# NVlabs/nvbio

Measured on AMD Instinct MI355X. Metric: aligned reads/s (100 bp, band=15), higher is better.
Workload: dtype int32 results (int16 lanes where proven exact; all-int32 kernel in roofline.a32); 1 GPU; nvbio::aln batched banded SW (configs[1]): 10000000 x 100 bp reads vs 150 bp windows per GPU, band=15, LOCAL Gotoh (2,-1,-2,-1); reads_per_gpu=10000000, read_len=100, band=15, type=LOCAL, parallelism=read-shard x1, gather to rank 0

## Files before the change

### include/nvbio_hip.h

```cpp
#ifndef NVBIO_HIP_H
#define NVBIO_HIP_H

#include <stdint.h>

#ifdef __cplusplus
extern "C" {
#endif

#define NVBIO_HIP_ABI_VERSION 2

enum { NVBIO_HIP_GLOBAL = 0, NVBIO_HIP_LOCAL = 1, NVBIO_HIP_SEMI_GLOBAL = 2 };

typedef struct nvbio_hip_string_set {
    const uint32_t* words;
    uint64_t        n_words;
    uint32_t        bits;
    uint32_t        big_endian;
    const uint64_t* begin;
    const uint32_t* length;
    uint32_t        fixed_length;
    uint32_t        _pad;
} nvbio_hip_string_set;

typedef struct nvbio_hip_gotoh_scheme {
    int32_t match, mismatch, gap_open, gap_ext;
} nvbio_hip_gotoh_scheme;


int nvbio_hip_banded_gotoh_score(
    const nvbio_hip_gotoh_scheme* scheme , int32_t type, uint32_t band_len,
    const nvbio_hip_string_set* patterns ,
    const nvbio_hip_string_set* texts    ,
    uint32_t max_pattern_len, uint32_t max_text_len ,
    uint32_t n, int32_t* out_score, uint32_t* out_sink, void* stream);

int nvbio_hip_gotoh_score(
    const nvbio_hip_gotoh_scheme* scheme , int32_t type,
    const nvbio_hip_string_set* patterns, const nvbio_hip_string_set* texts,
    uint32_t max_pattern_len, uint32_t max_text_len, const int32_t* min_score ,
    uint32_t n, int32_t* out_score, uint32_t* out_sink, uint8_t* out_ok, void* stream);

typedef struct nvbio_hip_sw_scheme { int32_t match, mismatch, deletion, insertion; } nvbio_hip_sw_scheme;

int nvbio_hip_banded_sw_score(
    const nvbio_hip_sw_scheme* scheme , int32_t type, uint32_t band_len,
    const nvbio_hip_string_set* patterns, const nvbio_hip_string_set* texts,
    uint32_t max_pattern_len, uint32_t max_text_len,
    uint32_t n, int32_t* out_score, uint32_t* out_sink, void* stream);
int nvbio_hip_sw_score(
    const nvbio_hip_sw_scheme* scheme , int32_t type,
    const nvbio_hip_string_set* patterns, const nvbio_hip_string_set* texts,
    uint32_t max_pattern_len, uint32_t max_text_len,
    uint32_t n, int32_t* out_score, uint32_t* out_sink, void* stream);

enum { NVBIO_HIP_GOTOH_ALIGNER = 0, NVBIO_HIP_SW_ALIGNER = 1 };
enum { NVBIO_HIP_PATTERN_BLOCKING = 0, NVBIO_HIP_TEXT_BLOCKING = 1 };
int nvbio_hip_alignment_score(
    int32_t aligner, int32_t algorithm, const int32_t* scheme4 , int32_t type,
    const nvbio_hip_string_set* patterns, const nvbio_hip_string_set* texts,
    uint32_t max_pattern_len, uint32_t max_text_len, const int32_t* min_score ,
    uint32_t n, int32_t* out_score, uint32_t* out_sink, uint8_t* out_ok , void* stream);

typedef struct nvbio_hip_gotoh_qual_scheme {
    int32_t match;
    int32_t pattern_gap_open, pattern_gap_ext, text_gap_open, text_gap_ext;
    int32_t mismatch[256];
} nvbio_hip_gotoh_qual_scheme;

int nvbio_hip_banded_gotoh_score_qual(
    const nvbio_hip_gotoh_qual_scheme* scheme , int32_t type, uint32_t band_len,
    const nvbio_hip_string_set* patterns, const uint8_t* quals, uint64_t n_quals,
    const nvbio_hip_string_set* texts,
    uint32_t max_pattern_len, uint32_t max_text_len,
    uint32_t n, int32_t* out_score, uint32_t* out_sink, void* stream);

int nvbio_hip_banded_gotoh_score_qual_views(
    const nvbio_hip_gotoh_qual_scheme* scheme , int32_t type, uint32_t band_len,
    const nvbio_hip_string_set* patterns, const uint8_t* quals, uint64_t n_quals, const uint8_t* pattern_flags ,
    const nvbio_hip_string_set* texts,
    uint32_t max_pattern_len, uint32_t max_text_len,
    uint32_t n, int32_t* out_score, uint32_t* out_sink, void* stream);

int nvbio_hip_banded_gotoh_score_qual_wave(
    const nvbio_hip_gotoh_qual_scheme* scheme, int32_t type, uint32_t band_len,
    const nvbio_hip_string_set* patterns, const uint8_t* quals , uint64_t n_quals,
    const nvbio_hip_string_set* texts, uint32_t max_pattern_len,
    uint32_t n, const uint32_t* n_on_device , const uint32_t* job_index , const uint32_t* out_index ,
    const uint32_t* gate , uint32_t gate_limit,
    int32_t* out_score, uint32_t* out_sink, void* stream);

int nvbio_hip_banded_gotoh_score_qual_bounded(
    const nvbio_hip_gotoh_qual_scheme* scheme, int32_t type, uint32_t band_len,
    const nvbio_hip_string_set* patterns, const uint8_t* quals, uint64_t n_quals, const uint8_t* pattern_flags,
    const nvbio_hip_string_set* texts,
    uint32_t max_pattern_len, uint32_t max_text_len,
    uint32_t n, const uint32_t* n_on_device, const int32_t* min_score, uint32_t* work_counter, const uint32_t* out_index,
    const uint32_t* gate , uint32_t gate_limit,
    int32_t* out_score, uint32_t* out_sink, void* stream);

uint64_t nvbio_hip_banded_gotoh_traceback_temp_bytes(uint32_t band_len, uint32_t max_pattern_len, uint32_t n);
int nvbio_hip_banded_gotoh_traceback(
    const nvbio_hip_gotoh_scheme* scheme , int32_t type, uint32_t band_len,
    const nvbio_hip_string_set* patterns, const nvbio_hip_string_set* texts,
    uint32_t max_pattern_len, uint32_t max_text_len, uint32_t n,
    int32_t* out_score, uint32_t* out_sink, uint32_t* out_source,
    uint16_t* out_cigar, uint32_t cigar_stride, uint32_t* out_cigar_len,
    void* temp, uint64_t temp_bytes, void* stream);
int nvbio_hip_banded_gotoh_traceback_qual(
    const nvbio_hip_gotoh_qual_scheme* scheme , int32_t type, uint32_t band_len,
    const nvbio_hip_string_set* patterns, const uint8_t* quals, uint64_t n_quals,
    const nvbio_hip_string_set* texts,
    uint32_t max_pattern_len, uint32_t max_text_len, uint32_t n,
    int32_t* out_score, uint32_t* out_sink, uint32_t* out_source,
    uint16_t* out_cigar, uint32_t cigar_stride, uint32_t* out_cigar_len,
    void* temp, uint64_t temp_bytes, void* stream);
int nvbio_hip_banded_gotoh_traceback_qual_known(
    const nvbio_hip_gotoh_qual_scheme* scheme , int32_t type, uint32_t band_len,
    const nvbio_hip_string_set* patterns, const uint8_t* quals, uint64_t n_quals,
    const nvbio_hip_string_set* texts,
    uint32_t max_pattern_len, uint32_t max_text_len, uint32_t n,
    int32_t* score , uint32_t* sink , uint32_t* out_source,
    uint16_t* out_cigar, uint32_t cigar_stride, uint32_t* out_cigar_len,
    void* temp, uint64_t temp_bytes, void* stream);

uint64_t nvbio_hip_gotoh_traceback_temp_bytes(uint32_t max_pattern_len, uint32_t max_text_len, uint32_t n);
int nvbio_hip_gotoh_traceback(
    const nvbio_hip_gotoh_scheme* scheme , int32_t type,
    const nvbio_hip_string_set* patterns, const nvbio_hip_string_set* texts,
    uint32_t max_pattern_len, uint32_t max_text_len, uint32_t n,
    int32_t* out_score, uint32_t* out_sink, uint32_t* out_source,
    uint16_t* out_cigar, uint32_t cigar_stride, uint32_t* out_cigar_len,
    void* temp, uint64_t temp_bytes, void* stream);

int nvbio_hip_gotoh_traceback_qual(
    const nvbio_hip_gotoh_qual_scheme* scheme , int32_t type,
    const nvbio_hip_string_set* patterns, const uint8_t* quals, uint64_t n_quals, const nvbio_hip_string_set* texts,
    uint32_t max_pattern_len, uint32_t max_text_len, uint32_t n,
    int32_t* out_score, uint32_t* out_sink, uint32_t* out_source,
    uint16_t* out_cigar, uint32_t cigar_stride, uint32_t* out_cigar_len,
    void* temp, uint64_t temp_bytes, void* stream);

int nvbio_hip_gotoh_traceback_known_score(
    const nvbio_hip_gotoh_scheme* scheme , int32_t type,
    const nvbio_hip_string_set* patterns, const nvbio_hip_string_set* texts, const int32_t* known_score,
    uint32_t max_pattern_len, uint32_t max_text_len, uint32_t n,
    int32_t* out_score, uint32_t* out_sink, uint32_t* out_source,
    uint16_t* out_cigar, uint32_t cigar_stride, uint32_t* out_cigar_len,
    void* temp, uint64_t temp_bytes, void* stream);
int nvbio_hip_gotoh_traceback_qual_known_score(
    const nvbio_hip_gotoh_qual_scheme* scheme , int32_t type,
    const nvbio_hip_string_set* patterns, const uint8_t* quals, uint64_t n_quals, const nvbio_hip_string_set* texts, const int32_t* known_score,
    uint32_t max_pattern_len, uint32_t max_text_len, uint32_t n,
    int32_t* out_score, uint32_t* out_sink, uint32_t* out_source,
    uint16_t* out_cigar, uint32_t cigar_stride, uint32_t* out_cigar_len,
    void* temp, uint64_t temp_bytes, void* stream);

uint64_t nvbio_hip_known_score_redone(void);

int nvbio_hip_banded_sw_traceback(
    const nvbio_hip_sw_scheme* scheme , int32_t type, uint32_t band_len,
    const nvbio_hip_string_set* patterns, const nvbio_hip_string_set* texts,
    uint32_t max_pattern_len, uint32_t max_text_len, uint32_t n,
    int32_t* out_score, uint32_t* out_sink, uint32_t* out_source,
    uint16_t* out_cigar, uint32_t cigar_stride, uint32_t* out_cigar_len,
    void* temp, uint64_t temp_bytes, void* stream);
int nvbio_hip_sw_traceback(
    const nvbio_hip_sw_scheme* scheme , int32_t type,
    const nvbio_hip_string_set* patterns, const nvbio_hip_string_set* texts,
    uint32_t max_pattern_len, uint32_t max_text_len, uint32_t n,
    int32_t* out_score, uint32_t* out_sink, uint32_t* out_source,
    uint16_t* out_cigar, uint32_t cigar_stride, uint32_t* out_cigar_len,
    void* temp, uint64_t temp_bytes, void* stream);

int nvbio_hip_alignment_score_qual(
    const nvbio_hip_gotoh_qual_scheme* scheme , int32_t algorithm, int32_t type,
    const nvbio_hip_string_set* patterns, const uint8_t* quals, uint64_t n_quals, const nvbio_hip_string_set* texts,
    uint32_t max_pattern_len, uint32_t max_text_len, const int32_t* min_score ,
    uint32_t n, int32_t* out_score, uint32_t* out_sink, uint8_t* out_ok , void* stream);

int nvbio_hip_alignment_score_qual_jobs(
    const nvbio_hip_gotoh_qual_scheme* scheme , int32_t algorithm, int32_t type,
    const nvbio_hip_string_set* patterns, const uint8_t* quals, uint64_t n_quals, const nvbio_hip_string_set* texts,
    uint32_t max_pattern_len, uint32_t max_text_len, const int32_t* min_score ,
    uint32_t n, const uint32_t* n_on_device, const uint32_t* job_index, const uint32_t* gate, uint32_t gate_limit, int32_t wave_form,
    int32_t* out_score, uint32_t* out_sink, uint8_t* out_ok , void* stream);

int nvbio_hip_hamming_score(
    const nvbio_hip_sw_scheme* scheme , int32_t algorithm, int32_t type,
    const nvbio_hip_string_set* patterns, const nvbio_hip_string_set* texts,
    uint32_t max_pattern_len, uint32_t max_text_len, const int32_t* min_score ,
    uint32_t n, int32_t* out_score, uint32_t* out_sink, uint8_t* out_ok , void* stream);
int nvbio_hip_hamming_score_qual(
    const nvbio_hip_gotoh_qual_scheme* scheme , int32_t algorithm, int32_t type,
    const nvbio_hip_string_set* patterns, const uint8_t* quals, uint64_t n_quals, const nvbio_hip_string_set* texts,
    uint32_t max_pattern_len, uint32_t max_text_len, const int32_t* min_score ,
    uint32_t n, int32_t* out_score, uint32_t* out_sink, uint8_t* out_ok , void* stream);
int nvbio_hip_hamming_score_qual_jobs(
    const nvbio_hip_gotoh_qual_scheme* scheme , int32_t algorithm, int32_t type,
    const nvbio_hip_string_set* patterns, const uint8_t* quals, uint64_t n_quals, const nvbio_hip_string_set* texts,
    uint32_t max_pattern_len, uint32_t max_text_len, const int32_t* min_score ,
    uint32_t n, const uint32_t* n_on_device, const uint32_t* job_index, const uint32_t* gate, uint32_t gate_limit, int32_t wave_form,
    int32_t* out_score, uint32_t* out_sink, uint8_t* out_ok , void* stream);

typedef struct nvbio_hip_fmindex {
    uint32_t        length;
    uint32_t        primary;
    uint32_t        L2[5];
    uint32_t        sa_int;
    const uint32_t* bwt_occ;
    const uint32_t* ssa;
    const uint32_t* ktab;
    uint32_t        ktab_k;
    uint32_t        _pad;
    const uint32_t* dimer;
    uint32_t        dimer_p1, dimer_fill1;
    uint32_t        dimer_S[4], dimer_T[4];
    const uint32_t* trimer;
} nvbio_hip_fmindex;

int nvbio_hip_fm_rank(const nvbio_hip_fmindex* fmi, const uint32_t* k, const uint8_t* c,
                      uint32_t n, uint32_t* out, void* stream);

int nvbio_hip_fm_rank4(const nvbio_hip_fmindex* fmi, const uint32_t* k,
                       uint32_t n, uint32_t* out, void* stream);

int nvbio_hip_fm_rank_range(const nvbio_hip_fmindex* fmi, const uint32_t* range, const uint8_t* c,
                            uint32_t n, uint32_t* out, void* stream);

int nvbio_hip_fm_match(const nvbio_hip_fmindex* fmi, const nvbio_hip_string_set* seeds,
                       uint32_t n, uint32_t* out_range, void* stream);

uint64_t nvbio_hip_fm_dimer_index_bytes(uint32_t length);
uint64_t nvbio_hip_fm_build_dimer_index_temp_bytes(uint32_t length);
int nvbio_hip_fm_build_dimer_index(const nvbio_hip_fmindex* fmi, uint32_t* out_dimer, void* temp, uint64_t temp_bytes, void* stream);
int nvbio_hip_fm_attach_dimer_index(nvbio_hip_fmindex* fmi, const uint32_t* dimer, void* stream);

uint64_t nvbio_hip_fm_trimer_index_bytes(uint32_t length);
uint64_t nvbio_hip_fm_build_trimer_index_temp_bytes(uint32_t length);
int nvbio_hip_fm_build_trimer_index(const nvbio_hip_fmindex* fmi, uint32_t* out_trimer, void* temp, uint64_t temp_bytes, void* stream);
int nvbio_hip_fm_attach_trimer_index(nvbio_hip_fmindex* fmi, const uint32_t* trimer, void* stream);

int nvbio_hip_banded_gotoh_score_host(const nvbio_hip_gotoh_scheme* scheme, int32_t type, uint32_t band_len,
                                      const nvbio_hip_string_set* patterns, const nvbio_hip_string_set* texts,
                                      uint32_t n, int32_t* out_score, uint32_t* out_sink, int32_t n_threads);
int nvbio_hip_banded_sw_score_host(const nvbio_hip_sw_scheme* scheme, int32_t type, uint32_t band_len,
                                   const nvbio_hip_string_set* patterns, const nvbio_hip_string_set* texts,
                                   uint32_t n, int32_t* out_score, uint32_t* out_sink, int32_t n_threads);
int nvbio_hip_alignment_score_host(int32_t aligner, int32_t algorithm, const int32_t* scheme4, int32_t type,
                                   const nvbio_hip_string_set* patterns, const nvbio_hip_string_set* texts, const int32_t* min_score ,
                                   uint32_t n, int32_t* out_score, uint32_t* out_sink, uint8_t* out_ok , int32_t n_threads);
int nvbio_hip_hamming_score_host(const nvbio_hip_sw_scheme* scheme, int32_t algorithm, int32_t type,
                                 const nvbio_hip_string_set* patterns, const nvbio_hip_string_set* texts, const int32_t* min_score ,
                                 uint32_t n, int32_t* out_score, uint32_t* out_sink, uint8_t* out_ok , int32_t n_threads);
int nvbio_hip_hamming_score_qual_host(const nvbio_hip_gotoh_qual_scheme* scheme, int32_t algorithm, int32_t type,
                                      const nvbio_hip_string_set* patterns, const uint8_t* quals, uint64_t n_quals, const nvbio_hip_string_set* texts,
                                      const int32_t* min_score ,
                                      uint32_t n, int32_t* out_score, uint32_t* out_sink, uint8_t* out_ok , int32_t n_threads);
int nvbio_hip_fm_rank_host(const nvbio_hip_fmindex* fmi, const uint32_t* k, const uint8_t* c, uint32_t n, uint32_t* out, int32_t n_threads);
int nvbio_hip_fm_match_host(const nvbio_hip_fmindex* fmi, const nvbio_hip_string_set* seeds, uint32_t n, uint32_t* out_range, int32_t n_threads);
int nvbio_hip_fm_locate_host(const nvbio_hip_fmindex* fmi, const uint32_t* sa_rows, uint32_t n, uint32_t* out_pos, int32_t n_threads);

int nvbio_hip_fm_build_ktab(const nvbio_hip_fmindex* fmi, uint32_t k, uint32_t* out_ktab, void* stream);
uint64_t nvbio_hip_fm_dense_ssa_entries(uint32_t length, uint32_t sa_int);
int nvbio_hip_fm_build_dense_ssa(const nvbio_hip_fmindex* fmi, uint32_t sa_int_out, uint32_t* out_ssa, void* stream);

typedef struct nvbio_hip_map_params {
    uint32_t seed_len;
    uint32_t min_read_len;
    uint32_t max_hits;
    uint32_t max_reseed;
    uint32_t retry;
    uint32_t rep_seeds;
    uint32_t fw, rc;
} nvbio_hip_map_params;

int nvbio_hip_map_exact(const nvbio_hip_fmindex* fmi, const nvbio_hip_string_set* reads,
                        const uint32_t* in_queue, uint32_t n, const nvbio_hip_map_params* params ,
                        const uint32_t* seed_freq_by_len ,
                        uint64_t* out_hits, uint32_t hits_stride, uint32_t* out_counts, uint8_t* out_reseed, void* stream);

enum { NVBIO_HIP_EXACT_MAPPING = 0, NVBIO_HIP_APPROX_MAPPING = 1, NVBIO_HIP_CASE_PRUNING_MAPPING = 2 };

int nvbio_hip_map(int32_t algorithm, uint32_t subseed_len,
                  const nvbio_hip_fmindex* fmi, const nvbio_hip_fmindex* rfmi ,
                  const nvbio_hip_string_set* reads, const uint32_t* in_queue, uint32_t n,
                  const nvbio_hip_map_params* params , const uint32_t* seed_freq_by_len ,
                  uint64_t* out_hits, uint32_t hits_stride, uint32_t* out_counts, uint8_t* out_reseed, void* stream);

uint64_t nvbio_hip_alignment_invalid(void);
int nvbio_hip_init_alignments(uint32_t n_reads, const uint32_t* read_len , uint32_t fixed_read_len,
                              const int32_t* worst_score_by_len , uint32_t mate,
                              uint64_t* best_alignments, uint32_t best_stride, void* stream);
int nvbio_hip_score_reduce(uint32_t n_active, const uint32_t* read_ids , const uint64_t* hit_begin,
                           const int32_t* hit_score, const uint32_t* hit_loc, const uint8_t* hit_rc,
                           const uint32_t* read_len , uint32_t fixed_read_len,
                           uint64_t* best_alignments, uint32_t best_stride, void* stream);

uint32_t nvbio_hip_sum_tree_node_count(uint32_t size);
int nvbio_hip_select_init(uint32_t n_reads, const char* read_names, const uint32_t* read_names_idx,
                          const uint64_t* hits, uint32_t hits_stride, const uint32_t* hit_counts,
                          float* probs, uint32_t probs_stride, uint32_t* trys , uint32_t* rseeds,
                          uint32_t max_effort_init, int32_t randomized, int32_t top_seed, void* stream);
int nvbio_hip_select_init_queued(uint32_t n_queue, const uint32_t* queue, const char* read_names, const uint32_t* read_names_idx,
                                 const uint64_t* hits, uint32_t hits_stride, const uint32_t* hit_counts,
                                 float* probs, uint32_t probs_stride, uint32_t* trys , uint32_t* rseeds,
                                 uint32_t max_effort_init, int32_t randomized, int32_t top_seed, void* stream);
uint64_t nvbio_hip_select_temp_bytes(uint32_t n_active, uint32_t n_multi);
int nvbio_hip_select(int32_t randomized, uint32_t n_multi, const uint32_t* active_in, uint32_t n_active,
                     uint64_t* hits, uint32_t hits_stride, uint32_t* hit_counts,
                     float* probs, uint32_t probs_stride, uint32_t* rseeds, const uint32_t* trys,
                     uint32_t* active_out, uint64_t* hit_begin, uint32_t* hit_read_id, uint32_t* hit_loc, uint32_t* hit_seed,
                     uint32_t* out_sizes, void* temp, uint64_t temp_bytes, void* stream);
int nvbio_hip_hit_deque_replay(uint32_t n_cases, const uint32_t* case_start, const uint8_t* ops, const uint64_t* vals, const uint32_t* caps,
                               const uint64_t* state_start, uint64_t* scratch, uint32_t scratch_stride, uint64_t* out_states, void* stream);
int nvbio_hip_locate_hits(const nvbio_hip_fmindex* fmi, const nvbio_hip_fmindex* rfmi, uint32_t n,
                          uint32_t* hit_loc, const uint32_t* hit_seed, void* stream);
int nvbio_hip_score_best_setup(uint32_t n_hits, const uint32_t* hit_read_id, const uint32_t* hit_loc, const uint32_t* hit_seed,
                               const uint64_t* read_begin , const uint32_t* read_len , uint32_t fixed_read_len,
                               uint64_t rc_offset, uint32_t band_len, uint32_t genome_length,
                               const uint64_t* best_alignments, uint32_t best_stride, int32_t score_limit,
                               uint64_t* pattern_begin, uint32_t* pattern_len ,
                               uint64_t* text_begin, uint32_t* text_len, int32_t* min_score,
                               int32_t* known_score ,
                               uint32_t* job_count , uint32_t* job_hit , void* stream);
int nvbio_hip_score_reduce_best_approx(uint32_t n_active, const uint32_t* active_reads, const uint64_t* hit_begin,
                                       const int32_t* hit_score, const uint32_t* hit_loc, const uint32_t* hit_seed,
                                       const uint32_t* read_len , uint32_t fixed_read_len,
                                       uint64_t* best_alignments, uint32_t best_stride, int32_t worst_score,
                                       uint32_t* trys, uint32_t* hit_counts,
                                       uint32_t n_ext, uint32_t min_ext, uint32_t max_ext, uint32_t max_effort,
                                       const int32_t* known_score ,
                                       const uint32_t* hit_sink , uint32_t* best_sink ,
                                       void* stream);
int nvbio_hip_traceback_best_known(uint32_t n, const uint32_t* idx , const uint64_t* best_alignments, const uint32_t* best_sink ,
                                   int32_t* out_score, uint32_t* out_sink , void* stream);

int nvbio_hip_score_reduce_paired(uint32_t n_active, const uint32_t* read_ids , const uint64_t* hit_begin,
    const uint32_t* hit_loc, const uint32_t* hit_sink, const int32_t* hit_score, const uint8_t* hit_rc,
    const uint32_t* opposite_loc, const uint32_t* opposite_sink, const uint32_t* opposite_sink2,
    const int32_t* opposite_score, const int32_t* opposite_score2,
    const uint32_t* read_len , uint32_t fixed_read_len, uint32_t anchor, int32_t pe_policy, int32_t pe_unpaired, int32_t score_limit,
    uint64_t* best_alignments, uint64_t* best_alignments_o, uint32_t best_stride, void* stream);

typedef struct nvbio_hip_pe_params {
    int32_t  pe_policy, min_frag_len, max_frag_len, pe_overlap, score_limit;
    uint32_t anchor, genome_length;
} nvbio_hip_pe_params;

int nvbio_hip_opposite_mate_windows(uint32_t n_hits, const uint32_t* hit_read_id, const uint8_t* hit_rc, const uint32_t* hit_loc, const int32_t* hit_score,
    const uint32_t* a_read_len , const uint32_t* o_read_len , uint32_t a_fixed_len, uint32_t o_fixed_len,
    const uint64_t* best_alignments, const uint64_t* best_alignments_o, uint32_t best_stride,
    int32_t match, const int32_t* min_score_by_len , int32_t text_gap_open, int32_t text_gap_ext, const nvbio_hip_pe_params* params ,
    uint8_t* out_valid, int32_t* out_min_score, uint8_t* out_read_rc, uint32_t* out_genome_begin, uint32_t* out_genome_end, void* stream);

int nvbio_hip_anchor_score_setup(uint32_t n_hits, const uint32_t* hit_read_id, const uint32_t* hit_loc, const uint32_t* hit_seed,
    const uint64_t* a_read_begin , const uint32_t* a_read_len , const uint32_t* o_read_len ,
    uint32_t a_fixed_len, uint32_t o_fixed_len, uint64_t rc_offset,
    uint32_t band_len, uint32_t genome_length, const uint64_t* best_alignments, const uint64_t* best_alignments_o, uint32_t best_stride,
    int32_t match, const int32_t* min_score_by_len , int32_t score_limit, uint32_t anchor,
    uint64_t* pattern_begin, uint32_t* pattern_len , uint64_t* text_begin, uint32_t* text_len, int32_t* min_score, void* stream);
int nvbio_hip_anchor_score_finish(uint32_t n_hits, const int32_t* raw_score, const uint32_t* raw_sink , const uint64_t* text_begin,
    const int32_t* min_score, int32_t worst_score, int32_t* hit_score, uint32_t* hit_sink, void* stream);
int nvbio_hip_opposite_score_setup(uint32_t n_hits, const uint32_t* hit_read_id, const uint32_t* hit_seed, const uint32_t* hit_loc, const int32_t* hit_score,
    int32_t worst_score, const uint32_t* a_read_len, const uint32_t* o_read_len, uint32_t a_fixed_len, uint32_t o_fixed_len,
    const uint64_t* best_alignments, const uint64_t* best_alignments_o, uint32_t best_stride,
    int32_t match, const int32_t* min_score_by_len , int32_t text_gap_open, int32_t text_gap_ext, const nvbio_hip_pe_params* params ,
    uint8_t* out_valid, int32_t* out_min_score, uint8_t* out_read_rc, uint32_t* out_genome_begin, uint32_t* out_genome_end,
    const uint64_t* o_read_begin, uint64_t o_rc_offset, uint64_t* out_pattern_begin, uint64_t* out_text_begin, uint32_t* out_text_len, void* stream);
int nvbio_hip_opposite_score_finish(uint32_t n_valid, const uint32_t* valid_idx, const uint8_t* valid_flags, const int32_t* raw_score , const uint32_t* raw_sink ,
    const int32_t* min_score , const uint32_t* genome_begin , int32_t worst_score,
    int32_t* opposite_score, int32_t* opposite_score2, uint32_t* opposite_loc, uint32_t* opposite_sink, uint32_t* opposite_sink2, void* stream);
int nvbio_hip_score_reduce_paired_best_approx(uint32_t n_active, const uint32_t* active_reads, const uint64_t* hit_begin,
    const uint32_t* hit_loc, const uint32_t* hit_sink, const int32_t* hit_score, const uint32_t* hit_seed,
    const uint32_t* opposite_loc, const uint32_t* opposite_sink, const uint32_t* opposite_sink2, const int32_t* opposite_score, const int32_t* opposite_score2,
    const uint32_t* read_len , uint32_t fixed_read_len, uint32_t anchor, int32_t pe_policy, int32_t pe_unpaired, int32_t score_limit,
    uint64_t* best_alignments, uint64_t* best_alignments_o, uint32_t best_stride,
    uint32_t* trys, uint32_t* hit_counts, uint32_t n_ext, uint32_t min_ext, uint32_t max_ext, uint32_t max_effort, void* stream);
int nvbio_hip_anchor_memo_mark(uint32_t n_hits, const uint32_t* hit_read_id, const uint32_t* hit_seed, const uint64_t* text_begin, const uint32_t* text_len,
    uint32_t anchor, const uint32_t* memo, uint8_t* from_memo, uint32_t* text_len_out,
    uint32_t* live_count , uint32_t* live_idx , void* stream);
int nvbio_hip_anchor_score_finish_memo(uint32_t n_hits, const int32_t* raw_score, const uint32_t* raw_sink, const uint64_t* text_begin, const int32_t* min_score,
    int32_t worst_score, const uint8_t* from_memo, const uint32_t* hit_read_id, const uint32_t* memo, int32_t* hit_score, uint32_t* hit_sink, void* stream);
int nvbio_hip_anchor_memo_update(uint32_t n_active, const uint32_t* active_reads, const uint64_t* hit_begin, const uint32_t* hit_read_id, const uint32_t* hit_seed,
    const uint64_t* text_begin, const uint32_t* text_len_setup, const uint8_t* from_memo, const int32_t* raw_score, const uint32_t* raw_sink, uint32_t anchor, uint32_t* memo, void* stream);
int nvbio_hip_list_flagged(uint32_t n, const uint8_t* flags, uint32_t value, uint32_t* count, uint32_t* idx, void* stream);
int nvbio_hip_opposite_memo_lookup(uint32_t n_hits, const uint32_t* hit_read_id, uint8_t* valid, const uint8_t* read_rc, const uint32_t* genome_begin,
    const uint32_t* genome_end, const int32_t* min_score, uint32_t anchor, const uint32_t* memo, int32_t worst_score,
    int32_t* opposite_score, int32_t* opposite_score2, uint32_t* opposite_loc, uint32_t* opposite_sink, uint32_t* opposite_sink2,
    uint32_t* text_len , void* stream);
int nvbio_hip_opposite_memo_update(uint32_t n_active, const uint32_t* active_reads, const uint64_t* hit_begin, const uint8_t* valid, const uint8_t* read_rc,
    const uint32_t* genome_begin, const uint32_t* genome_end, const int32_t* min_score, const int32_t* opposite_score, const uint32_t* opposite_sink,
    uint32_t anchor, uint32_t* memo, void* stream);
int nvbio_hip_mark_discordant(uint32_t n_reads, uint64_t* best_alignments, uint64_t* best_alignments_o, uint32_t best_stride, void* stream);

int nvbio_hip_pack_read_queue(uint32_t n, const uint32_t* queue, uint32_t top_flag, uint32_t* out, void* stream);

int nvbio_hip_mark_unaligned(uint32_t n_active, const uint32_t* active_reads, const uint64_t* best_alignments, uint8_t* reseed, void* stream);
uint64_t nvbio_hip_copy_flagged_temp_bytes(uint32_t n);
int nvbio_hip_copy_flagged(uint32_t n, const uint32_t* in, const uint8_t* flags, uint32_t* out, uint32_t* out_count ,
                           void* temp, uint64_t temp_bytes, void* stream);
int nvbio_hip_scatter_rows(uint32_t n, const uint32_t* idx, const void* src, void* dst, uint32_t row_bytes , void* stream);
int nvbio_hip_gather_rows(uint32_t n, const uint32_t* idx, const void* src, void* dst, uint32_t row_bytes , void* stream);
int nvbio_hip_traceback_best_setup(uint32_t n, const uint32_t* idx , const uint64_t* best_alignments, uint32_t band_len, uint32_t genome_length,
                                   const uint64_t* read_begin , const uint32_t* read_len , uint32_t fixed_read_len,
                                   uint64_t rc_offset, uint64_t mate_offset, int32_t want,
                                   uint8_t* out_valid, uint64_t* pattern_begin, uint32_t* pattern_len ,
                                   uint64_t* text_begin, uint32_t* text_len, void* stream);
int nvbio_hip_traceback_best_setup_mates(uint32_t n, const uint32_t* idx , const uint64_t* best_alignments, uint32_t band_len, uint32_t genome_length,
                                         const uint64_t* const read_begin[2] , const uint32_t* const read_len[2],
                                         const uint32_t fixed_read_len[2], const uint64_t rc_offset[2], uint64_t mate_offset, int32_t want,
                                         uint8_t* out_valid, uint64_t* pattern_begin, uint32_t* pattern_len, uint64_t* text_begin, uint32_t* text_len, void* stream);

int nvbio_hip_finish_alignment(uint32_t n, const uint8_t* valid, const nvbio_hip_string_set* patterns, const uint8_t* quals , uint64_t n_quals,
                               const nvbio_hip_string_set* texts, const uint16_t* cigar, uint32_t cigar_stride, const uint32_t* cigar_len,
                               const uint32_t* cigar_source , int32_t match, const int32_t* mismatch_by_quality , int32_t n_penalty,
                               const int32_t* gap_costs , const uint32_t* idx , uint64_t* best_alignments, uint8_t* out_mds, uint32_t mds_stride, uint32_t* out_mds_len, void* stream);

int nvbio_hip_gather_ranges(uint32_t n_ranges, uint32_t n_reads, const uint64_t* hits, uint32_t hits_stride, const uint32_t* hit_count_scan,
                            uint64_t* out_ranges, void* stream);
int nvbio_hip_select_all(uint64_t begin, uint32_t count, uint32_t n_reads, uint32_t n_ranges, const uint64_t* hits, uint32_t hits_stride,
                         const uint32_t* hit_count_scan, const uint64_t* hit_range_scan, uint32_t* out_loc, uint32_t* out_seed, uint32_t* out_read_id,
                         void* stream);
int nvbio_hip_mark_straddling(uint32_t n, const uint32_t* idx_queue, uint32_t n_sequences, const uint32_t* sequence_index, const uint32_t* hit_loc,
                              uint32_t seed_len, uint8_t* flags, void* stream);
int nvbio_hip_score_all_setup(uint32_t n, const uint32_t* idx , const uint32_t* hit_read_id, const uint32_t* hit_loc, const uint32_t* hit_seed,
                              const uint64_t* read_begin , const uint32_t* read_len , uint32_t fixed_read_len, uint64_t rc_offset,
                              uint32_t band_len, uint32_t genome_length,
                              uint64_t* pattern_begin, uint32_t* pattern_len , uint64_t* text_begin, uint32_t* text_len, void* stream);
int nvbio_hip_score_all_output(uint32_t n, const uint32_t* idx , const uint32_t* hit_read_id, const uint32_t* hit_loc, const uint32_t* hit_seed,
                               const int32_t* score, const int32_t* min_score_by_len , const uint32_t* read_len , uint32_t fixed_read_len,
                               uint8_t* out_flags, uint64_t* out_alignments, uint32_t* out_read_id, void* stream);
int nvbio_hip_traceback_all_setup(uint32_t n, const uint64_t* alignments, const uint32_t* read_id,
                                  const uint64_t* read_begin , const uint32_t* read_len , uint32_t fixed_read_len, uint64_t rc_offset,
                                  uint32_t band_len, uint32_t genome_length,
                                  uint64_t* pattern_begin, uint32_t* pattern_len , uint64_t* text_begin, uint32_t* text_len, void* stream);

uint64_t nvbio_hip_all_mapping_temp_bytes(uint32_t n);
int nvbio_hip_inclusive_scan_u32(uint32_t n, const uint32_t* in, uint32_t* out, void* temp, uint64_t temp_bytes, void* stream);
int nvbio_hip_inclusive_scan_u64(uint32_t n, const uint64_t* in, uint64_t* out, void* temp, uint64_t temp_bytes, void* stream);
int nvbio_hip_sort_hi_bits(uint32_t n, const uint32_t* keys, uint32_t* out_idx, void* temp, uint64_t temp_bytes, void* stream);
int nvbio_hip_sort_hits(uint32_t n, const uint32_t* hit_read_id, const uint32_t* hit_loc, const uint32_t* hit_seed, uint32_t* out_idx, uint8_t* out_first,
                        void* temp, uint64_t temp_bytes, void* stream);
int nvbio_hip_sort_hits_pingpong(uint32_t n, const uint32_t* hit_read_id, const uint32_t* hit_loc, const uint32_t* hit_seed, uint32_t* out_idx, uint8_t* out_first,
                                 uint32_t* out_stale, void* temp, uint64_t temp_bytes, void* stream);

int nvbio_hip_mapq(int32_t version, int32_t match, int32_t monotone, const int32_t* min_score_by_len ,
                   uint32_t n_reads, const uint64_t* best_alignments, uint32_t best_stride,
                   const uint32_t* read_len , uint32_t fixed_read_len, uint8_t* out_mapq, void* stream);

int nvbio_hip_mapq_paired(int32_t version, int32_t match, int32_t monotone, const int32_t* min_score_by_len ,
                          uint32_t n_reads, const uint64_t* best_alignments, const uint64_t* best_alignments_o, uint32_t best_stride,
                          const uint32_t* read_len , const uint32_t* o_read_len ,
                          uint32_t fixed_read_len, uint32_t o_fixed_read_len, uint8_t* out_mapq, void* stream);

int nvbio_hip_fm_locate(const nvbio_hip_fmindex* fmi, const uint32_t* sa_rows,
                        uint32_t n, uint32_t* out_pos, void* stream);

int nvbio_hip_fm_locate_ssa_iterator(const nvbio_hip_fmindex* fmi, const uint32_t* sa_rows,
                                     uint32_t n, uint32_t* out_it, void* stream);
int nvbio_hip_fm_lookup_ssa_iterator(const nvbio_hip_fmindex* fmi, const uint32_t* it,
                                     uint32_t n, uint32_t* out_pos, void* stream);

uint64_t nvbio_hip_fm_filter_temp_bytes(uint32_t n);
int nvbio_hip_fm_filter_rank(const nvbio_hip_fmindex* fmi, const nvbio_hip_string_set* seeds,
                             uint32_t n, uint32_t* out_range, uint64_t* out_slots,
                             void* temp, uint64_t temp_bytes, void* stream);

int nvbio_hip_fm_filter_locate(const nvbio_hip_fmindex* fmi, const uint32_t* range, const uint64_t* slots,
                               uint32_t n_queries, uint64_t begin, uint64_t end,
                               uint32_t* out_hits, void* stream);

#define NVBIO_HIP_EXTEND_FORWARD   0
#define NVBIO_HIP_EXTEND_BACKWARDS 1
int nvbio_hip_fm_extend(int32_t direction, const nvbio_hip_fmindex* f_fmi, const nvbio_hip_fmindex* r_fmi,
                        const uint32_t* f_ranges, const uint32_t* r_ranges, const uint8_t* c, uint32_t n,
                        uint32_t* out_f_ranges, uint32_t* out_r_ranges, void* stream);

#define NVBIO_HIP_ERROR_CAPACITY 0x10001
uint64_t nvbio_hip_fm_mem_temp_bytes(uint32_t n, uint32_t max_pattern_len);
int nvbio_hip_fm_mem_rank(const nvbio_hip_fmindex* f_fmi, const nvbio_hip_fmindex* r_fmi, const nvbio_hip_string_set* strings,
                          uint32_t n, uint32_t max_pattern_len, uint32_t min_intv, uint32_t max_intv, uint32_t min_span,
                          uint32_t* out_ranges, uint64_t capacity, uint64_t* out_index, uint64_t* out_slots, uint64_t* out_n_ranges,
                          void* temp, uint64_t temp_bytes, void* stream);

int nvbio_hip_fm_mem_locate(const nvbio_hip_fmindex* f_fmi, const uint32_t* ranges, const uint64_t* slots, uint64_t n_ranges,
                            uint64_t begin, uint64_t end, uint32_t* out_hits, void* stream);

int nvbio_hip_fm_extend_host(int32_t direction, const nvbio_hip_fmindex* f_fmi, const nvbio_hip_fmindex* r_fmi,
                             const uint32_t* f_ranges, const uint32_t* r_ranges, const uint8_t* c, uint32_t n,
                             uint32_t* out_f_ranges, uint32_t* out_r_ranges, int32_t n_threads);
int nvbio_hip_fm_mem_rank_host(const nvbio_hip_fmindex* f_fmi, const nvbio_hip_fmindex* r_fmi, const nvbio_hip_string_set* strings,
                               uint32_t n, uint32_t max_pattern_len, uint32_t min_intv, uint32_t max_intv, uint32_t min_span,
                               uint32_t* out_ranges, uint64_t capacity, uint64_t* out_index, uint64_t* out_slots, uint64_t* out_n_ranges,
                               uint64_t* out_records, int32_t n_threads);
int nvbio_hip_fm_mem_locate_host(const nvbio_hip_fmindex* f_fmi, const uint32_t* ranges, const uint64_t* slots, uint64_t n_ranges,
                                 uint64_t begin, uint64_t end, uint32_t* out_hits, int32_t n_threads);

uint64_t nvbio_hip_fm_mem_split_temp_bytes(uint32_t n, uint32_t max_pattern_len, uint64_t capacity);
int nvbio_hip_fm_mem_rank_split(const nvbio_hip_fmindex* f_fmi, const nvbio_hip_fmindex* r_fmi, const nvbio_hip_string_set* strings,
                                uint32_t n, uint32_t max_pattern_len, uint32_t min_intv, uint32_t max_intv, uint32_t min_span,
                                uint32_t split_len, uint32_t split_width,
                                uint32_t* out_ranges, uint64_t capacity, uint64_t* out_index, uint64_t* out_slots, uint64_t* out_n_ranges,
                                void* temp, uint64_t temp_bytes, void* stream);
int nvbio_hip_fm_mem_rank_split_host(const nvbio_hip_fmindex* f_fmi, const nvbio_hip_fmindex* r_fmi, const nvbio_hip_string_set* strings,
                                     uint32_t n, uint32_t max_pattern_len, uint32_t min_intv, uint32_t max_intv, uint32_t min_span,
                                     uint32_t split_len, uint32_t split_width,
                                     uint32_t* out_ranges, uint64_t capacity, uint64_t* out_index, uint64_t* out_slots, uint64_t* out_n_ranges,
                                     uint64_t* out_records, int32_t n_threads);

uint64_t nvbio_hip_build_bwt_occ_temp_bytes(uint32_t n);
int nvbio_hip_build_bwt_occ(uint32_t n, const uint32_t* bwt_words, uint32_t* out_bwt_occ, uint32_t* out_L2,
                            void* temp, uint64_t temp_bytes, void* stream);

uint64_t nvbio_hip_suffix_sort_temp_bytes(uint64_t n);
int nvbio_hip_suffix_sort(const uint32_t* words, uint32_t bits, uint32_t big_endian, uint64_t n, uint32_t* sa_out,
                          void* temp, uint64_t temp_bytes, void* stream);
uint32_t nvbio_hip_suffix_sort_last_rounds(uint64_t* out_unresolved, uint32_t capacity);
uint64_t nvbio_hip_bwt_temp_bytes(uint64_t n);
int nvbio_hip_bwt(const uint32_t* words, uint32_t bits, uint32_t big_endian, uint64_t n, uint32_t sa_int, uint32_t* bwt_words_out,
                  uint32_t* primary_out, uint32_t* ssa_out, uint32_t* sa_out, void* temp, uint64_t temp_bytes, void* stream);
int nvbio_hip_suffix_sort_host(const uint32_t* words, uint32_t bits, uint32_t big_endian, uint64_t n, uint32_t* sa_out, int32_t n_threads);
int nvbio_hip_bwt_host(const uint32_t* words, uint32_t bits, uint32_t big_endian, uint64_t n, uint32_t sa_int, uint32_t* bwt_words_out,
                       uint32_t* primary_out, uint32_t* ssa_out, uint32_t* sa_out, int32_t n_threads);

int nvbio_hip_device_malloc(void** ptr, uint64_t bytes);
int nvbio_hip_device_free(void* ptr);
int nvbio_hip_device_free_ordered(void* ptr);
int nvbio_hip_device_free_after(void* ptr, void* stream);
int nvbio_hip_device_trim(void);
int nvbio_hip_device_mem_info(uint64_t* free_bytes, uint64_t* total_bytes, uint64_t* idle_cached_bytes);
int nvbio_hip_memcpy(void* dst, const void* src, uint64_t bytes, int kind, void* stream);
int nvbio_hip_memset(void* dst, int value, uint64_t bytes, void* stream);
int nvbio_hip_stream_synchronize(void* stream);
int nvbio_hip_stream_query(void* stream);
int nvbio_hip_host_malloc(void** ptr, uint64_t bytes);
int nvbio_hip_host_free(void* ptr);

int nvbio_hip_stream_create(void** stream, uint32_t non_blocking);
int nvbio_hip_stream_destroy(void* stream);

int nvbio_hip_comm_available(void);
int nvbio_hip_device_count(void);
int nvbio_hip_set_device(int device);
int nvbio_hip_get_device(void);
int nvbio_hip_comm_unique_id(uint8_t* id128);
int nvbio_hip_comm_init_rank(void** comm, int world, int rank, const uint8_t* id128);
int nvbio_hip_comm_init_all(void** comms, int n_devices, const int* devices );
int nvbio_hip_comm_destroy(void* comm);
int nvbio_hip_comm_rank(void* comm, int* rank, int* world);
int nvbio_hip_gather_records(void* comm, const void* send, const uint64_t* counts, uint32_t record_bytes, void* recv , int root, void* stream);
int nvbio_hip_comm_abort(void* comm);
typedef struct nvbio_hip_comm_transport {
    int (*rank)(void* comm, int* rank, int* world);
    int (*group_start)(void* comm);
    int (*group_end)(void* comm);
    int (*send)(void* comm, const void* buf, uint64_t bytes, int peer, void* stream);
    int (*recv)(void* comm, void* buf, uint64_t bytes, int peer, void* stream);
    int (*copy)(void* comm, void* dst, const void* src, uint64_t bytes, void* stream);
    int (*abort)(void* comm);
} nvbio_hip_comm_transport;
void nvbio_hip_comm_set_transport(const nvbio_hip_comm_transport* transport);

int nvbio_hip_set_test_switch(const char* name, int value);
int nvbio_hip_get_test_switch(const char* name);
const char* nvbio_hip_test_switch_name(int index);

int         nvbio_hip_abi_version(void);
const char* nvbio_hip_arch(void);
const char* nvbio_hip_last_kernel(void);
const char* nvbio_hip_last_kernel_detail(void);
const char* nvbio_hip_last_kernel_cell(void);
const char* nvbio_hip_last_kernel_frame(void);
const char* nvbio_hip_last_kernel_row(void);
const char* nvbio_hip_last_kernel_const(void);
const char* nvbio_hip_last_kernel_fetch(void);

#ifdef __cplusplus
}
#endif
#endif
```

### nvbio_amd/_lib.py

```python
import ctypes as C
import os

HERE = os.path.dirname(os.path.abspath(__file__))
LIB_PATH = os.path.join(HERE, "lib", "libnvbio_hip.so")

SYMBOLS = [
    "nvbio_hip_banded_gotoh_score", "nvbio_hip_banded_gotoh_score_qual", "nvbio_hip_banded_gotoh_score_qual_views", "nvbio_hip_banded_gotoh_score_qual_bounded", "nvbio_hip_banded_gotoh_score_qual_wave", "nvbio_hip_gotoh_score", "nvbio_hip_banded_sw_score", "nvbio_hip_sw_score", "nvbio_hip_alignment_score", "nvbio_hip_alignment_score_qual", "nvbio_hip_alignment_score_qual_jobs",
    "nvbio_hip_hamming_score", "nvbio_hip_hamming_score_qual", "nvbio_hip_hamming_score_qual_jobs", "nvbio_hip_hamming_score_host", "nvbio_hip_hamming_score_qual_host",
    "nvbio_hip_banded_gotoh_traceback_temp_bytes", "nvbio_hip_banded_gotoh_traceback", "nvbio_hip_banded_gotoh_traceback_qual",
    "nvbio_hip_gotoh_traceback_temp_bytes", "nvbio_hip_gotoh_traceback", "nvbio_hip_gotoh_traceback_qual", "nvbio_hip_gotoh_traceback_known_score", "nvbio_hip_gotoh_traceback_qual_known_score", "nvbio_hip_known_score_redone", "nvbio_hip_banded_sw_traceback", "nvbio_hip_sw_traceback",
    "nvbio_hip_fm_rank", "nvbio_hip_fm_rank4", "nvbio_hip_fm_rank_range",
    "nvbio_hip_fm_match", "nvbio_hip_fm_build_ktab", "nvbio_hip_fm_dense_ssa_entries", "nvbio_hip_fm_build_dense_ssa",
    "nvbio_hip_banded_gotoh_score_host", "nvbio_hip_banded_sw_score_host", "nvbio_hip_alignment_score_host",
    "nvbio_hip_fm_rank_host", "nvbio_hip_fm_match_host", "nvbio_hip_fm_locate_host",
    "nvbio_hip_fm_dimer_index_bytes", "nvbio_hip_fm_build_dimer_index_temp_bytes", "nvbio_hip_fm_build_dimer_index", "nvbio_hip_fm_attach_dimer_index",
    "nvbio_hip_fm_trimer_index_bytes", "nvbio_hip_fm_build_trimer_index_temp_bytes", "nvbio_hip_fm_build_trimer_index", "nvbio_hip_fm_attach_trimer_index", "nvbio_hip_map_exact", "nvbio_hip_map",
    "nvbio_hip_alignment_invalid", "nvbio_hip_init_alignments", "nvbio_hip_score_reduce", "nvbio_hip_score_reduce_paired", "nvbio_hip_opposite_mate_windows", "nvbio_hip_mapq", "nvbio_hip_mapq_paired", "nvbio_hip_fm_locate",
    "nvbio_hip_sum_tree_node_count", "nvbio_hip_select_init", "nvbio_hip_select_init_queued", "nvbio_hip_select_temp_bytes", "nvbio_hip_select", "nvbio_hip_locate_hits", "nvbio_hip_hit_deque_replay",
    "nvbio_hip_score_best_setup", "nvbio_hip_score_reduce_best_approx",
    "nvbio_hip_anchor_score_setup", "nvbio_hip_anchor_score_finish", "nvbio_hip_anchor_memo_mark", "nvbio_hip_anchor_score_finish_memo", "nvbio_hip_anchor_memo_update", "nvbio_hip_opposite_score_setup", "nvbio_hip_opposite_score_finish",
    "nvbio_hip_score_reduce_paired_best_approx", "nvbio_hip_mark_discordant",
    "nvbio_hip_pack_read_queue", "nvbio_hip_mark_unaligned", "nvbio_hip_copy_flagged_temp_bytes", "nvbio_hip_copy_flagged", "nvbio_hip_traceback_best_setup", "nvbio_hip_traceback_best_setup_mates", "nvbio_hip_finish_alignment", "nvbio_hip_scatter_rows",
    "nvbio_hip_gather_ranges", "nvbio_hip_select_all", "nvbio_hip_mark_straddling", "nvbio_hip_score_all_setup", "nvbio_hip_score_all_output",
    "nvbio_hip_traceback_all_setup", "nvbio_hip_all_mapping_temp_bytes", "nvbio_hip_inclusive_scan_u32", "nvbio_hip_inclusive_scan_u64", "nvbio_hip_sort_hi_bits",
    "nvbio_hip_sort_hits", "nvbio_hip_sort_hits_pingpong", "nvbio_hip_gather_rows", "nvbio_hip_list_flagged", "nvbio_hip_opposite_memo_lookup", "nvbio_hip_opposite_memo_update", "nvbio_hip_traceback_best_known", "nvbio_hip_banded_gotoh_traceback_qual_known",
    "nvbio_hip_fm_locate_ssa_iterator", "nvbio_hip_fm_lookup_ssa_iterator",
    "nvbio_hip_fm_filter_temp_bytes", "nvbio_hip_fm_filter_rank", "nvbio_hip_fm_filter_locate",
    "nvbio_hip_fm_extend", "nvbio_hip_fm_mem_temp_bytes", "nvbio_hip_fm_mem_rank", "nvbio_hip_fm_mem_locate",
    "nvbio_hip_fm_extend_host", "nvbio_hip_fm_mem_rank_host", "nvbio_hip_fm_mem_locate_host",
    "nvbio_hip_fm_mem_split_temp_bytes", "nvbio_hip_fm_mem_rank_split", "nvbio_hip_fm_mem_rank_split_host",
    "nvbio_hip_build_bwt_occ_temp_bytes", "nvbio_hip_build_bwt_occ",
    "nvbio_hip_suffix_sort_temp_bytes", "nvbio_hip_suffix_sort", "nvbio_hip_suffix_sort_last_rounds", "nvbio_hip_bwt_temp_bytes", "nvbio_hip_bwt",
    "nvbio_hip_suffix_sort_host", "nvbio_hip_bwt_host",
    "nvbio_hip_device_malloc", "nvbio_hip_device_free", "nvbio_hip_device_free_ordered", "nvbio_hip_device_free_after", "nvbio_hip_device_trim", "nvbio_hip_device_mem_info", "nvbio_hip_memcpy", "nvbio_hip_memset",
    "nvbio_hip_stream_synchronize", "nvbio_hip_stream_query", "nvbio_hip_host_malloc", "nvbio_hip_host_free", "nvbio_hip_stream_create", "nvbio_hip_stream_destroy",
    "nvbio_hip_comm_available", "nvbio_hip_device_count", "nvbio_hip_set_device", "nvbio_hip_get_device", "nvbio_hip_comm_unique_id", "nvbio_hip_comm_init_rank",
    "nvbio_hip_comm_init_all", "nvbio_hip_comm_destroy", "nvbio_hip_comm_rank", "nvbio_hip_gather_records", "nvbio_hip_comm_abort", "nvbio_hip_comm_set_transport",
    "nvbio_hip_abi_version", "nvbio_hip_arch", "nvbio_hip_last_kernel", "nvbio_hip_last_kernel_detail", "nvbio_hip_last_kernel_cell", "nvbio_hip_last_kernel_frame", "nvbio_hip_last_kernel_row", "nvbio_hip_last_kernel_const", "nvbio_hip_last_kernel_fetch", "nvbio_hip_set_test_switch", "nvbio_hip_get_test_switch", "nvbio_hip_test_switch_name",
]


class PeParamsStruct(C.Structure):
    _fields_ = [("pe_policy", C.c_int32), ("min_frag_len", C.c_int32), ("max_frag_len", C.c_int32), ("pe_overlap", C.c_int32),
                ("score_limit", C.c_int32), ("anchor", C.c_uint32), ("genome_length", C.c_uint32)]


class StringSetStruct(C.Structure):
    _fields_ = [("words", C.c_void_p), ("n_words", C.c_uint64), ("bits", C.c_uint32), ("big_endian", C.c_uint32),
                ("begin", C.c_void_p), ("length", C.c_void_p), ("fixed_length", C.c_uint32), ("_pad", C.c_uint32)]


class GotohSchemeStruct(C.Structure):
    _fields_ = [("match", C.c_int32), ("mismatch", C.c_int32), ("gap_open", C.c_int32), ("gap_ext", C.c_int32)]


class GotohQualSchemeStruct(C.Structure):
    _fields_ = [("match", C.c_int32), ("pattern_gap_open", C.c_int32), ("pattern_gap_ext", C.c_int32),
                ("text_gap_open", C.c_int32), ("text_gap_ext", C.c_int32), ("mismatch", C.c_int32 * 256)]


class MapParamsStruct(C.Structure):
    _fields_ = [(k, C.c_uint32) for k in ("seed_len", "min_read_len", "max_hits", "max_reseed", "retry", "rep_seeds", "fw", "rc")]


class FMIndexStruct(C.Structure):
    _fields_ = [("length", C.c_uint32), ("primary", C.c_uint32), ("L2", C.c_uint32 * 5), ("sa_int", C.c_uint32),
                ("bwt_occ", C.c_void_p), ("ssa", C.c_void_p), ("ktab", C.c_void_p), ("ktab_k", C.c_uint32), ("_pad", C.c_uint32),
                ("dimer", C.c_void_p), ("dimer_p1", C.c_uint32), ("dimer_fill1", C.c_uint32),
                ("dimer_S", C.c_uint32 * 4), ("dimer_T", C.c_uint32 * 4), ("trimer", C.c_void_p)]


_lib = None
ABI_VERSION = 2
ERROR_CAPACITY = 0x10001


def lib():
    global _lib
    if _lib is None:
        if not os.path.exists(LIB_PATH):
            raise RuntimeError(
                "nvbio_amd: %s is missing -- build it with `python -m nvbio_amd.build` "
                "(hipcc --offload-arch=gfx950); there is no CPU fallback" % LIB_PATH)
        L = C.CDLL(LIB_PATH)
        try:
            L.nvbio_hip_abi_version.restype = C.c_int
            found = L.nvbio_hip_abi_version()
        except AttributeError:
            found = None
        if found != ABI_VERSION:
            raise RuntimeError("nvbio_amd: lib/libnvbio_hip.so has ABI version %s, this package needs %d -- rebuild it (python -m nvbio_amd.build)" % (found, ABI_VERSION))
        for s in SYMBOLS:
            getattr(L, s)
        vp, u32, u64, i32 = C.c_void_p, C.c_uint32, C.c_uint64, C.c_int32
        P = C.POINTER
        L.nvbio_hip_banded_gotoh_score.argtypes = [P(GotohSchemeStruct), i32, u32, P(StringSetStruct), P(StringSetStruct), u32, u32, u32, vp, vp, vp]
        L.nvbio_hip_banded_gotoh_score_qual.argtypes = [P(GotohQualSchemeStruct), i32, u32, P(StringSetStruct), vp, u64, P(StringSetStruct), u32, u32, u32, vp, vp, vp]
        L.nvbio_hip_banded_gotoh_score_qual_views.argtypes = [P(GotohQualSchemeStruct), i32, u32, P(StringSetStruct), vp, u64, vp, P(StringSetStruct), u32, u32, u32, vp, vp, vp]
        L.nvbio_hip_banded_gotoh_score_qual_bounded.argtypes = [P(GotohQualSchemeStruct), i32, u32, P(StringSetStruct), vp, u64, vp, P(StringSetStruct), u32, u32, u32, vp, vp, vp, vp, vp, u32, vp, vp, vp]
        L.nvbio_hip_banded_gotoh_score_qual_wave.argtypes = [P(GotohQualSchemeStruct), i32, u32, P(StringSetStruct), vp, u64, P(StringSetStruct), u32, u32, vp, vp, vp, vp, u32, vp, vp, vp]
        L.nvbio_hip_banded_gotoh_traceback_temp_bytes.argtypes = [u32, u32, u32]
        L.nvbio_hip_banded_gotoh_traceback_temp_bytes.restype = u64
        L.nvbio_hip_banded_gotoh_traceback.argtypes = [P(GotohSchemeStruct), i32, u32, P(StringSetStruct), P(StringSetStruct), u32, u32, u32,
                                                       vp, vp, vp, vp, u32, vp, vp, u64, vp]
        L.nvbio_hip_banded_gotoh_traceback_qual.argtypes = [P(GotohQualSchemeStruct), i32, u32, P(StringSetStruct), vp, u64, P(StringSetStruct), u32, u32, u32,
                                                            vp, vp, vp, vp, u32, vp, vp, u64, vp]
        L.nvbio_hip_banded_gotoh_traceback_qual_known.argtypes = [P(GotohQualSchemeStruct), i32, u32, P(StringSetStruct), vp, u64, P(StringSetStruct), u32, u32, u32,
                                                            vp, vp, vp, vp, u32, vp, vp, u64, vp]
        L.nvbio_hip_banded_sw_score.argtypes = [P(GotohSchemeStruct), i32, u32, P(StringSetStruct), P(StringSetStruct), u32, u32, u32, vp, vp, vp]
        L.nvbio_hip_sw_score.argtypes = [P(GotohSchemeStruct), i32, P(StringSetStruct), P(StringSetStruct), u32, u32, u32, vp, vp, vp]
        L.nvbio_hip_alignment_score.argtypes = [i32, i32, vp, i32, P(StringSetStruct), P(StringSetStruct), u32, u32, vp, u32, vp, vp, vp, vp]
        L.nvbio_hip_gotoh_traceback_temp_bytes.argtypes = [u32, u32, u32]
        L.nvbio_hip_gotoh_traceback_temp_bytes.restype = u64
        L.nvbio_hip_gotoh_traceback.argtypes = [P(GotohSchemeStruct), i32, P(StringSetStruct), P(StringSetStruct), u32, u32, u32,
                                                vp, vp, vp, vp, u32, vp, vp, u64, vp]
        L.nvbio_hip_gotoh_traceback_qual.argtypes = [P(GotohQualSchemeStruct), i32, P(StringSetStruct), vp, u64, P(StringSetStruct), u32, u32, u32,
                                                     vp, vp, vp, vp, u32, vp, vp, u64, vp]
        L.nvbio_hip_gotoh_traceback_known_score.argtypes = [P(GotohSchemeStruct), i32, P(StringSetStruct), P(StringSetStruct), vp, u32, u32, u32,
                                                            vp, vp, vp, vp, u32, vp, vp, u64, vp]
        L.nvbio_hip_gotoh_traceback_qual_known_score.argtypes = [P(GotohQualSchemeStruct), i32, P(StringSetStruct), vp, u64, P(StringSetStruct), vp, u32, u32, u32,
                                                                 vp, vp, vp, vp, u32, vp, vp, u64, vp]
        L.nvbio_hip_known_score_redone.argtypes = []; L.nvbio_hip_known_score_redone.restype = u64
        L.nvbio_hip_banded_sw_traceback.argtypes = [P(GotohSchemeStruct), i32, u32, P(StringSetStruct), P(StringSetStruct), u32, u32, u32,
                                                    vp, vp, vp, vp, u32, vp, vp, u64, vp]
        L.nvbio_hip_sw_traceback.argtypes = [P(GotohSchemeStruct), i32, P(StringSetStruct), P(StringSetStruct), u32, u32, u32,
                                             vp, vp, vp, vp, u32, vp, vp, u64, vp]
        L.nvbio_hip_alignment_score_qual.argtypes = [P(GotohQualSchemeStruct), i32, i32, P(StringSetStruct), vp, u64, P(StringSetStruct), u32, u32, vp, u32, vp, vp, vp, vp]
        L.nvbio_hip_gotoh_score.argtypes = [P(GotohSchemeStruct), i32, P(StringSetStruct), P(StringSetStruct), u32, u32, vp, u32, vp, vp, vp, vp]
        L.nvbio_hip_hamming_score.argtypes = [P(GotohSchemeStruct), i32, i32, P(StringSetStruct), P(StringSetStruct), u32, u32, vp, u32, vp, vp, vp, vp]
        L.nvbio_hip_hamming_score_qual.argtypes = [P(GotohQualSchemeStruct), i32, i32, P(StringSetStruct), vp, u64, P(StringSetStruct), u32, u32, vp, u32, vp, vp, vp, vp]
        L.nvbio_hip_hamming_score_qual_jobs.argtypes = [P(GotohQualSchemeStruct), i32, i32, P(StringSetStruct), vp, u64, P(StringSetStruct), u32, u32, vp,
                                                        u32, vp, vp, vp, u32, i32, vp, vp, vp, vp]
        L.nvbio_hip_hamming_score_host.argtypes = [P(GotohSchemeStruct), i32, i32, P(StringSetStruct), P(StringSetStruct), vp, u32, vp, vp, vp, i32]
        L.nvbio_hip_hamming_score_qual_host.argtypes = [P(GotohQualSchemeStruct), i32, i32, P(StringSetStruct), vp, u64, P(StringSetStruct), vp, u32, vp, vp, vp, i32]
        L.nvbio_hip_fm_rank.argtypes = [P(FMIndexStruct), vp, vp, u32, vp, vp]
        L.nvbio_hip_fm_rank4.argtypes = [P(FMIndexStruct), vp, u32, vp, vp]
        L.nvbio_hip_fm_rank_range.argtypes = [P(FMIndexStruct), vp, vp, u32, vp, vp]
        L.nvbio_hip_fm_match.argtypes = [P(FMIndexStruct), P(StringSetStruct), u32, vp, vp]
        L.nvbio_hip_fm_build_ktab.argtypes = [P(FMIndexStruct), u32, vp, vp]
        L.nvbio_hip_banded_gotoh_score_host.argtypes = [P(GotohSchemeStruct), i32, u32, P(StringSetStruct), P(StringSetStruct), u32, vp, vp, i32]
        L.nvbio_hip_banded_sw_score_host.argtypes = [P(GotohSchemeStruct), i32, u32, P(StringSetStruct), P(StringSetStruct), u32, vp, vp, i32]
        L.nvbio_hip_alignment_score_host.argtypes = [i32, i32, vp, i32, P(StringSetStruct), P(StringSetStruct), vp, u32, vp, vp, vp, i32]
        L.nvbio_hip_fm_rank_host.argtypes = [P(FMIndexStruct), vp, vp, u32, vp, i32]
        L.nvbio_hip_fm_match_host.argtypes = [P(FMIndexStruct), P(StringSetStruct), u32, vp, i32]
        L.nvbio_hip_fm_locate_host.argtypes = [P(FMIndexStruct), vp, u32, vp, i32]
        L.nvbio_hip_fm_dimer_index_bytes.argtypes = [u32]; L.nvbio_hip_fm_dimer_index_bytes.restype = u64
        L.nvbio_hip_fm_build_dimer_index_temp_bytes.argtypes = [u32]; L.nvbio_hip_fm_build_dimer_index_temp_bytes.restype = u64
        L.nvbio_hip_fm_build_dimer_index.argtypes = [P(FMIndexStruct), vp, vp, u64, vp]
        L.nvbio_hip_fm_attach_dimer_index.argtypes = [P(FMIndexStruct), vp, vp]
        L.nvbio_hip_fm_trimer_index_bytes.argtypes = [u32]; L.nvbio_hip_fm_trimer_index_bytes.restype = u64
        L.nvbio_hip_fm_build_trimer_index_temp_bytes.argtypes = [u32]; L.nvbio_hip_fm_build_trimer_index_temp_bytes.restype = u64
        L.nvbio_hip_fm_build_trimer_index.argtypes = [P(FMIndexStruct), vp, vp, u64, vp]
        L.nvbio_hip_fm_attach_trimer_index.argtypes = [P(FMIndexStruct), vp, vp]
        L.nvbio_hip_map_exact.argtypes = [P(FMIndexStruct), P(StringSetStruct), vp, u32, P(MapParamsStruct), vp, vp, u32, vp, vp, vp]
        L.nvbio_hip_map.argtypes = [i32, u32, P(FMIndexStruct), P(FMIndexStruct), P(StringSetStruct), vp, u32, P(MapParamsStruct), vp, vp, u32, vp, vp, vp]
        L.nvbio_hip_alignment_invalid.argtypes = []
        L.nvbio_hip_alignment_invalid.restype = u64
        L.nvbio_hip_init_alignments.argtypes = [u32, vp, u32, vp, u32, vp, u32, vp]
        L.nvbio_hip_score_reduce.argtypes = [u32, vp, vp, vp, vp, vp, vp, u32, vp, u32, vp]
        L.nvbio_hip_sum_tree_node_count.argtypes = [u32]; L.nvbio_hip_sum_tree_node_count.restype = u32
        L.nvbio_hip_select_init.argtypes = [u32, vp, vp, vp, u32, vp, vp, u32, vp, vp, u32, i32, i32, vp]
        L.nvbio_hip_select_init_queued.argtypes = [u32, vp, vp, vp, vp, u32, vp, vp, u32, vp, vp, u32, i32, i32, vp]
        L.nvbio_hip_select_temp_bytes.argtypes = [u32, u32]; L.nvbio_hip_select_temp_bytes.restype = u64
        L.nvbio_hip_select.argtypes = [i32, u32, vp, u32, vp, u32, vp, vp, u32, vp, vp, vp, vp, vp, vp, vp, vp, vp, u64, vp]
        L.nvbio_hip_hit_deque_replay.argtypes = [u32, vp, vp, vp, vp, vp, vp, u32, vp, vp]
        L.nvbio_hip_locate_hits.argtypes = [P(FMIndexStruct), P(FMIndexStruct), u32, vp, vp, vp]
        L.nvbio_hip_score_best_setup.argtypes = [u32, vp, vp, vp, vp, vp, u32, u64, u32, u32, vp, u32, i32, vp, vp, vp, vp, vp, vp, vp, vp, vp]
        L.nvbio_hip_score_reduce_best_approx.argtypes = [u32, vp, vp, vp, vp, vp, vp, u32, vp, u32, i32, vp, vp, u32, u32, u32, u32, vp, vp, vp, vp]
        L.nvbio_hip_traceback_best_known.argtypes = [u32, vp, vp, vp, vp, vp, vp]
        L.nvbio_hip_anchor_score_setup.argtypes = [u32, vp, vp, vp, vp, vp, vp, u32, u32, u64, u32, u32, vp, vp, u32, i32, vp, i32, u32, vp, vp, vp, vp, vp, vp]
        L.nvbio_hip_anchor_score_finish.argtypes = [u32, vp, vp, vp, vp, i32, vp, vp, vp]
        L.nvbio_hip_opposite_score_setup.argtypes = [u32, vp, vp, vp, vp, i32, vp, vp, u32, u32, vp, vp, u32, i32, vp, i32, i32, P(PeParamsStruct), vp, vp, vp, vp, vp, vp, u64, vp, vp, vp, vp]
        L.nvbio_hip_scatter_rows.argtypes = [u32, vp, vp, vp, u32, vp]
        L.nvbio_hip_gather_rows.argtypes = [u32, vp, vp, vp, u32, vp]
        L.nvbio_hip_opposite_memo_lookup.argtypes = [u32, vp, vp, vp, vp, vp, vp, u32, vp, i32, vp, vp, vp, vp, vp, vp, vp]
        L.nvbio_hip_opposite_memo_update.argtypes = [u32, vp, vp, vp, vp, vp, vp, vp, vp, vp, u32, vp, vp]
        L.nvbio_hip_gather_ranges.argtypes = [u32, u32, vp, u32, vp, vp, vp]
        L.nvbio_hip_select_all.argtypes = [u64, u32, u32, u32, vp, u32, vp, vp, vp, vp, vp, vp]
        L.nvbio_hip_mark_straddling.argtypes = [u32, vp, u32, vp, vp, u32, vp, vp]
        L.nvbio_hip_score_all_setup.argtypes = [u32, vp, vp, vp, vp, vp, vp, u32, u64, u32, u32, vp, vp, vp, vp, vp]
        L.nvbio_hip_score_all_output.argtypes = [u32, vp, vp, vp, vp, vp, vp, vp, u32, vp, vp, vp, vp]
        L.nvbio_hip_traceback_all_setup.argtypes = [u32, vp, vp, vp, vp, u32, u64, u32, u32, vp, vp, vp, vp, vp]
        L.nvbio_hip_all_mapping_temp_bytes.argtypes = [u32]; L.nvbio_hip_all_mapping_temp_bytes.restype = u64
        L.nvbio_hip_inclusive_scan_u32.argtypes = [u32, vp, vp, vp, u64, vp]
        L.nvbio_hip_inclusive_scan_u64.argtypes = [u32, vp, vp, vp, u64, vp]
        L.nvbio_hip_sort_hi_bits.argtypes = [u32, vp, vp, vp, u64, vp]
        L.nvbio_hip_sort_hits.argtypes = [u32, vp, vp, vp, vp, vp, vp, u64, vp]
        L.nvbio_hip_sort_hits_pingpong.argtypes = [u32, vp, vp, vp, vp, vp, vp, vp, u64, vp]
        L.nvbio_hip_opposite_score_finish.argtypes = [u32, vp, vp, vp, vp, vp, vp, i32, vp, vp, vp, vp, vp, vp]
        L.nvbio_hip_score_reduce_paired_best_approx.argtypes = [u32, vp, vp, vp, vp, vp, vp, vp, vp, vp, vp, vp, vp, u32, u32, i32, i32, i32, vp, vp, u32, vp, vp, u32, u32, u32, u32, vp]
        L.nvbio_hip_mark_discordant.argtypes = [u32, vp, vp, u32, vp]
        L.nvbio_hip_pack_read_queue.argtypes = [u32, vp, u32, vp, vp]
        L.nvbio_hip_mark_unaligned.argtypes = [u32, vp, vp, vp, vp]
        L.nvbio_hip_copy_flagged_temp_bytes.argtypes = [u32]; L.nvbio_hip_copy_flagged_temp_bytes.restype = u64
        L.nvbio_hip_copy_flagged.argtypes = [u32, vp, vp, vp, vp, vp, u64, vp]
        L.nvbio_hip_finish_alignment.argtypes = [u32, vp, P(StringSetStruct), vp, u64, P(StringSetStruct), vp, u32, vp, vp, i32, vp, i32, vp, vp, vp, vp, u32, vp, vp]
        L.nvbio_hip_traceback_best_setup.argtypes = [u32, vp, vp, u32, u32, vp, vp, u32, u64, u64, i32, vp, vp, vp, vp, vp, vp]
        L.nvbio_hip_traceback_best_setup_mates.argtypes = [u32, vp, vp, u32, u32, C.POINTER(C.c_void_p), C.POINTER(C.c_void_p), C.POINTER(C.c_uint32), C.POINTER(C.c_uint64),
                                                           u64, i32, vp, vp, vp, vp, vp, vp]
        L.nvbio_hip_score_reduce_paired.argtypes = [u32, vp, vp, vp, vp, vp, vp, vp, vp, vp, vp, vp, vp, u32, u32, i32, i32, i32, vp, vp, u32, vp]
        L.nvbio_hip_opposite_mate_windows.argtypes = [u32, vp, vp, vp, vp, vp, vp, u32, u32, vp, vp, u32, i32, vp, i32, i32, P(PeParamsStruct),
                                                      vp, vp, vp, vp, vp, vp]
        L.nvbio_hip_mapq.argtypes = [i32, i32, i32, vp, u32, vp, u32, vp, u32, vp, vp]
        L.nvbio_hip_mapq_paired.argtypes = [i32, i32, i32, vp, u32, vp, vp, u32, vp, vp, u32, u32, vp, vp]
        L.nvbio_hip_fm_locate.argtypes = [P(FMIndexStruct), vp, u32, vp, vp]
        L.nvbio_hip_fm_locate_ssa_iterator.argtypes = [P(FMIndexStruct), vp, u32, vp, vp]
        L.nvbio_hip_fm_lookup_ssa_iterator.argtypes = [P(FMIndexStruct), vp, u32, vp, vp]
        L.nvbio_hip_fm_filter_temp_bytes.argtypes = [u32]
        L.nvbio_hip_fm_filter_temp_bytes.restype = u64
        L.nvbio_hip_fm_filter_rank.argtypes = [P(FMIndexStruct), P(StringSetStruct), u32, vp, vp, vp, u64, vp]
        L.nvbio_hip_fm_filter_locate.argtypes = [P(FMIndexStruct), vp, vp, u32, u64, u64, vp, vp]
        L.nvbio_hip_fm_extend.argtypes = [i32, P(FMIndexStruct), P(FMIndexStruct), vp, vp, vp, u32, vp, vp, vp]
        L.nvbio_hip_fm_mem_temp_bytes.argtypes = [u32, u32]
        L.nvbio_hip_fm_mem_temp_bytes.restype = u64
        L.nvbio_hip_fm_mem_rank.argtypes = [P(FMIndexStruct), P(FMIndexStruct), P(StringSetStruct), u32, u32, u32, u32, u32, vp, u64, vp, vp, P(u64), vp, u64, vp]
        L.nvbio_hip_fm_mem_locate.argtypes = [P(FMIndexStruct), vp, vp, u64, u64, u64, vp, vp]
        L.nvbio_hip_fm_extend_host.argtypes = [i32, P(FMIndexStruct), P(FMIndexStruct), vp, vp, vp, u32, vp, vp, i32]
        L.nvbio_hip_fm_mem_rank_host.argtypes = [P(FMIndexStruct), P(FMIndexStruct), P(StringSetStruct), u32, u32, u32, u32, u32, vp, u64, vp, vp, P(u64), P(u64), i32]
        L.nvbio_hip_fm_mem_locate_host.argtypes = [P(FMIndexStruct), vp, vp, u64, u64, u64, vp, i32]
        L.nvbio_hip_fm_mem_split_temp_bytes.argtypes = [u32, u32, u64]
        L.nvbio_hip_fm_mem_split_temp_bytes.restype = u64
        L.nvbio_hip_fm_mem_rank_split.argtypes = [P(FMIndexStruct), P(FMIndexStruct), P(StringSetStruct), u32, u32, u32, u32, u32, u32, u32, vp, u64, vp, vp, P(u64), vp, u64, vp]
        L.nvbio_hip_fm_mem_rank_split_host.argtypes = [P(FMIndexStruct), P(FMIndexStruct), P(StringSetStruct), u32, u32, u32, u32, u32, u32, u32, vp, u64, vp, vp, P(u64), P(u64), i32]
        L.nvbio_hip_build_bwt_occ_temp_bytes.argtypes = [u32]
        L.nvbio_hip_build_bwt_occ_temp_bytes.restype = u64
        L.nvbio_hip_build_bwt_occ.argtypes = [u32, vp, vp, vp, vp, u64, vp]
        L.nvbio_hip_suffix_sort_temp_bytes.argtypes = [u64]
        L.nvbio_hip_suffix_sort_temp_bytes.restype = u64
        L.nvbio_hip_suffix_sort.argtypes = [vp, u32, u32, u64, vp, vp, u64, vp]
        L.nvbio_hip_suffix_sort_last_rounds.argtypes = [P(u64), u32]
        L.nvbio_hip_suffix_sort_last_rounds.restype = u32
        L.nvbio_hip_bwt_temp_bytes.argtypes = [u64]
        L.nvbio_hip_bwt_temp_bytes.restype = u64
        L.nvbio_hip_bwt.argtypes = [vp, u32, u32, u64, u32, vp, P(u32), vp, vp, vp, u64, vp]
        L.nvbio_hip_suffix_sort_host.argtypes = [vp, u32, u32, u64, vp, i32]
        L.nvbio_hip_bwt_host.argtypes = [vp, u32, u32, u64, u32, vp, P(u32), vp, vp, i32]
        L.nvbio_hip_comm_unique_id.argtypes = [vp]
        L.nvbio_hip_comm_init_rank.argtypes = [P(vp), C.c_int, C.c_int, vp]
        L.nvbio_hip_comm_init_all.argtypes = [vp, C.c_int, vp]
        L.nvbio_hip_comm_destroy.argtypes = [vp]
        L.nvbio_hip_comm_rank.argtypes = [vp, P(C.c_int), P(C.c_int)]
        L.nvbio_hip_gather_records.argtypes = [vp, vp, vp, u32, vp, C.c_int, vp]
        L.nvbio_hip_set_device.argtypes = [C.c_int]
        L.nvbio_hip_abi_version.restype = C.c_int
        L.nvbio_hip_set_test_switch.argtypes = [C.c_char_p, C.c_int]
        L.nvbio_hip_get_test_switch.argtypes = [C.c_char_p]
        L.nvbio_hip_fm_dense_ssa_entries.argtypes = [u32, u32]
        L.nvbio_hip_fm_dense_ssa_entries.restype = u64
        L.nvbio_hip_fm_build_dense_ssa.argtypes = [P(FMIndexStruct), u32, vp, vp]
        L.nvbio_hip_test_switch_name.argtypes = [C.c_int]
        L.nvbio_hip_test_switch_name.restype = C.c_char_p
        L.nvbio_hip_device_free_after.argtypes = [vp, vp]
        L.nvbio_hip_device_mem_info.argtypes = [P(u64), P(u64), P(u64)]
        L.nvbio_hip_arch.restype = C.c_char_p
        L.nvbio_hip_last_kernel.restype = C.c_char_p
        L.nvbio_hip_last_kernel_detail.restype = C.c_char_p
        L.nvbio_hip_last_kernel_cell.restype = C.c_char_p
        L.nvbio_hip_last_kernel_frame.restype = C.c_char_p
        L.nvbio_hip_last_kernel_fetch.restype = C.c_char_p
        L.nvbio_hip_last_kernel_row.restype = C.c_char_p
        L.nvbio_hip_last_kernel_const.restype = C.c_char_p
        _lib = L
    return _lib


def check(err, what):
    if err != 0:
        raise RuntimeError("nvbio_amd: %s failed with hipError %d" % (what, err))


def test_switch_names():
    out, k = [], 0
    while True:
        n = lib().nvbio_hip_test_switch_name(k)
        if not n:
            return out
        out.append(n.decode()); k += 1


def device_mem_info():
    f, t, i = C.c_uint64(), C.c_uint64(), C.c_uint64()
    check(lib().nvbio_hip_device_mem_info(C.byref(f), C.byref(t), C.byref(i)), "nvbio_hip_device_mem_info")
    return f.value, t.value, i.value


def set_test_switch(name, value):
    check(lib().nvbio_hip_set_test_switch(name.encode(), int(value)), "nvbio_hip_set_test_switch(%s)" % name)


class test_switch:

    def __init__(self, name, value):
        self.name, self.value = name, int(value)

    def __enter__(self):
        self.saved = lib().nvbio_hip_get_test_switch(self.name.encode())
        set_test_switch(self.name, self.value)
        return self

    def __exit__(self, *exc):
        set_test_switch(self.name, self.saved)
        return False


def current_stream_ptr():
    import torch
    if not torch.cuda.is_available():
        return C.c_void_p(0)
    return C.c_void_p(torch.cuda.current_stream().cuda_stream)
```

### nvbio_amd/csrc/banded_gotoh.hip

```cpp
#include "banded_gotoh_bounded.h"
#define NVB_PAIR_EXTERN
#include "banded_gotoh_pair.h"
#include <mutex>
#include <unordered_map>
#include <atomic>
#include <vector>
#include <algorithm>
#include <cstring>
#include <cstdlib>

namespace nvb {

thread_local const char* g_last_kernel = "";
thread_local PairLaunch g_last_pair;

#define NVB_DECL(B) \
    extern template hipError_t launch_band_width<B, NoQual>(const GotohParams&, const NoQual&, int, bool, hipStream_t); \
    extern template hipError_t launch_band_width<B, QualArgs>(const GotohParams&, const QualArgs&, int, bool, hipStream_t);
NVB_DECL(3) NVB_DECL(5) NVB_DECL(7) NVB_DECL(15) NVB_DECL(31)
#undef NVB_DECL
#define NVB_DECL(B) extern template hipError_t launch_band_width_asym<B>(const GotohParams&, int, bool, hipStream_t);
NVB_DECL(3) NVB_DECL(5) NVB_DECL(7) NVB_DECL(15) NVB_DECL(31)
#undef NVB_DECL
#define NVB_DECL(B) \
    extern template hipError_t launch_band_width_bounded<B, NoQual>(const GotohParams&, const NoQual&, const BoundArgs&, int, bool, hipStream_t); \
    extern template hipError_t launch_band_width_bounded<B, QualArgs>(const GotohParams&, const QualArgs&, const BoundArgs&, int, bool, hipStream_t);
NVB_DECL(3) NVB_DECL(5) NVB_DECL(7) NVB_DECL(15) NVB_DECL(31)
#undef NVB_DECL

template <typename QA>
static hipError_t launch_bounded(const GotohParams& p, const QA& qa, const BoundArgs& ba, int type, uint32_t band, bool width16, hipStream_t s)
{
    switch (band) {
    case 3:  return launch_band_width_bounded<3, QA>(p, qa, ba, type, width16, s);
    case 5:  return launch_band_width_bounded<5, QA>(p, qa, ba, type, width16, s);
    case 7:  return launch_band_width_bounded<7, QA>(p, qa, ba, type, width16, s);
    case 15: return launch_band_width_bounded<15, QA>(p, qa, ba, type, width16, s);
    case 31: return launch_band_width_bounded<31, QA>(p, qa, ba, type, width16, s);
    default: return hipErrorNotSupported;
    }
}

static hipError_t launch_asym(const GotohParams& p, int type, uint32_t band, bool width16, hipStream_t s)
{
    switch (band) {
    case 3:  return launch_band_width_asym<3>(p, type, width16, s);
    case 5:  return launch_band_width_asym<5>(p, type, width16, s);
    case 7:  return launch_band_width_asym<7>(p, type, width16, s);
    case 15: return launch_band_width_asym<15>(p, type, width16, s);
    case 31: return launch_band_width_asym<31>(p, type, width16, s);
    default: return hipErrorNotSupported;
    }
}

template <typename QA>
static hipError_t launch(const GotohParams& p, const QA& qa, int type, uint32_t band, bool width16, hipStream_t s)
{
    switch (band) {
    case 3:  return launch_band_width<3, QA>(p, qa, type, width16, s);
    case 5:  return launch_band_width<5, QA>(p, qa, type, width16, s);
    case 7:  return launch_band_width<7, QA>(p, qa, type, width16, s);
    case 15: return launch_band_width<15, QA>(p, qa, type, width16, s);
    case 31: return launch_band_width<31, QA>(p, qa, type, width16, s);
    default: return hipErrorNotSupported;
    }
}

static uint32_t max_len_16bit(int32_t match, int32_t best_pair , int64_t A , int32_t gap_open, int32_t gap_ext, int type, uint32_t band,
                              int32_t row_step )
{
    if (gap_open > 0 || gap_ext > 0) return 0;
    if (A == 0) return 0xFFFFFFFFu;
    if (type == NVBIO_HIP_LOCAL) {
        if (match < 0 || A > 100) return 0;
        const int64_t per_row = int64_t(std::max(best_pair, 0)) + row_step;
        if (per_row <= 0) return 0xFFFFFFFFu;
        return uint32_t(1022 / per_row);
    }
    const int64_t lim = (15000 / A - int64_t(band) - 2) / (row_step ? 2 : 1);
    return lim <= 0 ? 0u : uint32_t(lim);
}

static bool pair_admitted(const GotohParams& p, int type, uint32_t band, uint32_t lim16)
{
    if (test_switch(SW_BANDED_PAIR) == 1 || type != NVBIO_HIP_LOCAL || band != 15u) return false;
    if (p.pat.length || p.txt.length || p.n_dev || p.out_index || p.gate) return false;
    const uint32_t M = p.pat.fixed_length, N = p.txt.fixed_length;
    if (M == 0u || M > lim16 || uint64_t(N) < uint64_t(M) + band - 1u) return false;
    if (p.gap_ext > 0 || p.gap_open > p.gap_ext) return false;
    return p.mismatch >= p.gap_open && int64_t(std::max(p.match, p.mismatch)) - p.gap_open <= 7 && p.match >= p.gap_open;
}

static bool pair_stream_admitted(const GotohParams& p)
{
    return p.pat.s.bits != 8u && p.pat.s.n_words <= (1ull << 29) && p.txt.s.n_words <= (1ull << 29);
}
template <typename CELL, int ROW>
static hipError_t launch_pair_row(const GotohParams& p, hipStream_t s)
{
    g_last_pair.row = (ROW & PF_ROW2) ? "fold2" : "plain";
    g_last_pair.consts = (ROW & PF_CONST2) ? "literal" : "scalar";
    g_last_pair.fetch = "generic";
    if (!pair_stream_admitted(p)) return launch_band_pair<15, CELL, PF_SINK_VCC | ROW>(p, s);
    g_last_pair.fetch = "stream";
    switch (PF_STREAM | (p.pat.s.bits == 2u ? PF_PAT2 : 0) | (p.pat.s.big_endian ? PF_PBE : 0) | (p.txt.s.big_endian ? PF_TBE : 0)) {
#define NVB_CASE(F) case (F): return launch_band_pair<15, CELL, (F) | ROW>(p, s);
    NVB_PAIR_STREAM_FORMS(NVB_CASE)
#undef NVB_CASE
    }
    return hipErrorNotSupported;
}
template <typename CELL>
static hipError_t launch_pair(const GotohParams& p, hipStream_t s)
{
    if constexpr (CELL::COLUMN)
    {
        if (test_switch(SW_PAIR_ROW) != 1)
        {
            if (test_switch(SW_PAIR_CONST) != 1)
                switch (p.gap_ext) {
                case  0: return launch_pair_row<CELL, PF_ROW2 | PF_CONST2>(p, s);
                case -1: return launch_pair_row<CELL, PF_ROW2 | PF_CONST2 | PF_GE1>(p, s);
                case -2: return launch_pair_row<CELL, PF_ROW2 | PF_CONST2 | PF_GE2>(p, s);
                case -3: return launch_pair_row<CELL, PF_ROW2 | PF_CONST2 | PF_GE3>(p, s);
                }
            return launch_pair_row<CELL, PF_ROW2>(p, s);
        }
    }
    return launch_pair_row<CELL, 0>(p, s);
}

static bool pair_max3_admitted(const GotohParams& p)
{
    if (test_switch(SW_BANDED_PAIR) == 2) return false;
    const int64_t per_row = int64_t(std::max(std::max(p.match, p.mismatch), 0)) - p.gap_ext;
    return int64_t(p.pat.fixed_length) * per_row <= PM3_ROW_LIMIT;
}

static bool pair_column_admitted(const GotohParams& p)
{
    if (test_switch(SW_BANDED_PAIR) == 3 || !pair_max3_admitted(p)) return false;
    const int64_t s_max = std::max(p.match, p.mismatch), G = -int64_t(p.gap_ext) * 32, D = (int64_t(p.gap_ext) - p.gap_open) * 32;
    if (s_max - p.gap_open - p.gap_ext > PD3_BYTE_LIMIT) return false;
    return pd3_top(D, G, p.pat.fixed_length, std::max<int64_t>(s_max, 0)) <= PD3_TOP;
}

}

template <typename QA>
static int banded_gotoh_dispatch(nvb::GotohParams& p, const QA& qa, int64_t max_abs_cost, int32_t best_pair, int32_t type, uint32_t band_len,
                                 const nvbio_hip_string_set* patterns, hipStream_t s, const char* tag16, const char* tag32, const bool views = false,
                                 const nvb::BoundArgs* bound = nullptr, const bool asym = false, const bool plain_entry = false)
{
    using namespace nvb;
    g_last_pair = PairLaunch();
    const bool rt = !asym && !bound;
    const uint32_t lim_plain = test_switch(SW_FORCE_32BIT) == 1 ? 0u
                             : max_len_16bit(p.match, best_pair, max_abs_cost, std::max(p.gap_open, p.txt_gap_open), std::max(p.gap_ext, p.txt_gap_ext), type, band_len, 0);
    const uint32_t lim16 = !rt ? lim_plain : test_switch(SW_FORCE_32BIT) == 1 ? 0u
                         : max_len_16bit(p.match, best_pair, max_abs_cost, std::max(p.gap_open, p.txt_gap_open), std::max(p.gap_ext, p.txt_gap_ext), type, band_len,
                                         p.gap_ext < 0 ? -p.gap_ext : 0);
    const uint32_t lim16p = (rt && type == NVBIO_HIP_LOCAL && lim_plain > lim16) ? lim_plain : lim16;
    const bool fixed = (patterns->length == nullptr);
    hipError_t e = hipSuccess;
    {
        const uint32_t maxM = fixed ? patterns->fixed_length : p.stage_pw ;
        p.stage_pw = p.stage_tw = 0;
        if (maxM != 0 && test_switch(SW_NO_STAGING) != 1) {
            uint32_t pw = stage_words_pattern(32u / patterns->bits - 1u, maxM, patterns->bits);
            if (views) {
                const uint32_t per = 32u / patterns->bits, c16 = (maxM + 15u) & ~15u;
                pw = std::max(pw, (per - 1u + c16 + 16u + per - 1u) / per + (patterns->bits == 4 ? 3u : 2u));
            }
            pw = (pw + 3u) & ~3u;
            const uint32_t tw = (stage_words_text(15u, maxM, band_len) + 3u) & ~3u;
            if ((pw + tw) * 1024u <= 32768u) { p.stage_pw = pw; p.stage_tw = tw; }
        }
    }
    auto go = [&](const bool width16) -> hipError_t {
        if (asym)   return launch_asym(p, type, band_len, width16, s);
        if (!bound) return launch<QA>(p, qa, type, band_len, width16, s);
        if (hipError_t z = hipMemsetAsync(bound->counter, 0, 4u, s)) return z;
        return launch_bounded<QA>(p, qa, *bound, type, band_len, width16, s);
    };
    p.plain16 = 0u;
    if (plain_entry && pair_admitted(p, type, band_len, lim16)) {
        g_last_kernel = g_last_pair.kernel = tag16;
        const bool max3 = pair_max3_admitted(p);
        const bool column = max3 && pair_column_admitted(p);
        g_last_pair.cell = max3 ? "max3" : "u16";
        g_last_pair.frame = column ? "column" : "row";
        return column ? launch_pair<PD3>(p, s) : max3 ? launch_pair<PM3>(p, s) : launch_pair<P16>(p, s);
    }
    if (lim16 > 0 && (!fixed || patterns->fixed_length <= lim16)) {
        p.len_lo = 0; p.len_hi = lim16;
        g_last_kernel = tag16;
        e = go(true);
        if (e != hipSuccess) return e;
    }
    if (lim16p > lim16 && (!fixed || (patterns->fixed_length > lim16 && patterns->fixed_length <= lim16p))) {
        p.len_lo = lim16 + 1u; p.len_hi = lim16p; p.plain16 = 1u;
        if (fixed) g_last_kernel = tag16;
        e = go(true);
        p.plain16 = 0u;
        if (e != hipSuccess) return e;
    }
    if (lim16p != 0xFFFFFFFFu && (!fixed || patterns->fixed_length > lim16p)) {
        p.len_lo = lim16p > 0 ? lim16p + 1 : 0; p.len_hi = 0xFFFFFFFFu;
        if (fixed || lim16p == 0) g_last_kernel = tag32;
        e = go(false);
    }
    return e;
}

static int check_banded_args(int32_t type, uint32_t band_len, const nvbio_hip_string_set* patterns, const nvbio_hip_string_set* texts)
{
    if (!patterns || !texts) return hipErrorInvalidValue;
    if (type < 0 || type > 2) return hipErrorInvalidValue;
    if (!(patterns->bits == 2 || patterns->bits == 4 || patterns->bits == 8) || texts->bits != 2) return hipErrorNotSupported;
    if (!(band_len == 3 || band_len == 5 || band_len == 7 || band_len == 15 || band_len == 31)) return hipErrorNotSupported;
    return hipSuccess;
}
static int check_banded_ptrs(const nvbio_hip_string_set* patterns, const nvbio_hip_string_set* texts, const int32_t* out_score, const uint32_t* out_sink)
{
    if (!out_score || !out_sink) return hipErrorInvalidValue;
    if (!patterns->words || !texts->words || !patterns->begin || !texts->begin ||
        patterns->n_words == 0 || texts->n_words == 0) return hipErrorInvalidValue;
    return hipSuccess;
}
static inline int64_t iabs64(int32_t v) { return v < 0 ? -int64_t(v) : int64_t(v); }

NVB_API int nvbio_hip_banded_gotoh_score(
    const nvbio_hip_gotoh_scheme* scheme, int32_t type, uint32_t band_len,
    const nvbio_hip_string_set* patterns, const nvbio_hip_string_set* texts,
    uint32_t max_pattern_len, uint32_t max_text_len,
    uint32_t n, int32_t* out_score, uint32_t* out_sink, void* stream)
{
    (void)max_text_len;
    using namespace nvb;
    if (!scheme) return hipErrorInvalidValue;
    if (int e = check_banded_args(type, band_len, patterns, texts)) return e;
    if (n == 0) return hipSuccess;
    if (int e = check_banded_ptrs(patterns, texts, out_score, out_sink)) return e;

    GotohParams p;
    p.pat = make_string_set(patterns);
    p.txt = make_string_set(texts);
    p.match = scheme->match; p.mismatch = scheme->mismatch;
    p.gap_open = scheme->gap_open; p.gap_ext = scheme->gap_ext;
    p.txt_gap_open = scheme->gap_open; p.txt_gap_ext = scheme->gap_ext;
    p.n = n; p.out_score = out_score; p.out_sink = out_sink; p.n_dev = nullptr; p.out_index = nullptr; p.gate = nullptr; p.gate_limit = 0;
    p.stage_pw = max_pattern_len; p.stage_tw = 0;
    const int64_t A = std::max(std::max(iabs64(scheme->match), iabs64(scheme->mismatch)), std::max(iabs64(scheme->gap_open), iabs64(scheme->gap_ext)));
    return banded_gotoh_dispatch(p, NoQual(), A, std::max(scheme->match, scheme->mismatch), type, band_len, patterns, to_stream(stream),
                                 "banded_gotoh_score_kernel<A16>", "banded_gotoh_score_kernel<A32>", false, nullptr, false, true);
}

NVB_API int nvbio_hip_banded_gotoh_score_qual(
    const nvbio_hip_gotoh_qual_scheme* scheme, int32_t type, uint32_t band_len,
    const nvbio_hip_string_set* patterns, const uint8_t* quals, uint64_t n_quals,
    const nvbio_hip_string_set* texts,
    uint32_t max_pattern_len, uint32_t max_text_len,
    uint32_t n, int32_t* out_score, uint32_t* out_sink, void* stream)
{
    return nvbio_hip_banded_gotoh_score_qual_views(scheme, type, band_len, patterns, quals, n_quals, nullptr, texts, max_pattern_len, max_text_len, n, out_score, out_sink, stream);
}

NVB_API int nvbio_hip_banded_gotoh_score_qual_views(
    const nvbio_hip_gotoh_qual_scheme* scheme, int32_t type, uint32_t band_len,
    const nvbio_hip_string_set* patterns, const uint8_t* quals, uint64_t n_quals, const uint8_t* pattern_flags,
    const nvbio_hip_string_set* texts,
    uint32_t max_pattern_len, uint32_t max_text_len,
    uint32_t n, int32_t* out_score, uint32_t* out_sink, void* stream)
{
    (void)max_text_len;
    using namespace nvb;
    if (!scheme) return hipErrorInvalidValue;
    if (int e = check_banded_args(type, band_len, patterns, texts)) return e;
    if (n == 0) return hipSuccess;
    if (int e = check_banded_ptrs(patterns, texts, out_score, out_sink)) return e;
    if (!quals || n_quals < 4) return hipErrorInvalidValue;
    if (pattern_flags && patterns->bits == 8u) return hipErrorNotSupported;

    GotohParams p;
    p.pat = make_string_set(patterns);
    p.txt = make_string_set(texts);
    p.match = scheme->match; p.mismatch = 0;
    p.gap_open = scheme->pattern_gap_open; p.gap_ext = scheme->pattern_gap_ext;
    p.txt_gap_open = scheme->text_gap_open; p.txt_gap_ext = scheme->text_gap_ext;
    p.n = n; p.out_score = out_score; p.out_sink = out_sink; p.n_dev = nullptr; p.out_index = nullptr; p.gate = nullptr; p.gate_limit = 0;
    p.stage_pw = max_pattern_len; p.stage_tw = 0;
    QualArgs qa;
    qa.quals = quals; qa.n_quals = n_quals; qa.flags = pattern_flags;
    int64_t A = std::max(std::max(iabs64(scheme->match), iabs64(scheme->pattern_gap_open)), std::max(iabs64(scheme->pattern_gap_ext),
                std::max(iabs64(scheme->text_gap_open), iabs64(scheme->text_gap_ext))));
    int32_t best_pair = scheme->match;
    for (int i = 0; i < 256; ++i) { qa.lut[i] = scheme->mismatch[i]; A = std::max(A, iabs64(scheme->mismatch[i])); best_pair = std::max(best_pair, scheme->mismatch[i]); }
    return banded_gotoh_dispatch(p, qa, A, best_pair, type, band_len, patterns, to_stream(stream),
                                 pattern_flags ? "banded_gotoh_score_kernel<A16,qual,views>" : "banded_gotoh_score_kernel<A16,qual>",
                                 pattern_flags ? "banded_gotoh_score_kernel<A32,qual,views>" : "banded_gotoh_score_kernel<A32,qual>", pattern_flags != nullptr);
}

NVB_API int nvbio_hip_banded_gotoh_score_qual_bounded(
    const nvbio_hip_gotoh_qual_scheme* scheme, int32_t type, uint32_t band_len,
    const nvbio_hip_string_set* patterns, const uint8_t* quals, uint64_t n_quals, const uint8_t* pattern_flags,
    const nvbio_hip_string_set* texts,
    uint32_t max_pattern_len, uint32_t max_text_len,
    uint32_t n, const uint32_t* n_on_device, const int32_t* min_score, uint32_t* work_counter, const uint32_t* out_index,
    const uint32_t* gate, uint32_t gate_limit,
    int32_t* out_score, uint32_t* out_sink, void* stream)
{
    (void)max_text_len;
    using namespace nvb;
    if (!scheme || (min_score && !work_counter) || (min_score && gate)) return hipErrorInvalidValue;
    if (int e = check_banded_args(type, band_len, patterns, texts)) return e;
    if (n == 0) return hipSuccess;
    if (int e = check_banded_ptrs(patterns, texts, out_score, out_sink)) return e;
    if (!quals || n_quals < 4) return hipErrorInvalidValue;
    if (pattern_flags && patterns->bits == 8u) return hipErrorNotSupported;

    GotohParams p;
    p.pat = make_string_set(patterns);
    p.txt = make_string_set(texts);
    p.match = scheme->match; p.mismatch = 0;
    p.gap_open = scheme->pattern_gap_open; p.gap_ext = scheme->pattern_gap_ext;
    p.txt_gap_open = scheme->text_gap_open; p.txt_gap_ext = scheme->text_gap_ext;
    p.n = n; p.out_score = out_score; p.out_sink = out_sink; p.n_dev = nullptr; p.out_index = nullptr; p.gate = nullptr; p.gate_limit = 0;
    p.stage_pw = max_pattern_len; p.stage_tw = 0;
    QualArgs qa;
    qa.quals = quals; qa.n_quals = n_quals; qa.flags = pattern_flags;
    int64_t A = std::max(std::max(iabs64(scheme->match), iabs64(scheme->pattern_gap_open)), std::max(iabs64(scheme->pattern_gap_ext),
                std::max(iabs64(scheme->text_gap_open), iabs64(scheme->text_gap_ext))));
    int32_t best_pair = scheme->match;
    for (int i = 0; i < 256; ++i) { qa.lut[i] = scheme->mismatch[i]; A = std::max(A, iabs64(scheme->mismatch[i])); best_pair = std::max(best_pair, scheme->mismatch[i]); }
    if (!min_score)
    {
        p.n_dev = n_on_device; p.out_index = out_index; p.gate = gate; p.gate_limit = gate_limit;
        return banded_gotoh_dispatch(p, qa, A, best_pair, type, band_len, patterns, to_stream(stream),
                                     pattern_flags ? "banded_gotoh_score_kernel<A16,qual,views>" : "banded_gotoh_score_kernel<A16,qual>",
                                     pattern_flags ? "banded_gotoh_score_kernel<A32,qual,views>" : "banded_gotoh_score_kernel<A32,qual>", pattern_flags != nullptr);
    }
    BoundArgs ba;
    const bool gaps_ok = scheme->pattern_gap_open <= 0 && scheme->pattern_gap_ext <= 0;
    ba.min_score = gaps_ok ? min_score : nullptr;
    ba.n_dev = n_on_device; ba.counter = work_counter; ba.out_index = out_index;
    ba.cap = std::max(best_pair, 0);
    static const int refill = [] { const char* e = getenv("NVBIO_HIP_BOUNDED_REFILL"); return std::min(64, std::max(1, e ? atoi(e) : 16)); }();
    ba.refill = uint32_t(refill);
    return banded_gotoh_dispatch(p, qa, A, best_pair, type, band_len, patterns, to_stream(stream),
                                 "banded_gotoh_score_bounded_kernel<A16,qual>", "banded_gotoh_score_bounded_kernel<A32,qual>", pattern_flags != nullptr, &ba);
}

NVB_API int nvbio_hip_banded_sw_score(
    const nvbio_hip_sw_scheme* scheme, int32_t type, uint32_t band_len,
    const nvbio_hip_string_set* patterns, const nvbio_hip_string_set* texts,
    uint32_t max_pattern_len, uint32_t max_text_len,
    uint32_t n, int32_t* out_score, uint32_t* out_sink, void* stream)
{
    if (!scheme) return hipErrorInvalidValue;
    if (scheme->deletion == scheme->insertion)
    {
        const nvbio_hip_gotoh_scheme g = { scheme->match, scheme->mismatch, scheme->deletion, scheme->deletion };
        return nvbio_hip_banded_gotoh_score(&g, type, band_len, patterns, texts, max_pattern_len, max_text_len, n, out_score, out_sink, stream);
    }
    (void)max_text_len;
    using namespace nvb;
    if (int e = check_banded_args(type, band_len, patterns, texts)) return e;
    if (n == 0) return hipSuccess;
    if (int e = check_banded_ptrs(patterns, texts, out_score, out_sink)) return e;
    GotohParams p;
    p.pat = make_string_set(patterns);
    p.txt = make_string_set(texts);
    p.match = scheme->match; p.mismatch = scheme->mismatch;
    p.gap_open = p.gap_ext = scheme->insertion;
    p.f_gap_open = p.f_gap_ext = scheme->deletion;
    p.txt_gap_open = p.txt_gap_ext = scheme->deletion;
    p.n = n; p.out_score = out_score; p.out_sink = out_sink; p.n_dev = nullptr; p.out_index = nullptr; p.gate = nullptr; p.gate_limit = 0;
    p.stage_pw = max_pattern_len; p.stage_tw = 0;
    const int64_t A = std::max(std::max(iabs64(scheme->match), iabs64(scheme->mismatch)), std::max(iabs64(scheme->deletion), iabs64(scheme->insertion)));
    return banded_gotoh_dispatch(p, NoQual(), A, std::max(scheme->match, scheme->mismatch), type, band_len, patterns, to_stream(stream),
                                 "banded_gotoh_score_kernel<A16X>", "banded_gotoh_score_kernel<A32X>", false, nullptr, true);
}

namespace nvb {
static std::mutex g_streams_mtx;
static std::vector<hipStream_t> g_streams[64];
static void register_stream(int dev, hipStream_t s) { if (dev >= 0 && dev < 64) { std::lock_guard<std::mutex> lock(g_streams_mtx); g_streams[dev].push_back(s); } }
static void forget_stream(hipStream_t s)
{
    std::lock_guard<std::mutex> lock(g_streams_mtx);
    for (auto& v : g_streams) v.erase(std::remove(v.begin(), v.end(), s), v.end());
}

struct CachedBlock { void* ptr; uint64_t bytes; uint64_t stamp; };
struct BlockCache
{
    std::mutex mtx;
    std::vector<CachedBlock> idle;
    std::unordered_map<void*, uint64_t> live;
    uint64_t idle_bytes = 0, clock = 0;
};
static BlockCache g_cache[64];
static int env_int(const char* name, int dflt) { const char* e = getenv(name); return e ? atoi(e) : dflt; }
static uint64_t cache_keep_bytes() { static const uint64_t keep = uint64_t(std::max(0, env_int("NVBIO_HIP_POOL_KEEP_MB", 2048))) << 20; return keep; }
static hipMemPool_t rocm_pool(int dev)
{
    static std::mutex mtx;
    static hipMemPool_t pools[64] = {};
    static bool tried[64] = {};
    static const bool use = env_int("NVBIO_HIP_ROCM_POOL", 0) == 1;
    if (!use || dev < 0 || dev >= 64) return nullptr;
    std::lock_guard<std::mutex> lock(mtx);
    if (!tried[dev]) {
        tried[dev] = true;
        hipMemPoolProps props = {};
        props.allocType = hipMemAllocationTypePinned;
        props.handleTypes = hipMemHandleTypeNone;
        props.location.type = hipMemLocationTypeDevice;
        props.location.id = dev;
        hipMemPool_t pool = nullptr;
        if (hipMemPoolCreate(&pool, &props) == hipSuccess) {
            uint64_t keep = uint64_t(256) << 20;
            (void)hipMemPoolSetAttribute(pool, hipMemPoolAttrReleaseThreshold, &keep);
            pools[dev] = pool;
        } else (void)hipGetLastError();
    }
    return pools[dev];
}
static void drop_idle(BlockCache& c, std::vector<void*>& victims, uint64_t keep)
{
    while (c.idle_bytes > keep && !c.idle.empty())
    {
        size_t k = 0;
        for (size_t j = 1; j < c.idle.size(); ++j) if (c.idle[j].stamp < c.idle[k].stamp) k = j;
        victims.push_back(c.idle[k].ptr);
        c.idle_bytes -= c.idle[k].bytes;
        c.idle[k] = c.idle.back(); c.idle.pop_back();
    }
}
}
NVB_API int nvbio_hip_device_malloc(void** ptr, uint64_t bytes)
{
    if (!ptr) return hipErrorInvalidValue;
    int dev = 0;
    if (hipError_t e = hipGetDevice(&dev)) return e;
    if (dev < 0 || dev >= 64) return hipMalloc(ptr, bytes ? bytes : 1);
    if (hipMemPool_t pool = nvb::rocm_pool(dev))
    {
        if (hipError_t e = hipMallocFromPoolAsync(ptr, bytes ? bytes : 1, pool, nullptr)) return e;
        return hipStreamSynchronize(nullptr);
    }
    const uint64_t n = ((bytes ? bytes : 1) + 511ull) & ~511ull;
    nvb::BlockCache& c = nvb::g_cache[dev];
    void* p = nullptr;
    {
        std::lock_guard<std::mutex> lock(c.mtx);
        size_t best = c.idle.size();
        for (size_t k = 0; k < c.idle.size(); ++k)
            if (c.idle[k].bytes >= n && c.idle[k].bytes <= 2u * n && (best == c.idle.size() || c.idle[k].bytes < c.idle[best].bytes)) best = k;
        if (best != c.idle.size())
        {
            p = c.idle[best].ptr;
            c.live[p] = c.idle[best].bytes;
            c.idle_bytes -= c.idle[best].bytes;
            c.idle[best] = c.idle.back(); c.idle.pop_back();
        }
    }
    if (!p)
    {
        hipError_t e = hipMalloc(&p, n);
        if (e != hipSuccess)
        {
            (void)hipGetLastError();
            std::vector<void*> victims;
            { std::lock_guard<std::mutex> lock(c.mtx); nvb::drop_idle(c, victims, 0); }
            for (void* v : victims) (void)hipFree(v);
            e = hipMalloc(&p, n);
            if (e != hipSuccess) return e;
        }
        std::lock_guard<std::mutex> lock(c.mtx);
        c.live[p] = n;
    }
    *ptr = p;
    static const int poison = nvb::env_int("NVBIO_HIP_POISON_ALLOC", -1);
    if (poison >= 0) (void)hipMemsetAsync(p, poison & 255, bytes ? bytes : 1, nullptr);
    return hipStreamSynchronize(nullptr);
}
static int free_impl(void* ptr, bool ordered, hipStream_t extra = nullptr)
{
    if (!ptr) return hipSuccess;
    int dev = 0;
    static const bool sync_free = nvb::env_int("NVBIO_HIP_SYNC_FREE", 0) == 1;
    const bool have_dev = hipGetDevice(&dev) == hipSuccess && dev >= 0 && dev < 64;
    if (!have_dev) { if (hipError_t e = hipDeviceSynchronize()) return e; return hipFree(ptr); }
    if (sync_free || !ordered) { if (hipError_t e = hipDeviceSynchronize()) return e; }
    else
    {
        std::lock_guard<std::mutex> lock(nvb::g_streams_mtx);
        std::vector<hipStream_t> behind(nvb::g_streams[dev]);
        if (extra && std::find(behind.begin(), behind.end(), extra) == behind.end()) behind.push_back(extra);
        for (hipStream_t s : behind)
        {
            hipEvent_t ev = nullptr;
            hipError_t e = hipEventCreateWithFlags(&ev, hipEventDisableTiming);
            if (e == hipSuccess) e = hipEventRecord(ev, s);
            if (e == hipSuccess) e = hipStreamWaitEvent(nullptr, ev, 0);
            if (ev) (void)hipEventDestroy(ev);
            if (e != hipSuccess)
            {
                (void)hipGetLastError();
                if (hipError_t es = hipDeviceSynchronize()) return es;
                break;
            }
        }
    }
    if (nvb::rocm_pool(dev)) return hipFreeAsync(ptr, nullptr);
    nvb::BlockCache& c = nvb::g_cache[dev];
    std::vector<void*> victims;
    {
        std::lock_guard<std::mutex> lock(c.mtx);
        auto it = c.live.find(ptr);
        if (it == c.live.end()) victims.push_back(ptr);
        else
        {
            c.idle.push_back(nvb::CachedBlock{ ptr, it->second, ++c.clock });
            c.idle_bytes += it->second;
            c.live.erase(it);
            nvb::drop_idle(c, victims, nvb::cache_keep_bytes());
        }
    }
    hipError_t r = hipSuccess;
    for (void* v : victims) { const hipError_t e = hipFree(v); if (e != hipSuccess) r = e; }
    return r;
}
NVB_API int nvbio_hip_device_free(void* ptr)         { return free_impl(ptr, false); }
NVB_API int nvbio_hip_device_free_ordered(void* ptr) { return free_impl(ptr, true); }
NVB_API int nvbio_hip_device_free_after(void* ptr, void* stream) { return free_impl(ptr, true, nvb::to_stream(stream)); }
NVB_API int nvbio_hip_device_trim(void)
{
    int dev = 0;
    if (hipError_t e = hipGetDevice(&dev)) return e;
    if (dev < 0 || dev >= 64) return hipSuccess;
    std::vector<void*> victims;
    { std::lock_guard<std::mutex> lock(nvb::g_cache[dev].mtx); nvb::drop_idle(nvb::g_cache[dev], victims, 0); }
    hipError_t r = hipSuccess;
    for (void* v : victims) { const hipError_t e = hipFree(v); if (e != hipSuccess) r = e; }
    return r;
}
NVB_API int nvbio_hip_device_mem_info(uint64_t* free_bytes, uint64_t* total_bytes, uint64_t* idle_cached_bytes)
{
    size_t f = 0, t = 0;
    if (hipError_t e = hipMemGetInfo(&f, &t)) return e;
    int dev = 0;
    uint64_t idle = 0;
    if (hipGetDevice(&dev) == hipSuccess && dev >= 0 && dev < 64) { std::lock_guard<std::mutex> lock(nvb::g_cache[dev].mtx); idle = nvb::g_cache[dev].idle_bytes; }
    if (free_bytes) *free_bytes = f;
    if (total_bytes) *total_bytes = t;
    if (idle_cached_bytes) *idle_cached_bytes = idle;
    return hipSuccess;
}
namespace nvb {
uint32_t seeding_grid(uint64_t n_items) { return uint32_t((n_items + 255u) / 256u); }
}
NVB_API int nvbio_hip_stream_create(void** stream, uint32_t non_blocking)
{
    if (!stream) return hipErrorInvalidValue;
    hipStream_t s = nullptr;
    const hipError_t e = hipStreamCreateWithFlags(&s, non_blocking ? hipStreamNonBlocking : hipStreamDefault);
    *stream = s;
    int dev = 0;
    if (e == hipSuccess && hipGetDevice(&dev) == hipSuccess) nvb::register_stream(dev, s);
    return e;
}
NVB_API int nvbio_hip_stream_destroy(void* stream)
{
    if (!stream) return hipSuccess;
    nvb::forget_stream(nvb::to_stream(stream));
    return hipStreamDestroy(nvb::to_stream(stream));
}

namespace nvb {
static std::atomic<int> g_switch[SW_COUNT];
static const char* const g_switch_name[SW_COUNT] = { "NVBIO_HIP_FORCE_32BIT", "NVBIO_HIP_NO_STAGING", "NVBIO_HIP_FULL_GENERIC", "NVBIO_HIP_ED_SWEEP",
                                                     "NVBIO_HIP_FULL_SINGLE_JOB", "NVBIO_HIP_FULL_ROWS", "NVBIO_HIP_TRACEBACK_LANES", "NVBIO_HIP_SELECT_LANES",
                                                     "NVBIO_HIP_BANDED_PAIR", "NVBIO_HIP_PAIR_ROW", "NVBIO_HIP_PAIR_CONST" };
static void seed_switches()
{
    static std::once_flag once;
    std::call_once(once, [] { for (int k = 0; k < SW_COUNT; ++k) { const char* e = getenv(g_switch_name[k]); g_switch[k].store(e ? atoi(e) : 0, std::memory_order_relaxed); } });
}
int test_switch(TestSwitch which) { seed_switches(); return g_switch[which].load(std::memory_order_relaxed); }
}
NVB_API int nvbio_hip_set_test_switch(const char* name, int value)
{
    if (!name) return hipErrorInvalidValue;
    nvb::seed_switches();
    for (int k = 0; k < nvb::SW_COUNT; ++k)
        if (strcmp(name, nvb::g_switch_name[k]) == 0) { nvb::g_switch[k].store(value, std::memory_order_relaxed); return hipSuccess; }
    return hipErrorInvalidValue;
}
NVB_API const char* nvbio_hip_test_switch_name(int index) { return (index >= 0 && index < nvb::SW_COUNT) ? nvb::g_switch_name[index] : nullptr; }
NVB_API int nvbio_hip_get_test_switch(const char* name)
{
    if (!name) return -1;
    for (int k = 0; k < nvb::SW_COUNT; ++k) if (strcmp(name, nvb::g_switch_name[k]) == 0) return nvb::test_switch(nvb::TestSwitch(k));
    return -1;
}

NVB_API int nvbio_hip_memcpy(void* dst, const void* src, uint64_t bytes, int kind, void* stream)
{
    const hipMemcpyKind k = kind == 1 ? hipMemcpyHostToDevice : kind == 2 ? hipMemcpyDeviceToHost : hipMemcpyDeviceToDevice;
    if (bytes == 0) return hipSuccess;
    hipError_t e = hipMemcpyAsync(dst, src, bytes, k, nvb::to_stream(stream));
    if (e != hipSuccess) return e;
    return kind == 2 ? hipStreamSynchronize(nvb::to_stream(stream)) : hipSuccess;
}
NVB_API int nvbio_hip_memset(void* dst, int value, uint64_t bytes, void* stream) { return bytes ? hipMemsetAsync(dst, value, bytes, nvb::to_stream(stream)) : hipSuccess; }
NVB_API int nvbio_hip_stream_synchronize(void* stream) { return hipStreamSynchronize(nvb::to_stream(stream)); }
NVB_API int nvbio_hip_stream_query(void* stream)
{
    const hipError_t e = hipStreamQuery(nvb::to_stream(stream));
    if (e == hipErrorNotReady) (void)hipGetLastError();
    return e;
}
NVB_API int nvbio_hip_host_malloc(void** ptr, uint64_t bytes)
{
    if (!ptr) return hipErrorInvalidValue;
    *ptr = nullptr;
    return hipHostMalloc(ptr, bytes ? bytes : 1u, hipHostMallocDefault);
}
NVB_API int nvbio_hip_host_free(void* ptr) { return ptr ? hipHostFree(ptr) : hipSuccess; }

NVB_API int         nvbio_hip_abi_version(void) { return NVBIO_HIP_ABI_VERSION; }
NVB_API const char* nvbio_hip_arch(void)        { return "gfx950"; }
NVB_API const char* nvbio_hip_last_kernel(void) { return nvb::g_last_kernel; }
static const char* pair_fact(const char* fact) { return (nvb::g_last_pair.kernel && nvb::g_last_pair.kernel == nvb::g_last_kernel) ? fact : ""; }
NVB_API const char* nvbio_hip_last_kernel_detail(void) { return pair_fact("pair"); }
NVB_API const char* nvbio_hip_last_kernel_fetch(void)  { return pair_fact(nvb::g_last_pair.fetch); }
NVB_API const char* nvbio_hip_last_kernel_frame(void)  { return pair_fact(nvb::g_last_pair.frame); }
NVB_API const char* nvbio_hip_last_kernel_row(void)    { return pair_fact(nvb::g_last_pair.row); }
NVB_API const char* nvbio_hip_last_kernel_const(void)  { return pair_fact(nvb::g_last_pair.consts); }
NVB_API const char* nvbio_hip_last_kernel_cell(void)   { return pair_fact(nvb::g_last_pair.cell); }
```

### nvbio_amd/csrc/banded_gotoh_pair.h

```cpp
#pragma once
#include "banded_gotoh_impl.h"

namespace nvb {

template <int BAND>
struct PairState {
    uint32_t S[BAND];
    uint32_t F[BAND - 1];
    uint32_t tc[16];
    uint32_t z;
    uint32_t best[2], besti[2];
};

enum PairForm : int {
    PF_SINK_VCC = 0, PF_SINK_KEY = 1,
    PF_STREAM   = 4,
    PF_PAT2     = 2,
    PF_PBE      = 8, PF_TBE = 256,
    PF_KO_SINK  = 16, PF_KO_TABLE = 32, PF_KO_FETCH = 64, PF_KO_BOUND = 128,
    PF_FOLD2    = 1024,
    PF_CONST2   = 16384 | 131072,
    PF_GE1      = 32768, PF_GE2 = 65536, PF_GE3 = PF_GE1 | PF_GE2
};
constexpr int pair_ge(int form)     { return (form / PF_GE1) & 3; }
constexpr int pair_ge_bits(int ge)  { return ge * PF_GE1; }
constexpr int PF_ROW2 = PF_FOLD2;
#define NVB_PAIR_STREAM_FORMS_(Y, A) \
    Y(A, PF_STREAM) Y(A, PF_STREAM | PF_PBE) Y(A, PF_STREAM | PF_TBE) Y(A, PF_STREAM | PF_PBE | PF_TBE) \
    Y(A, PF_STREAM | PF_PAT2) Y(A, PF_STREAM | PF_PAT2 | PF_PBE) Y(A, PF_STREAM | PF_PAT2 | PF_TBE) Y(A, PF_STREAM | PF_PAT2 | PF_PBE | PF_TBE)
#define NVB_PAIR_APPLY_(X, F) X(F)
#define NVB_PAIR_STREAM_FORMS(X) NVB_PAIR_STREAM_FORMS_(NVB_PAIR_APPLY_, X)
#define NVB_PAIR_CELLS_(X, F) X(P16, (F)) X(PM3, (F)) X(PD3, (F)) X(PD3, (F) | PF_ROW2)
#define NVB_PAIR_GES_(X, F)   X(PD3, (F) | PF_ROW2 | PF_CONST2) X(PD3, (F) | PF_ROW2 | PF_CONST2 | PF_GE1) X(PD3, (F) | PF_ROW2 | PF_CONST2 | PF_GE2) X(PD3, (F) | PF_ROW2 | PF_CONST2 | PF_GE3)
#define NVB_PAIR_INSTANCES_B15(X)     NVB_PAIR_CELLS_(X, PF_SINK_VCC) NVB_PAIR_STREAM_FORMS_(NVB_PAIR_CELLS_, X)
#define NVB_PAIR_INSTANCES_B15_LIT(X) NVB_PAIR_GES_(X, PF_SINK_VCC) NVB_PAIR_STREAM_FORMS_(NVB_PAIR_GES_, X)
#define NVB_PAIR_INSTANCES(X)         NVB_PAIR_INSTANCES_B15(X) NVB_PAIR_INSTANCES_B15_LIT(X)

struct PairOps {
    static constexpr bool COLUMN = false;
    static __device__ __forceinline__ uint32_t rep(int32_t c)               { return (uint32_t(c) & 0xFFFFu) * 0x10001u; }
    static __device__ __forceinline__ uint32_t mx(uint32_t a, uint32_t b)   { uint32_t r; asm("v_pk_max_u16 %0, %1, %2" : "=v"(r) : "v"(a), "v"(b)); return r; }
    static constexpr uint32_t SEL_BASE = 0x0C040C00u;
    static __device__ __forceinline__ uint32_t subst(uint32_t tlo, uint32_t thi, uint32_t sel) { return __builtin_amdgcn_perm(thi, tlo, sel); }

    template <int FORM, int BAND>
    static __device__ __forceinline__ void sink(PairState<BAND>& st, uint32_t rowkey, const uint32_t i) { fold<FORM>(st, rowkey - st.z, i); }
    template <int FORM, int BAND>
    static __device__ __forceinline__ void fold(PairState<BAND>& st, const uint32_t rowkey, const uint32_t i)
    {
        if (FORM & PF_KO_SINK) { st.best[0] = mx(st.best[0], rowkey); return; }
        if (FORM & PF_SINK_KEY)
        {
            const uint32_t frame = (31u << 15) | (i << 5);
            uint32_t a, b, wa, wb;
            asm("v_and_b32 %[a], 0xffff, %[rk]\n\t"
                "v_lshrrev_b32 %[b], 16, %[rk]\n\t"
                "v_lshl_or_b32 %[wa], %[a], 15, %[fr]\n\t"
                "v_lshl_or_b32 %[wb], %[b], 15, %[fr]\n\t"
                "v_and_or_b32 %[wa], %[a], 31, %[wa]\n\t"
                "v_and_or_b32 %[wb], %[b], 31, %[wb]\n\t"
                "v_max_u32 %[ba], %[ba], %[wa]\n\t"
                "v_max_u32 %[bb], %[bb], %[wb]"
                : [a] "=&v"(a), [b] "=&v"(b), [wa] "=&v"(wa), [wb] "=&v"(wb), [ba] "+&v"(st.best[0]), [bb] "+&v"(st.best[1])
                : [rk] "v"(rowkey), [fr] "s"(frame));
            return;
        }
        const uint32_t rk[2] = { rowkey & 0xFFFFu, rowkey >> 16 };
        #pragma unroll
        for (int h = 0; h < 2; ++h)
        {
            const bool upd = (rk[h] | 31u) >= st.best[h];
            st.best[h]  = upd ? rk[h] : st.best[h];
            st.besti[h] = upd ? i : st.besti[h];
        }
    }
};

struct P16 : PairOps {
    static constexpr int32_t FLOOR = 0;

    template <int J, bool EDGE>
    static __device__ __forceinline__ void cell(uint32_t& Fj, const uint32_t Fnext, const uint32_t Snext, uint32_t& Sj, uint32_t& E, uint32_t& rowkey,
                                                const uint32_t g, const uint32_t D, const uint32_t G, const uint32_t tlo, const uint32_t thi, const uint32_t Z)
    {
        uint32_t d, h;
        if (EDGE)
            asm("v_perm_b32 %[d], %[thi], %[tlo], %[g]\n\t"
                "v_mov_b32 %[f], %[sn]\n\t"
                "v_add_u32 %[d], %[s], %[d]\n\t"
                "v_pk_max_u16 %[h], %[sn], %[z]\n\t"
                "v_pk_max_u16 %[h], %[h], %[d]\n\t"
                "v_pk_max_u16 %[h], %[h], %[e]\n\t"
                "v_sub_u32 %[s], %[h], %[dd]\n\t"
                "v_add_u32 %[d], %[sj], %[h]\n\t"
                "v_pk_max_u16 %[e], %[e], %[s]\n\t"
                "v_sub_u32 %[e], %[e], %[gg]\n\t"
                "v_pk_max_u16 %[rk], %[rk], %[d]"
                : [f] "=&v"(Fj), [d] "=&v"(d), [h] "=&v"(h), [s] "+v"(Sj), [e] "+v"(E), [rk] "+v"(rowkey)
                : [g] "v"(g), [tlo] "v"(tlo), [thi] "v"(thi), [sn] "v"(Snext), [dd] "v"(D), [gg] "v"(G), [z] "v"(Z), [sj] "n"(J * 0x10001));
        else
            asm("v_perm_b32 %[d], %[thi], %[tlo], %[g]\n\t"
                "v_pk_max_u16 %[f], %[fn], %[sn]\n\t"
                "v_add_u32 %[d], %[s], %[d]\n\t"
                "v_pk_max_u16 %[h], %[f], %[z]\n\t"
                "v_pk_max_u16 %[h], %[h], %[d]\n\t"
                "v_pk_max_u16 %[h], %[h], %[e]\n\t"
                "v_sub_u32 %[s], %[h], %[dd]\n\t"
                "v_add_u32 %[d], %[sj], %[h]\n\t"
                "v_pk_max_u16 %[e], %[e], %[s]\n\t"
                "v_sub_u32 %[e], %[e], %[gg]\n\t"
                "v_pk_max_u16 %[rk], %[rk], %[d]"
                : [f] "=&v"(Fj), [d] "=&v"(d), [h] "=&v"(h), [s] "+v"(Sj), [e] "+v"(E), [rk] "+v"(rowkey)
                : [g] "v"(g), [tlo] "v"(tlo), [thi] "v"(thi), [fn] "v"(Fnext), [sn] "v"(Snext), [dd] "v"(D), [gg] "v"(G), [z] "v"(Z), [sj] "n"(J * 0x10001));
    }

    template <int BAND, int R, int J, int END>
    struct Cells {
        static __device__ __forceinline__ void run(PairState<BAND>& st, uint32_t& E, uint32_t& rowkey, const uint32_t D, const uint32_t G, const uint32_t tlo, const uint32_t thi)
        {
            cell<J, J + 1 == BAND - 1>(st.F[J], st.F[J + 1 < BAND - 1 ? J + 1 : 0], st.S[J + 1], st.S[J], E, rowkey, st.tc[(R + J) & 15], D, G, tlo, thi, st.z);
            Cells<BAND, R, J + 1, END>::run(st, E, rowkey, D, G, tlo, thi);
        }
    };
    template <int BAND, int R, int END>
    struct Cells<BAND, R, END, END> {
        static __device__ __forceinline__ void run(PairState<BAND>&, uint32_t&, uint32_t&, uint32_t, uint32_t, uint32_t, uint32_t) {}
    };

    template <int BAND, int R, int FORM>
    static __device__ __forceinline__ void row(PairState<BAND>& st, const uint32_t i, const uint32_t D, const uint32_t G, const uint32_t g_new, const uint32_t tlo, const uint32_t thi)
    {
        st.z += G;
        st.F[0] = (1 == BAND - 1) ? st.S[1] : mx(st.F[1 < BAND - 1 ? 1 : 0], st.S[1]);
        uint32_t hi = mx(mx(st.F[0], st.S[0] + subst(tlo, thi, st.tc[R & 15])), st.z);
        uint32_t rowkey = hi;
        st.S[0] = hi - D;
        uint32_t E = st.S[0] - G;
        Cells<BAND, R, 1, BAND - 1>::run(st, E, rowkey, D, G, tlo, thi);
        st.tc[(R + BAND - 1) & 15] = g_new;
        hi = mx(mx(E, st.S[BAND - 1] + subst(tlo, thi, g_new)), st.z);
        rowkey = mx(rowkey, hi + uint32_t(BAND - 1) * 0x10001u);
        st.S[BAND - 1] = hi - D;
        sink<FORM>(st, rowkey, i);
    }
};

constexpr int32_t PM3_ROW_LIMIT = (0x7BFF - 255 - 0x0400 - 448) / 32;
struct PM3 : PairOps {
    static constexpr int32_t FLOOR = 0x0400;
    static __device__ __forceinline__ uint32_t mx3(uint32_t a, uint32_t b, uint32_t c) { uint32_t r; asm("v_pk_maximum3_f16 %0, %1, %2, %3" : "=v"(r) : "v"(a), "v"(b), "v"(c)); return r; }

    template <int J>
    static __device__ __forceinline__ void cell2(uint32_t& F0, uint32_t& F1, const uint32_t F2, uint32_t& S0, uint32_t& S1, const uint32_t S2, uint32_t& E, uint32_t& rowkey,
                                                 const uint32_t g0, const uint32_t g1, const uint32_t D, const uint32_t G, const uint32_t tlo, const uint32_t thi, const uint32_t Z)
    {
        uint32_t d0, d1, h;
        asm("v_perm_b32 %[d0], %[thi], %[tlo], %[g0]\n\t"
            "v_perm_b32 %[d1], %[thi], %[tlo], %[g1]\n\t"
            "v_pk_maximum3_f16 %[f0], %[f1], %[s1], %[z]\n\t"
            "v_pk_maximum3_f16 %[f1], %[f2], %[s2], %[z]\n\t"
            "v_add_u32 %[d0], %[s0], %[d0]\n\t"
            "v_add_u32 %[d1], %[s1], %[d1]\n\t"
            "v_pk_maximum3_f16 %[h], %[f0], %[d0], %[e]\n\t"
            "v_sub_u32 %[s0], %[h], %[dd]\n\t"
            "v_add_u32 %[d0], %[j0], %[h]\n\t"
            "v_pk_max_u16 %[e], %[e], %[s0]\n\t"
            "v_sub_u32 %[e], %[e], %[gg]\n\t"
            "v_pk_maximum3_f16 %[h], %[f1], %[d1], %[e]\n\t"
            "v_sub_u32 %[s1], %[h], %[dd]\n\t"
            "v_add_u32 %[d1], %[j1], %[h]\n\t"
            "v_pk_max_u16 %[e], %[e], %[s1]\n\t"
            "v_sub_u32 %[e], %[e], %[gg]\n\t"
            "v_pk_maximum3_f16 %[rk], %[rk], %[d0], %[d1]"
            : [f0] "=&v"(F0), [f1] "+&v"(F1), [d0] "=&v"(d0), [d1] "=&v"(d1), [h] "=&v"(h), [s0] "+&v"(S0), [s1] "+&v"(S1), [e] "+&v"(E), [rk] "+&v"(rowkey)
            : [g0] "v"(g0), [g1] "v"(g1), [tlo] "v"(tlo), [thi] "v"(thi), [f2] "v"(F2), [s2] "v"(S2), [dd] "v"(D), [gg] "v"(G), [z] "v"(Z),
              [j0] "n"(J * 0x10001), [j1] "n"((J + 1) * 0x10001));
    }

    template <int J>
    static __device__ __forceinline__ void tail2(uint32_t& F0, uint32_t& S0, uint32_t& S1, uint32_t& E, uint32_t& rowkey,
                                                 const uint32_t g0, const uint32_t g1, const uint32_t D, const uint32_t G, const uint32_t tlo, const uint32_t thi, const uint32_t Z)
    {
        uint32_t d0, d1, h;
        asm("v_perm_b32 %[d0], %[thi], %[tlo], %[g0]\n\t"
            "v_perm_b32 %[d1], %[thi], %[tlo], %[g1]\n\t"
            "v_pk_max_u16 %[f0], %[s1], %[z]\n\t"
            "v_add_u32 %[d0], %[s0], %[d0]\n\t"
            "v_add_u32 %[d1], %[s1], %[d1]\n\t"
            "v_pk_maximum3_f16 %[h], %[f0], %[d0], %[e]\n\t"
            "v_sub_u32 %[s0], %[h], %[dd]\n\t"
            "v_add_u32 %[d0], %[j0], %[h]\n\t"
            "v_pk_max_u16 %[e], %[e], %[s0]\n\t"
            "v_sub_u32 %[e], %[e], %[gg]\n\t"
            "v_pk_maximum3_f16 %[h], %[e], %[d1], %[z]\n\t"
            "v_sub_u32 %[s1], %[h], %[dd]\n\t"
            "v_add_u32 %[d1], %[j1], %[h]\n\t"
            "v_pk_maximum3_f16 %[rk], %[rk], %[d0], %[d1]"
            : [f0] "=&v"(F0), [d0] "=&v"(d0), [d1] "=&v"(d1), [h] "=&v"(h), [s0] "+&v"(S0), [s1] "+&v"(S1), [e] "+&v"(E), [rk] "+&v"(rowkey)
            : [g0] "v"(g0), [g1] "v"(g1), [tlo] "v"(tlo), [thi] "v"(thi), [dd] "v"(D), [gg] "v"(G), [z] "v"(Z),
              [j0] "n"(J * 0x10001), [j1] "n"((J + 1) * 0x10001));
    }

    template <int BAND, int R, int J, int END>
    struct Cells {
        static __device__ __forceinline__ void run(PairState<BAND>& st, uint32_t& E, uint32_t& rowkey, const uint32_t D, const uint32_t G, const uint32_t tlo, const uint32_t thi)
        {
            cell2<J>(st.F[J], st.F[J + 1], st.F[J + 2], st.S[J], st.S[J + 1], st.S[J + 2], E, rowkey, st.tc[(R + J) & 15], st.tc[(R + J + 1) & 15], D, G, tlo, thi, st.z);
            Cells<BAND, R, J + 2, END>::run(st, E, rowkey, D, G, tlo, thi);
        }
    };
    template <int BAND, int R, int END>
    struct Cells<BAND, R, END, END> {
        static __device__ __forceinline__ void run(PairState<BAND>&, uint32_t&, uint32_t&, uint32_t, uint32_t, uint32_t, uint32_t) {}
    };

    template <int BAND, int R, int FORM>
    static __device__ __forceinline__ void row(PairState<BAND>& st, const uint32_t i, const uint32_t D, const uint32_t G, const uint32_t g_new, const uint32_t tlo, const uint32_t thi)
    {
        static_assert(BAND % 2 == 1, "columns 1 ... BAND-3 go two at a time");
        st.z += G;
        st.F[0] = (1 == BAND - 1) ? mx(st.S[1], st.z) : mx3(st.F[1 < BAND - 1 ? 1 : 0], st.S[1], st.z);
        const uint32_t hi = mx(st.F[0], st.S[0] + subst(tlo, thi, st.tc[R & 15]));
        uint32_t rowkey = hi;
        st.S[0] = hi - D;
        uint32_t E = st.S[0] - G;
        Cells<BAND, R, 1, BAND - 2>::run(st, E, rowkey, D, G, tlo, thi);
        st.tc[(R + BAND - 1) & 15] = g_new;
        tail2<BAND - 2>(st.F[BAND - 2], st.S[BAND - 2], st.S[BAND - 1], E, rowkey, st.tc[(R + BAND - 2) & 15], g_new, D, G, tlo, thi, st.z);
        sink<FORM>(st, rowkey, i);
    }
};

constexpr int32_t PD3_TOP = 0x7BFF, PD3_BYTE_LIMIT = 7;
constexpr int64_t pd3_top(int64_t D, int64_t G, int64_t M, int64_t s_plus, int64_t band = 15)
{
    return 0x0400 + D + G + G * (2 * M + band - 1) + 32 * M * s_plus + 255;
}
template <int BAND>
struct ColumnFrame {
    uint32_t z[16];
    uint32_t k[BAND];
    uint32_t D, step;
    uint32_t pair;
};
struct PD3 : PairOps {
    static constexpr bool COLUMN = true;
    static constexpr int32_t FLOOR = 0x0400;

    template <int FORM> static constexpr int32_t klit(int j)     { return int32_t(uint32_t(j + (14 - j) * 32 * pair_ge(FORM)) * 0x10001u); }
    template <int FORM> static constexpr int32_t pairlit()       { return int32_t(uint32_t(2 * 32 * pair_ge(FORM)) * 0x10001u); }

#define NVB_PD3_COL0 \
            "v_perm_b32 %[d], %[thi], %[tlo], %[g0]\n\t" \
            "v_pk_maximum3_f16 %[f0], %[f1], %[s1], %[z0]\n\t" \
            "v_add_u32 %[d], %[s0], %[d]\n\t" \
            "v_pk_max_u16 %[h], %[f0], %[d]\n\t" \
            "v_subrev_u32 %[s0], %[dd], %[h]\n\t" \
            "v_add_u32 %[rk], %[k0], %[h]"
#define NVB_PD3_COL0_OUT [f0] "=&v"(F0), [d] "=&v"(d), [h] "=&v"(h), [s0] "+&v"(S0), [rk] "=&v"(rowkey)
#define NVB_PD3_COL0_IN  [g0] "v"(g0), [tlo] "v"(tlo), [thi] "v"(thi), [f1] "v"(F1), [s1] "v"(S1), [z0] "s"(Z0)
    template <int FORM>
    static __device__ __forceinline__ void col0(uint32_t& F0, const uint32_t F1, uint32_t& S0, const uint32_t S1, uint32_t& rowkey,
                                                const uint32_t g0, const uint32_t D, const uint32_t tlo, const uint32_t thi, const uint32_t Z0, const uint32_t K0)
    {
        uint32_t d, h;
        if constexpr ((FORM & PF_CONST2) != 0) asm(NVB_PD3_COL0 : NVB_PD3_COL0_OUT : NVB_PD3_COL0_IN, [dd] "v"(D), [k0] "n"(klit<FORM>(0)));
        else                                   asm(NVB_PD3_COL0 : NVB_PD3_COL0_OUT : NVB_PD3_COL0_IN, [dd] "s"(D), [k0] "s"(K0));
    }

#define NVB_PD3_CELL2(P) \
            "v_perm_b32 %[d0], %[thi], %[tlo], %[g0]\n\t" \
            "v_perm_b32 %[d1], %[thi], %[tlo], %[g1]\n\t" \
            "v_pk_maximum3_f16 %[f0], %[f1], %[s1], %[z0]\n\t" \
            "v_pk_maximum3_f16 %[f1], %[f2], %[s2], %[z1]\n\t" \
            "v_add_u32 %[d0], %[s0], %[d0]\n\t" \
            "v_add_u32 %[d1], %[s1], %[d1]\n\t" P \
            "v_pk_maximum3_f16 %[h], %[f0], %[d0], %[ei]\n\t" \
            "v_subrev_u32 %[s0], %[dd], %[h]\n\t" \
            "v_add_u32 %[d0], %[k0], %[h]\n\t" P \
            "v_pk_max_u16 %[e], %[ei], %[s0]\n\t" \
            "v_pk_maximum3_f16 %[h], %[f1], %[d1], %[e]\n\t" \
            "v_subrev_u32 %[s1], %[dd], %[h]\n\t" \
            "v_add_u32 %[d1], %[k1], %[h]\n\t" P \
            "v_pk_max_u16 %[e], %[e], %[s1]\n\t" \
            "v_pk_maximum3_f16 %[rk], %[rk], %[d0], %[d1]"
#define NVB_PD3_CELL2_OUT [f0] "=&v"(F0), [f1] "+&v"(F1), [d0] "=&v"(d0), [d1] "=&v"(d1), [h] "=&v"(h), [s0] "+&v"(S0), [s1] "+&v"(S1), [e] "=&v"(E), [rk] "+&v"(rowkey)
#define NVB_PD3_CELL2_IN  [g0] "v"(g0), [g1] "v"(g1), [tlo] "v"(tlo), [thi] "v"(thi), [f2] "v"(F2), [s2] "v"(S2), [ei] "v"(Ein), [z0] "s"(Z0), [z1] "s"(Z1)
    template <int FORM, int J>
    static __device__ __forceinline__ void cell2(uint32_t& F0, uint32_t& F1, const uint32_t F2, uint32_t& S0, uint32_t& S1, const uint32_t S2, const uint32_t Ein, uint32_t& E,
                                                 uint32_t& rowkey, const uint32_t g0, const uint32_t g1, const uint32_t D, const uint32_t tlo, const uint32_t thi,
                                                 const uint32_t Z0, const uint32_t Z1, const uint32_t K0, const uint32_t K1)
    {
        uint32_t d0, d1, h;
        if constexpr ((FORM & PF_CONST2) != 0) asm(NVB_PD3_CELL2("s_nop 0\n\t") : NVB_PD3_CELL2_OUT : NVB_PD3_CELL2_IN, [dd] "v"(D), [k0] "n"(klit<FORM>(J)), [k1] "n"(klit<FORM>(J + 1)));
        else                                   asm(NVB_PD3_CELL2("") : NVB_PD3_CELL2_OUT : NVB_PD3_CELL2_IN, [dd] "s"(D), [k0] "s"(K0), [k1] "s"(K1));
    }

#define NVB_PD3_TAIL2 \
            "v_perm_b32 %[d0], %[thi], %[tlo], %[g0]\n\t" \
            "v_perm_b32 %[d1], %[thi], %[tlo], %[g1]\n\t" \
            "v_pk_max_u16 %[f0], %[s1], %[z0]\n\t" \
            "v_add_u32 %[d0], %[s0], %[d0]\n\t" \
            "v_add_u32 %[d1], %[s1], %[d1]\n\t" \
            "v_pk_maximum3_f16 %[h], %[f0], %[d0], %[ei]\n\t" \
            "v_subrev_u32 %[s0], %[dd], %[h]\n\t" \
            "v_add_u32 %[d0], %[k0], %[h]\n\t" \
            "v_pk_max_u16 %[e], %[ei], %[s0]\n\t" \
            "v_pk_maximum3_f16 %[h], %[e], %[d1], %[z1]\n\t" \
            "v_subrev_u32 %[s1], %[dd], %[h]\n\t" \
            "v_add_u32 %[d1], %[k1], %[h]\n\t" \
            "v_pk_maximum3_f16 %[rk], %[rk], %[d0], %[d1]"
#define NVB_PD3_TAIL2_OUT [f0] "=&v"(F0), [d0] "=&v"(d0), [d1] "=&v"(d1), [h] "=&v"(h), [e] "=&v"(e), [s0] "+&v"(S0), [s1] "+&v"(S1), [rk] "+&v"(rowkey)
#define NVB_PD3_TAIL2_IN  [g0] "v"(g0), [g1] "v"(g1), [tlo] "v"(tlo), [thi] "v"(thi), [ei] "v"(Ein), [z0] "s"(Z0), [z1] "s"(Z1)
    template <int FORM, int J>
    static __device__ __forceinline__ void tail2(uint32_t& F0, uint32_t& S0, uint32_t& S1, const uint32_t Ein, uint32_t& rowkey,
                                                 const uint32_t g0, const uint32_t g1, const uint32_t D, const uint32_t tlo, const uint32_t thi,
                                                 const uint32_t Z0, const uint32_t Z1, const uint32_t K0, const uint32_t K1)
    {
        uint32_t d0, d1, h, e;
        if constexpr ((FORM & PF_CONST2) != 0) asm(NVB_PD3_TAIL2 : NVB_PD3_TAIL2_OUT : NVB_PD3_TAIL2_IN, [dd] "v"(D), [k0] "n"(klit<FORM>(J)), [k1] "n"(klit<FORM>(J + 1)));
        else                                   asm(NVB_PD3_TAIL2 : NVB_PD3_TAIL2_OUT : NVB_PD3_TAIL2_IN, [dd] "s"(D), [k0] "s"(K0), [k1] "s"(K1));
    }

    template <int BAND, int R, int FORM, int J, int END>
    struct Cells {
        static __device__ __forceinline__ void run(PairState<BAND>& st, const ColumnFrame<BAND>& fr, const uint32_t Ein, uint32_t& E, uint32_t& rowkey, const uint32_t tlo, const uint32_t thi)
        {
            uint32_t En;
            cell2<FORM, J>(st.F[J], st.F[J + 1], st.F[J + 2], st.S[J], st.S[J + 1], st.S[J + 2], Ein, En, rowkey, st.tc[(R + J) & 15], st.tc[(R + J + 1) & 15], fr.D, tlo, thi,
                           fr.z[(2 * R + J) & 15], fr.z[(2 * R + J + 1) & 15], fr.k[J], fr.k[J + 1]);
            Cells<BAND, R, FORM, J + 2, END>::run(st, fr, En, E, rowkey, tlo, thi);
        }
    };
    template <int BAND, int R, int FORM, int END>
    struct Cells<BAND, R, FORM, END, END> {
        static __device__ __forceinline__ void run(PairState<BAND>&, const ColumnFrame<BAND>&, const uint32_t Ein, uint32_t& E, uint32_t&, uint32_t, uint32_t) { E = Ein; }
    };

    template <int BAND>
    static __device__ __forceinline__ void open(ColumnFrame<BAND>& fr, const int32_t d32, const int32_t g32)
    {
        #pragma unroll
        for (int s = 0; s < 16; ++s) fr.z[s] = rep(d32 + g32 + FLOOR + g32 * (2 + (s <= BAND - 3 ? s : s - 16)));
        #pragma unroll
        for (int j = 0; j < BAND; ++j) fr.k[j] = rep(j + (BAND - 1 - j) * g32);
        fr.D = rep(d32);
        fr.step = rep(16 * g32);
        fr.pair = rep(2 * g32);
    }

    template <int BAND, int R, int FORM>
    static __device__ __forceinline__ void row(PairState<BAND>& st, ColumnFrame<BAND>& fr, const uint32_t i, const uint32_t g_new, const uint32_t tlo, const uint32_t thi, uint32_t& rk2)
    {
        static_assert(BAND == 15, "a row's zeros, 2 i ... 2 i + BAND - 1, and the two the next row adds fill the ring of 16; columns go two at a time");
        fr.z[(2 * R + BAND - 2) & 15] += fr.step;
        fr.z[(2 * R + BAND - 1) & 15] += fr.step;
        uint32_t rowkey, E;
        col0<FORM>(st.F[0], st.F[1], st.S[0], st.S[1], rowkey, st.tc[R & 15], fr.D, tlo, thi, fr.z[(2 * R) & 15], fr.k[0]);
        Cells<BAND, R, FORM, 1, BAND - 2>::run(st, fr, st.S[0], E, rowkey, tlo, thi);
        st.tc[(R + BAND - 1) & 15] = g_new;
        tail2<FORM, BAND - 2>(st.F[BAND - 2], st.S[BAND - 2], st.S[BAND - 1], E, rowkey, st.tc[(R + BAND - 2) & 15], g_new, fr.D, tlo, thi,
                              fr.z[(2 * R + BAND - 2) & 15], fr.z[(2 * R + BAND - 1) & 15], fr.k[BAND - 2], fr.k[BAND - 1]);
        if constexpr ((FORM & PF_FOLD2) != 0)
        {
            if constexpr ((R & 1) == 0) rk2 = rowkey;
            else fold<FORM>(st, mx(rk2 + ((FORM & PF_CONST2) ? uint32_t(pairlit<FORM>()) : fr.pair), rowkey + rep(16)) - fr.z[(2 * R + BAND - 1) & 15], i - 1u);
        }
        else fold<FORM>(st, rowkey - fr.z[(2 * R + BAND - 1) & 15], i);
    }

    template <int BAND, int FORM>
    static __device__ __forceinline__ void fold_last(PairState<BAND>& st, const uint32_t rk2, const uint32_t M, const int32_t d32, const int32_t g32)
    {
        fold<FORM>(st, rk2 - rep(d32 + g32 + FLOOR + g32 * int32_t(2u * M + BAND - 1)), M - 1u);
    }
};

template <typename CELL, int BAND, int FORM, int R, int END>
struct PairRows {
    static __device__ __forceinline__ void run(PairState<BAND>& st, ColumnFrame<BAND>& fr, const uint32_t i0, const uint32_t M, const uint32_t D, const uint32_t G,
                                               const uint64_t PA, const uint64_t PB, const uint32_t (&XT)[2], const uint32_t* tab, const uint32_t (&KT)[2], uint32_t& rk2)
    {
        if ((FORM & PF_KO_BOUND) || i0 + R < M)
        {
            const uint32_t g = ((XT[R >> 3] >> (2 * (R & 7))) & 0x00030003u) | CELL::SEL_BASE;
            if constexpr (CELL::COLUMN)
            {
                if (FORM & PF_KO_TABLE) CELL::template row<BAND, R, FORM>(st, fr, i0 + R, g, KT[0], KT[1], rk2);
                else                    CELL::template row<BAND, R, FORM>(st, fr, i0 + R, g, tab[uint32_t(PA >> (4 * R)) & 15u], tab[uint32_t(PB >> (4 * R)) & 15u], rk2);
            }
            else
            {
                if (FORM & PF_KO_TABLE) CELL::template row<BAND, R, FORM>(st, i0 + R, D, G, g, KT[0], KT[1]);
                else                    CELL::template row<BAND, R, FORM>(st, i0 + R, D, G, g, tab[uint32_t(PA >> (4 * R)) & 15u], tab[uint32_t(PB >> (4 * R)) & 15u]);
            }
        }
        PairRows<CELL, BAND, FORM, R + 1, END>::run(st, fr, i0, M, D, G, PA, PB, XT, tab, KT, rk2);
    }
};
template <typename CELL, int BAND, int FORM, int END> struct PairRows<CELL, BAND, FORM, END, END> {
    static __device__ __forceinline__ void run(PairState<BAND>&, ColumnFrame<BAND>&, uint32_t, uint32_t, uint32_t, uint32_t, uint64_t, uint64_t, const uint32_t (&)[2], const uint32_t*, const uint32_t (&)[2], uint32_t&) {}
};

constexpr int PAIR_LANES = 128;
template <int BAND, typename CELL, int FORM>
__global__ void __launch_bounds__(PAIR_LANES)
banded_gotoh_pair_kernel(const GotohParams p)
{
    static_assert(BAND >= 3 && BAND <= 16, "the ring of 16");
    constexpr bool STREAM = (FORM & PF_STREAM) != 0, KEY = (FORM & PF_SINK_KEY) != 0, FOLD2 = (FORM & PF_FOLD2) != 0;
    static_assert(!(FORM & (PF_FOLD2 | PF_CONST2)) || CELL::COLUMN, "the pair fold and the literals are the column frame's");
    static_assert(!FOLD2 || !(FORM & (PF_SINK_KEY | PF_KO_SINK | PF_KO_BOUND)), "the pair fold is the compare-and-select fold's, over the job's own rows");
    static_assert(!(FORM & PF_GE3) || (FORM & PF_CONST2), "|G_e| is the literal form's parameter");
    constexpr bool P4 = !(FORM & PF_PAT2), PBE = (FORM & PF_PBE) != 0, TBE = (FORM & PF_TBE) != 0;
    __shared__ uint32_t s_tab[16];
    if (threadIdx.x < 16u)
    {
        const uint32_t tg = CELL::COLUMN ? uint32_t(-p.gap_ext * 32) : 0u;
        const uint32_t sm = uint32_t((p.match - p.gap_open) * 32) + tg, sx = uint32_t((p.mismatch - p.gap_open) * 32) + tg;
        uint32_t t = sx * 0x01010101u;
        if (threadIdx.x < 4u) t = (t & ~(0xFFu << (8u * threadIdx.x))) | (sm << (8u * threadIdx.x));
        s_tab[threadIdx.x] = t;
    }
    __syncthreads();
    const uint32_t lane = blockIdx.x * uint32_t(PAIR_LANES) + threadIdx.x;
    if (lane >= p.n / 2u + (p.n & 1u)) return;
    const uint32_t id[2] = { 2u * lane, 2u * lane + 1u < p.n ? 2u * lane + 1u : 2u * lane };
    const uint32_t M = (FORM & PF_KO_BOUND) ? 96u : p.pat.fixed_length;
    const Stream ps[2] = { p.pat.s, p.pat.s }, ts[2] = { p.txt.s, p.txt.s };
    const uint64_t pb[2] = { p.pat.begin[id[0]], p.pat.begin[id[1]] }, tb[2] = { p.txt.begin[id[0]], p.txt.begin[id[1]] };

    const int32_t d32 = (p.gap_ext - p.gap_open) * 32, g32 = -p.gap_ext * 32;
    uint32_t D = CELL::rep(d32), G = CELL::rep(g32);
    if (!CELL::COLUMN) { asm("" : "+v"(D)); asm("" : "+v"(G)); }
    uint32_t KT[2] = { 0u, 0u };
    if (FORM & PF_KO_TABLE) { KT[0] = s_tab[threadIdx.x & 3u]; KT[1] = s_tab[(threadIdx.x >> 2) & 3u]; asm("" : "+v"(KT[0])); asm("" : "+v"(KT[1])); }

    PairState<BAND> st;
    #pragma unroll
    for (int j = 0; j < BAND; ++j) st.S[j] = CELL::rep(g32 + CELL::FLOOR + (CELL::COLUMN ? g32 * j : 0));
    #pragma unroll
    for (int j = 0; j < BAND - 1; ++j) st.F[j] = CELL::rep(CELL::FLOOR);
    st.z = CELL::rep(d32 + g32 + CELL::FLOOR);
    ColumnFrame<BAND> fr;
    if constexpr (CELL::COLUMN) CELL::open(fr, d32, g32);
    if constexpr ((FORM & PF_CONST2) != 0) asm("" : "+v"(fr.D));
    st.best[0] = st.best[1] = 0u; st.besti[0] = st.besti[1] = 0u;
    uint32_t rk2 = 0u;
    {
        const uint32_t TA = fetch16_2bit(ts[0], tb[0]), TB = fetch16_2bit(ts[1], tb[1]);
        #pragma unroll
        for (int j = 0; j < BAND - 1; ++j)
            st.tc[j] = CELL::SEL_BASE | ((TA >> (2 * j)) & 3u) | (((TB >> (2 * j)) & 3u) << 16);
    }

    const uint32_t plast = stream_last_off(p.pat.s), tlast = stream_last_off(p.txt.s);
    GroupStream gp[2], gt[2];
    uint64_t PA, PB;
    uint32_t TA, TB;
    if (STREAM)
    {
        if (P4) { PA = stream_open_4bit<PBE>(ps[0], plast, pb[0], gp[0]); PB = stream_open_4bit<PBE>(ps[1], plast, pb[1], gp[1]); }
        else    { PA = expand_2to4(stream_open_2bit<PBE>(ps[0], plast, pb[0], gp[0])); PB = expand_2to4(stream_open_2bit<PBE>(ps[1], plast, pb[1], gp[1])); }
        TA = stream_open_2bit<TBE>(ts[0], tlast, tb[0] + BAND - 1, gt[0]); TB = stream_open_2bit<TBE>(ts[1], tlast, tb[1] + BAND - 1, gt[1]);
    }
    else
    {
        PA = fetch_pattern16(ps[0], pb[0]); PB = fetch_pattern16(ps[1], pb[1]);
        TA = fetch16_2bit(ts[0], tb[0] + BAND - 1); TB = fetch16_2bit(ts[1], tb[1] + BAND - 1);
    }
    for (uint32_t i0 = 0; i0 < M; i0 += 16u)
    {
        uint64_t PAn = 0, PBn = 0;
        uint32_t TAn = 0, TBn = 0;
        uint2 rp[2] = { make_uint2(0u, 0u), make_uint2(0u, 0u) };
        uint32_t rt[2] = { 0u, 0u };
        if (FORM & PF_KO_FETCH) {}
        else if (STREAM)
        {
            if (P4) { rp[0] = stream_load_4bit(ps[0], plast, gp[0]); rp[1] = stream_load_4bit(ps[1], plast, gp[1]); }
            else    { rp[0].x = stream_load_2bit(ps[0], plast, gp[0]); rp[1].x = stream_load_2bit(ps[1], plast, gp[1]); }
            rt[0] = stream_load_2bit(ts[0], tlast, gt[0]); rt[1] = stream_load_2bit(ts[1], tlast, gt[1]);
        }
        else
        {
            PAn = fetch_pattern16(ps[0], pb[0] + i0 + 16u); PBn = fetch_pattern16(ps[1], pb[1] + i0 + 16u);
            TAn = fetch16_2bit(ts[0], tb[0] + i0 + 16u + BAND - 1); TBn = fetch16_2bit(ts[1], tb[1] + i0 + 16u + BAND - 1);
        }
        const uint32_t XT[2] = { (TA & 0xFFFFu) | (TB << 16), (TA >> 16) | (TB & 0xFFFF0000u) };
        PairRows<CELL, BAND, FORM, 0, 16>::run(st, fr, i0, M, D, G, PA, PB, XT, s_tab, KT, rk2);
        if (FORM & PF_KO_FETCH)
        {
            PA = (PA << 4) | (PA >> 60); PB = (PB << 8) | (PB >> 56);
            TA = funnel(TA, TA, 2u); TB = funnel(TB, TB, 6u);
        }
        else if (STREAM)
        {
            if (P4) { PA = stream_group_4bit<PBE>(gp[0], rp[0]); PB = stream_group_4bit<PBE>(gp[1], rp[1]); }
            else    { PA = expand_2to4(stream_group_2bit<PBE>(gp[0], rp[0].x)); PB = expand_2to4(stream_group_2bit<PBE>(gp[1], rp[1].x)); }
            TA = stream_group_2bit<TBE>(gt[0], rt[0]); TB = stream_group_2bit<TBE>(gt[1], rt[1]);
        }
        else { PA = PAn; PB = PBn; TA = TAn; TB = TBn; }
    }

    if constexpr (FOLD2) { if (M & 1u) CELL::template fold_last<BAND, FORM>(st, rk2, M, d32, g32); }
    #pragma unroll
    for (int h = 0; h < 2; ++h)
    {
        if (h == 1 && id[1] == id[0]) break;
        const uint32_t j = st.best[h] & (FOLD2 ? 15u : 31u), i = KEY ? (st.best[h] >> 5) & 1023u : st.besti[h] + (FOLD2 ? (st.best[h] >> 4) & 1u : 0u);
        p.out_score[id[h]] = int32_t(st.best[h] >> (KEY ? 20 : 5));
        reinterpret_cast<uint2*>(p.out_sink)[id[h]] = make_uint2(i + j + 1u, i + 1u);
    }
}

template <int BAND, typename CELL, int FORM>
hipError_t launch_band_pair(const GotohParams& p, hipStream_t stream)
{
    const uint32_t n_lanes = p.n / 2u + (p.n & 1u);
    hipLaunchKernelGGL((banded_gotoh_pair_kernel<BAND, CELL, FORM>), dim3((n_lanes + PAIR_LANES - 1u) / PAIR_LANES), dim3(PAIR_LANES), 0, stream, p);
    return hipGetLastError();
}

#ifdef NVB_PAIR_EXTERN
#define NVB_DECL(CELL, F) extern template hipError_t launch_band_pair<15, CELL, (F)>(const GotohParams&, hipStream_t);
NVB_PAIR_INSTANCES(NVB_DECL)
#undef NVB_DECL
#endif

}
```

### nvbio_amd/csrc/common.h

```cpp
#pragma once
#include <hip/hip_runtime.h>
#include <stdint.h>
#include "../../include/nvbio_hip.h"

#define NVB_API extern "C" __attribute__((visibility("default")))

namespace nvb {

extern thread_local const char* g_last_kernel;
struct PairLaunch {
    const char* kernel = nullptr;
    const char* cell   = "";
    const char* fetch  = "";
    const char* frame  = "";
    const char* row    = "";
    const char* consts = "";
};
extern thread_local PairLaunch g_last_pair;

enum TestSwitch { SW_FORCE_32BIT = 0, SW_NO_STAGING, SW_FULL_GENERIC, SW_ED_SWEEP, SW_FULL_SINGLE_JOB, SW_FULL_ROWS, SW_TRACEBACK_LANES, SW_SELECT_LANES, SW_BANDED_PAIR, SW_PAIR_ROW, SW_PAIR_CONST, SW_COUNT };
int test_switch(TestSwitch which);


__device__ __forceinline__ uint32_t rev2(uint32_t x)
{
    x = __brev(x);
    return ((x & 0xAAAAAAAAu) >> 1) | ((x & 0x55555555u) << 1);
}
__device__ __forceinline__ uint32_t rev4(uint32_t x)
{
    x = __builtin_bswap32(x);
    return ((x & 0xF0F0F0F0u) >> 4) | ((x & 0x0F0F0F0Fu) << 4);
}
__device__ __forceinline__ uint32_t funnel(uint32_t lo, uint32_t hi, uint32_t sh)
{
    return __builtin_amdgcn_alignbit(hi, lo, sh);
}

typedef const uint32_t __attribute__((address_space(3)))* lds_words_t;

struct Stream {
    const uint32_t* words;
    uint64_t        n_words;
    uint32_t        bits;
    uint32_t        big_endian;
    lds_words_t     lds;
    uint64_t        kb;
};

__device__ __forceinline__ uint32_t ld_word_global(const Stream& s, uint64_t k)
{
    return s.words[k < s.n_words ? k : s.n_words - 1];
}
__device__ __forceinline__ uint32_t ld_word(const Stream& s, uint64_t k)
{
    return s.lds ? s.lds[(k - s.kb) * 256u] : ld_word_global(s, k);
}

__device__ __forceinline__ uint32_t fetch16_2bit(const Stream& s, uint64_t sym)
{
    const uint64_t k  = sym >> 4;
    const uint32_t sh = (uint32_t(sym) & 15u) << 1;
    uint32_t w0 = ld_word(s, k), w1 = ld_word(s, k + 1);
    if (s.big_endian) { w0 = rev2(w0); w1 = rev2(w1); }
    return funnel(w0, w1, sh);
}
__device__ __forceinline__ uint64_t fetch16_4bit(const Stream& s, uint64_t sym)
{
    const uint64_t k  = sym >> 3;
    const uint32_t sh = (uint32_t(sym) & 7u) << 2;
    uint32_t w0 = ld_word(s, k), w1 = ld_word(s, k + 1), w2 = ld_word(s, k + 2);
    if (s.big_endian) { w0 = rev4(w0); w1 = rev4(w1); w2 = rev4(w2); }
    const uint32_t lo = funnel(w0, w1, sh), hi = funnel(w1, w2, sh);
    return (uint64_t(hi) << 32) | lo;
}
struct GroupStream {
    uint32_t off;
    uint32_t carry;
    uint32_t sh;
};
__device__ __forceinline__ uint32_t stream_last_off(const Stream& s) { return uint32_t(s.n_words - 1u) * 4u; }
__device__ __forceinline__ uint32_t stream_raw(const Stream& s, uint32_t off) { return *reinterpret_cast<const uint32_t*>(reinterpret_cast<const char*>(s.words) + off); }
template <int BITS, bool BE>
__device__ __forceinline__ uint32_t canonical(uint32_t w) { return !BE ? w : BITS == 2 ? rev2(w) : rev4(w); }
__device__ __forceinline__ uint32_t stream_min(uint32_t a, uint32_t b) { return a < b ? a : b; }
template <bool BE>
__device__ __forceinline__ uint32_t stream_open_2bit(const Stream& s, const uint32_t last, uint64_t sym, GroupStream& g)
{
    const uint64_t k = sym >> 4;
    const uint32_t o0 = k < s.n_words ? uint32_t(k) * 4u : last;
    g.off = stream_min(o0 + 4u, last); g.sh = (uint32_t(sym) & 15u) << 1;
    const uint32_t w0 = canonical<2, BE>(stream_raw(s, o0));
    g.carry = canonical<2, BE>(stream_raw(s, g.off));
    return funnel(w0, g.carry, g.sh);
}
template <bool BE>
__device__ __forceinline__ uint64_t stream_open_4bit(const Stream& s, const uint32_t last, uint64_t sym, GroupStream& g)
{
    const uint64_t k = sym >> 3;
    const uint32_t o0 = k < s.n_words ? uint32_t(k) * 4u : last, o1 = stream_min(o0 + 4u, last);
    g.off = stream_min(o0 + 8u, last); g.sh = (uint32_t(sym) & 7u) << 2;
    const uint32_t w0 = canonical<4, BE>(stream_raw(s, o0)), w1 = canonical<4, BE>(stream_raw(s, o1));
    g.carry = canonical<4, BE>(stream_raw(s, g.off));
    return (uint64_t(funnel(w1, g.carry, g.sh)) << 32) | funnel(w0, w1, g.sh);
}
__device__ __forceinline__ uint32_t stream_load_2bit(const Stream& s, const uint32_t last, GroupStream& g)
{
    g.off = stream_min(g.off + 4u, last);
    return stream_raw(s, g.off);
}
__device__ __forceinline__ uint2 stream_load_4bit(const Stream& s, const uint32_t last, GroupStream& g)
{
    const uint32_t o1 = stream_min(g.off + 4u, last);
    g.off = stream_min(g.off + 8u, last);
    return make_uint2(stream_raw(s, o1), stream_raw(s, g.off));
}
template <bool BE>
__device__ __forceinline__ uint32_t stream_group_2bit(GroupStream& g, const uint32_t raw)
{
    const uint32_t w0 = g.carry;
    g.carry = canonical<2, BE>(raw);
    return funnel(w0, g.carry, g.sh);
}
template <bool BE>
__device__ __forceinline__ uint64_t stream_group_4bit(GroupStream& g, const uint2 raw)
{
    const uint32_t w0 = g.carry, w1 = canonical<4, BE>(raw.x);
    g.carry = canonical<4, BE>(raw.y);
    return (uint64_t(funnel(w1, g.carry, g.sh)) << 32) | funnel(w0, w1, g.sh);
}

__device__ __forceinline__ uint64_t fetch16_8bit(const Stream& s, uint64_t sym)
{
    const uint64_t k  = sym >> 2;
    const uint32_t sh = (uint32_t(sym) & 3u) << 3;
    uint32_t w[5];
    #pragma unroll
    for (int i = 0; i < 5; ++i) { w[i] = ld_word(s, k + i); if (s.big_endian) w[i] = __builtin_bswap32(w[i]); }
    uint64_t out = 0;
    #pragma unroll
    for (int i = 0; i < 4; ++i)
    {
        const uint32_t b = funnel(w[i], w[i + 1], sh);
        const uint32_t t = b & 0xFCFCFCFCu;
        const uint32_t big = ((((t & 0x7F7F7F7Fu) + 0x7F7F7F7Fu) | t) & 0x80808080u) >> 7;
        const uint32_t n = ~b;
        const uint32_t ff = ((((n & 0x7F7F7F7Fu) + 0x7F7F7F7Fu) | n) & 0x80808080u) >> 7;
        uint32_t v = ((b & 0x03030303u) & ~(big * 3u)) | (big << 2) | ((big & ~ff) * 15u);
        v = (v | (v >> 4)) & 0x00FF00FFu;
        v = (v | (v >> 8)) & 0x0000FFFFu;
        out |= uint64_t(v) << (16 * i);
    }
    return out;
}
__device__ __forceinline__ uint64_t expand_2to4(uint32_t v)
{
    uint64_t x = v;
    x = (x | (x << 16)) & 0x0000FFFF0000FFFFull;
    x = (x | (x <<  8)) & 0x00FF00FF00FF00FFull;
    x = (x | (x <<  4)) & 0x0F0F0F0F0F0F0F0Full;
    x = (x | (x <<  2)) & 0x3333333333333333ull;
    return x;
}
__device__ __forceinline__ uint64_t fetch_pattern16(const Stream& s, uint64_t sym)
{
    return (s.bits == 4) ? fetch16_4bit(s, sym) : (s.bits == 8) ? fetch16_8bit(s, sym) : expand_2to4(fetch16_2bit(s, sym));
}
__device__ __forceinline__ uint32_t get_symbol(const Stream& s, uint64_t sym)
{
    if (s.bits == 2) {
        const uint32_t w = ld_word(s, sym >> 4), k = uint32_t(sym) & 15u;
        return (w >> (s.big_endian ? 30u - 2u * k : 2u * k)) & 3u;
    } else if (s.bits == 4) {
        const uint32_t w = ld_word(s, sym >> 3), k = uint32_t(sym) & 7u;
        return (w >> (s.big_endian ? 28u - 4u * k : 4u * k)) & 15u;
    } else {
        const uint32_t w = ld_word(s, sym >> 2), k = uint32_t(sym) & 3u;
        return (w >> (s.big_endian ? 24u - 8u * k : 8u * k)) & 255u;
    }
}

__host__ __device__ inline uint32_t empty_pattern_exit_block(uint32_t N, uint32_t BLK, int32_t match, int32_t min_score)
{
    const uint32_t nb = BLK * ((N + BLK - 1u) / BLK), end_block = nb > BLK ? nb : BLK;
    for (uint32_t block = 0; block + BLK < end_block; block += BLK)
        if (-(1 << 30) + int32_t(N - block - BLK) * match < min_score) return block;
    return 0xFFFFFFFFu;
}

struct StringSet {
    Stream          s;
    const uint64_t* begin;
    const uint32_t* length;
    uint32_t        fixed_length;
};

inline StringSet make_string_set(const nvbio_hip_string_set* h)
{
    StringSet d;
    d.s.words = h->words; d.s.n_words = h->n_words; d.s.bits = h->bits; d.s.big_endian = h->big_endian;
    d.s.lds = nullptr; d.s.kb = 0;
    d.begin = h->begin; d.length = h->length; d.fixed_length = h->fixed_length;
    return d;
}

inline hipStream_t to_stream(void* s) { return reinterpret_cast<hipStream_t>(s); }

uint32_t seeding_grid(uint64_t n_items);

}
```

Before: 6.627 billion reads/s.

## Replace per-cell v_perm substitution lookup with a 256-entry LDS score table

Adds a PF_SUBLDS form of the pair-row banded Gotoh kernel, now the default path. It precomputes a 256-entry shared-memory table of packed match/mismatch scores indexed by both reads' pattern and text codes, so each cell reads one LDS word instead of running v_perm_b32 on packed table registers. Pattern and text symbols are repacked into byte/nibble index words, and the LDS loads are split into head and tail batches so latency can overlap the cell chain. It also sets waves_per_eu=5 for this form to raise occupancy, at the cost of register pressure and 15 LDS loads per row.

```diff
diff --git a/include/nvbio_hip.h b/include/nvbio_hip.h
--- a/include/nvbio_hip.h
+++ b/include/nvbio_hip.h
@@ -573,6 +573,7 @@
 const char* nvbio_hip_last_kernel_frame(void);
 const char* nvbio_hip_last_kernel_row(void);
 const char* nvbio_hip_last_kernel_const(void);
+const char* nvbio_hip_last_kernel_sub(void);
 const char* nvbio_hip_last_kernel_fetch(void);
 
 #ifdef __cplusplus
diff --git a/nvbio_amd/_lib.py b/nvbio_amd/_lib.py
--- a/nvbio_amd/_lib.py
+++ b/nvbio_amd/_lib.py
@@ -36,7 +36,7 @@
     "nvbio_hip_stream_synchronize", "nvbio_hip_stream_query", "nvbio_hip_host_malloc", "nvbio_hip_host_free", "nvbio_hip_stream_create", "nvbio_hip_stream_destroy",
     "nvbio_hip_comm_available", "nvbio_hip_device_count", "nvbio_hip_set_device", "nvbio_hip_get_device", "nvbio_hip_comm_unique_id", "nvbio_hip_comm_init_rank",
     "nvbio_hip_comm_init_all", "nvbio_hip_comm_destroy", "nvbio_hip_comm_rank", "nvbio_hip_gather_records", "nvbio_hip_comm_abort", "nvbio_hip_comm_set_transport",
-    "nvbio_hip_abi_version", "nvbio_hip_arch", "nvbio_hip_last_kernel", "nvbio_hip_last_kernel_detail", "nvbio_hip_last_kernel_cell", "nvbio_hip_last_kernel_frame", "nvbio_hip_last_kernel_row", "nvbio_hip_last_kernel_const", "nvbio_hip_last_kernel_fetch", "nvbio_hip_set_test_switch", "nvbio_hip_get_test_switch", "nvbio_hip_test_switch_name",
+    "nvbio_hip_abi_version", "nvbio_hip_arch", "nvbio_hip_last_kernel", "nvbio_hip_last_kernel_detail", "nvbio_hip_last_kernel_cell", "nvbio_hip_last_kernel_frame", "nvbio_hip_last_kernel_row", "nvbio_hip_last_kernel_const", "nvbio_hip_last_kernel_sub", "nvbio_hip_last_kernel_fetch", "nvbio_hip_set_test_switch", "nvbio_hip_get_test_switch", "nvbio_hip_test_switch_name",
 ]
 
 
@@ -260,6 +260,7 @@
         L.nvbio_hip_last_kernel_fetch.restype = C.c_char_p
         L.nvbio_hip_last_kernel_row.restype = C.c_char_p
         L.nvbio_hip_last_kernel_const.restype = C.c_char_p
+        L.nvbio_hip_last_kernel_sub.restype = C.c_char_p
         _lib = L
     return _lib
 
diff --git a/nvbio_amd/csrc/banded_gotoh.hip b/nvbio_amd/csrc/banded_gotoh.hip
--- a/nvbio_amd/csrc/banded_gotoh.hip
+++ b/nvbio_amd/csrc/banded_gotoh.hip
@@ -100,6 +100,7 @@
 {
     g_last_pair.row = (ROW & PF_ROW2) ? "fold2" : "plain";
     g_last_pair.consts = (ROW & PF_CONST2) ? "literal" : "scalar";
+    g_last_pair.sub = (ROW & PF_SUBLDS) ? "lds" : "perm";
     g_last_pair.fetch = "generic";
     if (!pair_stream_admitted(p)) return launch_band_pair<15, CELL, PF_SINK_VCC | ROW>(p, s);
     g_last_pair.fetch = "stream";
@@ -117,6 +118,13 @@
     {
         if (test_switch(SW_PAIR_ROW) != 1)
         {
+            if (test_switch(SW_PAIR_CONST) != 1 && test_switch(SW_PAIR_SUB) != 1)
+                switch (p.gap_ext) {
+                case  0: return launch_pair_row<CELL, PF_ROW2 | PF_CONST2 | PF_SUBLDS>(p, s);
+                case -1: return launch_pair_row<CELL, PF_ROW2 | PF_CONST2 | PF_SUBLDS | PF_GE1>(p, s);
+                case -2: return launch_pair_row<CELL, PF_ROW2 | PF_CONST2 | PF_SUBLDS | PF_GE2>(p, s);
+                case -3: return launch_pair_row<CELL, PF_ROW2 | PF_CONST2 | PF_SUBLDS | PF_GE3>(p, s);
+                }
             if (test_switch(SW_PAIR_CONST) != 1)
                 switch (p.gap_ext) {
                 case  0: return launch_pair_row<CELL, PF_ROW2 | PF_CONST2>(p, s);
@@ -583,7 +591,7 @@
 static std::atomic<int> g_switch[SW_COUNT];
 static const char* const g_switch_name[SW_COUNT] = { "NVBIO_HIP_FORCE_32BIT", "NVBIO_HIP_NO_STAGING", "NVBIO_HIP_FULL_GENERIC", "NVBIO_HIP_ED_SWEEP",
                                                      "NVBIO_HIP_FULL_SINGLE_JOB", "NVBIO_HIP_FULL_ROWS", "NVBIO_HIP_TRACEBACK_LANES", "NVBIO_HIP_SELECT_LANES",
-                                                     "NVBIO_HIP_BANDED_PAIR", "NVBIO_HIP_PAIR_ROW", "NVBIO_HIP_PAIR_CONST" };
+                                                     "NVBIO_HIP_BANDED_PAIR", "NVBIO_HIP_PAIR_ROW", "NVBIO_HIP_PAIR_CONST", "NVBIO_HIP_PAIR_SUB" };
 static void seed_switches()
 {
     static std::once_flag once;
@@ -640,4 +648,5 @@
 NVB_API const char* nvbio_hip_last_kernel_frame(void)  { return pair_fact(nvb::g_last_pair.frame); }
 NVB_API const char* nvbio_hip_last_kernel_row(void)    { return pair_fact(nvb::g_last_pair.row); }
 NVB_API const char* nvbio_hip_last_kernel_const(void)  { return pair_fact(nvb::g_last_pair.consts); }
+NVB_API const char* nvbio_hip_last_kernel_sub(void)    { return pair_fact(nvb::g_last_pair.sub); }
 NVB_API const char* nvbio_hip_last_kernel_cell(void)   { return pair_fact(nvb::g_last_pair.cell); }
diff --git a/nvbio_amd/csrc/banded_gotoh_pair.h b/nvbio_amd/csrc/banded_gotoh_pair.h
--- a/nvbio_amd/csrc/banded_gotoh_pair.h
+++ b/nvbio_amd/csrc/banded_gotoh_pair.h
@@ -20,7 +20,9 @@
     PF_KO_SINK  = 16, PF_KO_TABLE = 32, PF_KO_FETCH = 64, PF_KO_BOUND = 128,
     PF_FOLD2    = 1024,
     PF_CONST2   = 16384 | 131072,
-    PF_GE1      = 32768, PF_GE2 = 65536, PF_GE3 = PF_GE1 | PF_GE2
+    PF_GE1      = 32768, PF_GE2 = 65536, PF_GE3 = PF_GE1 | PF_GE2,
+    PF_SUBLDS   = 262144,
+    PF_KO_PERM  = 524288
 };
 constexpr int pair_ge(int form)     { return (form / PF_GE1) & 3; }
 constexpr int pair_ge_bits(int ge)  { return ge * PF_GE1; }
@@ -34,7 +36,26 @@
 #define NVB_PAIR_GES_(X, F)   X(PD3, (F) | PF_ROW2 | PF_CONST2) X(PD3, (F) | PF_ROW2 | PF_CONST2 | PF_GE1) X(PD3, (F) | PF_ROW2 | PF_CONST2 | PF_GE2) X(PD3, (F) | PF_ROW2 | PF_CONST2 | PF_GE3)
 #define NVB_PAIR_INSTANCES_B15(X)     NVB_PAIR_CELLS_(X, PF_SINK_VCC) NVB_PAIR_STREAM_FORMS_(NVB_PAIR_CELLS_, X)
 #define NVB_PAIR_INSTANCES_B15_LIT(X) NVB_PAIR_GES_(X, PF_SINK_VCC) NVB_PAIR_STREAM_FORMS_(NVB_PAIR_GES_, X)
-#define NVB_PAIR_INSTANCES(X)         NVB_PAIR_INSTANCES_B15(X) NVB_PAIR_INSTANCES_B15_LIT(X)
+#define NVB_PAIR_SUBS_(X, F)  NVB_PAIR_GES_(X, (F) | PF_SUBLDS)
+#define NVB_PAIR_INSTANCES_B15_SUB(X) NVB_PAIR_SUBS_(X, PF_SINK_VCC) NVB_PAIR_STREAM_FORMS_(NVB_PAIR_SUBS_, X)
+#define NVB_PAIR_INSTANCES(X)         NVB_PAIR_INSTANCES_B15(X) NVB_PAIR_INSTANCES_B15_LIT(X) NVB_PAIR_INSTANCES_B15_SUB(X)
+
+__host__ __device__ constexpr uint32_t sub_index(uint32_t ca, uint32_t cb) { return (ca & 3u) | (cb << 2) | ((ca >> 2) << 6); }
+__host__ __device__ constexpr uint32_t sub_code_a(uint32_t index)          { return (index & 3u) | ((index >> 6) << 2); }
+__host__ __device__ constexpr uint32_t sub_code_b(uint32_t index)          { return (index >> 2) & 15u; }
+__device__ __forceinline__ uint32_t sub_bfi(uint32_t mask, uint32_t a, uint32_t b) { return (a & mask) | (b & ~mask); }
+__device__ __forceinline__ void sub_row_words(const uint64_t PA, const uint64_t PB, uint64_t& RE, uint64_t& RO)
+{
+    uint32_t re[2], ro[2];
+    #pragma unroll
+    for (int h = 0; h < 2; ++h)
+    {
+        const uint32_t a = uint32_t(PA >> (32 * h)), b = uint32_t(PB >> (32 * h));
+        re[h] = sub_bfi(0x03030303u, a,      sub_bfi(0x3C3C3C3Cu, b << 2, a << 4));
+        ro[h] = sub_bfi(0x03030303u, a >> 4, sub_bfi(0x3C3C3C3Cu, b >> 2, a));
+    }
+    RE = re[0] | uint64_t(re[1]) << 32; RO = ro[0] | uint64_t(ro[1]) << 32;
+}
 
 struct PairOps {
     static constexpr bool COLUMN = false;
@@ -250,8 +271,11 @@
     template <int FORM> static constexpr int32_t klit(int j)     { return int32_t(uint32_t(j + (14 - j) * 32 * pair_ge(FORM)) * 0x10001u); }
     template <int FORM> static constexpr int32_t pairlit()       { return int32_t(uint32_t(2 * 32 * pair_ge(FORM)) * 0x10001u); }
 
-#define NVB_PD3_COL0 \
-            "v_perm_b32 %[d], %[thi], %[tlo], %[g0]\n\t" \
+#define NVB_PD3_PERM1 "v_perm_b32 %[d], %[thi], %[tlo], %[g0]\n\t"
+#define NVB_PD3_PERM2 "v_perm_b32 %[d0], %[thi], %[tlo], %[g0]\n\t" "v_perm_b32 %[d1], %[thi], %[tlo], %[g1]\n\t"
+#define NVB_PD3_XOR1  "v_xor_b32 %[d], %[tlo], %[g0]\n\t"
+#define NVB_PD3_XOR2  "v_xor_b32 %[d0], %[tlo], %[g0]\n\t" "v_xor_b32 %[d1], %[tlo], %[g1]\n\t"
+#define NVB_PD3_COL0(L) L \
             "v_pk_maximum3_f16 %[f0], %[f1], %[s1], %[z0]\n\t" \
             "v_add_u32 %[d], %[s0], %[d]\n\t" \
             "v_pk_max_u16 %[h], %[f0], %[d]\n\t" \
@@ -263,14 +287,15 @@
     static __device__ __forceinline__ void col0(uint32_t& F0, const uint32_t F1, uint32_t& S0, const uint32_t S1, uint32_t& rowkey,
                                                 const uint32_t g0, const uint32_t D, const uint32_t tlo, const uint32_t thi, const uint32_t Z0, const uint32_t K0)
     {
-        uint32_t d, h;
-        if constexpr ((FORM & PF_CONST2) != 0) asm(NVB_PD3_COL0 : NVB_PD3_COL0_OUT : NVB_PD3_COL0_IN, [dd] "v"(D), [k0] "n"(klit<FORM>(0)));
-        else                                   asm(NVB_PD3_COL0 : NVB_PD3_COL0_OUT : NVB_PD3_COL0_IN, [dd] "s"(D), [k0] "s"(K0));
-    }
-
-#define NVB_PD3_CELL2(P) \
-            "v_perm_b32 %[d0], %[thi], %[tlo], %[g0]\n\t" \
-            "v_perm_b32 %[d1], %[thi], %[tlo], %[g1]\n\t" \
+        uint32_t d = g0, h;
+        if constexpr ((FORM & PF_SUBLDS) != 0)      asm(NVB_PD3_COL0("") : [f0] "=&v"(F0), [d] "+&v"(d), [h] "=&v"(h), [s0] "+&v"(S0), [rk] "=&v"(rowkey)
+                                                                         : [f1] "v"(F1), [s1] "v"(S1), [z0] "s"(Z0), [dd] "v"(D), [k0] "n"(klit<FORM>(0)));
+        else if constexpr ((FORM & PF_KO_PERM) != 0) asm(NVB_PD3_COL0(NVB_PD3_XOR1) : NVB_PD3_COL0_OUT : NVB_PD3_COL0_IN, [dd] "v"(D), [k0] "n"(klit<FORM>(0)));
+        else if constexpr ((FORM & PF_CONST2) != 0) asm(NVB_PD3_COL0(NVB_PD3_PERM1) : NVB_PD3_COL0_OUT : NVB_PD3_COL0_IN, [dd] "v"(D), [k0] "n"(klit<FORM>(0)));
+        else                                        asm(NVB_PD3_COL0(NVB_PD3_PERM1) : NVB_PD3_COL0_OUT : NVB_PD3_COL0_IN, [dd] "s"(D), [k0] "s"(K0));
+    }
+
+#define NVB_PD3_CELL2(L, P) L \
             "v_pk_maximum3_f16 %[f0], %[f1], %[s1], %[z0]\n\t" \
             "v_pk_maximum3_f16 %[f1], %[f2], %[s2], %[z1]\n\t" \
             "v_add_u32 %[d0], %[s0], %[d0]\n\t" \
@@ -291,14 +316,17 @@
                                                  uint32_t& rowkey, const uint32_t g0, const uint32_t g1, const uint32_t D, const uint32_t tlo, const uint32_t thi,
                                                  const uint32_t Z0, const uint32_t Z1, const uint32_t K0, const uint32_t K1)
     {
-        uint32_t d0, d1, h;
-        if constexpr ((FORM & PF_CONST2) != 0) asm(NVB_PD3_CELL2("s_nop 0\n\t") : NVB_PD3_CELL2_OUT : NVB_PD3_CELL2_IN, [dd] "v"(D), [k0] "n"(klit<FORM>(J)), [k1] "n"(klit<FORM>(J + 1)));
-        else                                   asm(NVB_PD3_CELL2("") : NVB_PD3_CELL2_OUT : NVB_PD3_CELL2_IN, [dd] "s"(D), [k0] "s"(K0), [k1] "s"(K1));
-    }
-
-#define NVB_PD3_TAIL2 \
-            "v_perm_b32 %[d0], %[thi], %[tlo], %[g0]\n\t" \
-            "v_perm_b32 %[d1], %[thi], %[tlo], %[g1]\n\t" \
+        uint32_t d0 = g0, d1 = g1, h;
+        if constexpr ((FORM & PF_SUBLDS) != 0)
+            asm(NVB_PD3_CELL2("", "s_nop 0\n\t")
+                : [f0] "=&v"(F0), [f1] "+&v"(F1), [d0] "+&v"(d0), [d1] "+&v"(d1), [h] "=&v"(h), [s0] "+&v"(S0), [s1] "+&v"(S1), [e] "=&v"(E), [rk] "+&v"(rowkey)
+                : [f2] "v"(F2), [s2] "v"(S2), [ei] "v"(Ein), [z0] "s"(Z0), [z1] "s"(Z1), [dd] "v"(D), [k0] "n"(klit<FORM>(J)), [k1] "n"(klit<FORM>(J + 1)));
+        else if constexpr ((FORM & PF_KO_PERM) != 0) asm(NVB_PD3_CELL2(NVB_PD3_XOR2, "s_nop 0\n\t") : NVB_PD3_CELL2_OUT : NVB_PD3_CELL2_IN, [dd] "v"(D), [k0] "n"(klit<FORM>(J)), [k1] "n"(klit<FORM>(J + 1)));
+        else if constexpr ((FORM & PF_CONST2) != 0) asm(NVB_PD3_CELL2(NVB_PD3_PERM2, "s_nop 0\n\t") : NVB_PD3_CELL2_OUT : NVB_PD3_CELL2_IN, [dd] "v"(D), [k0] "n"(klit<FORM>(J)), [k1] "n"(klit<FORM>(J + 1)));
+        else                                        asm(NVB_PD3_CELL2(NVB_PD3_PERM2, "") : NVB_PD3_CELL2_OUT : NVB_PD3_CELL2_IN, [dd] "s"(D), [k0] "s"(K0), [k1] "s"(K1));
+    }
+
+#define NVB_PD3_TAIL2(L) L \
             "v_pk_max_u16 %[f0], %[s1], %[z0]\n\t" \
             "v_add_u32 %[d0], %[s0], %[d0]\n\t" \
             "v_add_u32 %[d1], %[s1], %[d1]\n\t" \
@@ -317,9 +345,14 @@
                                                  const uint32_t g0, const uint32_t g1, const uint32_t D, const uint32_t tlo, const uint32_t thi,
                                                  const uint32_t Z0, const uint32_t Z1, const uint32_t K0, const uint32_t K1)
     {
-        uint32_t d0, d1, h, e;
-        if constexpr ((FORM & PF_CONST2) != 0) asm(NVB_PD3_TAIL2 : NVB_PD3_TAIL2_OUT : NVB_PD3_TAIL2_IN, [dd] "v"(D), [k0] "n"(klit<FORM>(J)), [k1] "n"(klit<FORM>(J + 1)));
-        else                                   asm(NVB_PD3_TAIL2 : NVB_PD3_TAIL2_OUT : NVB_PD3_TAIL2_IN, [dd] "s"(D), [k0] "s"(K0), [k1] "s"(K1));
+        uint32_t d0 = g0, d1 = g1, h, e;
+        if constexpr ((FORM & PF_SUBLDS) != 0)
+            asm(NVB_PD3_TAIL2("")
+                : [f0] "=&v"(F0), [d0] "+&v"(d0), [d1] "+&v"(d1), [h] "=&v"(h), [e] "=&v"(e), [s0] "+&v"(S0), [s1] "+&v"(S1), [rk] "+&v"(rowkey)
+                : [ei] "v"(Ein), [z0] "s"(Z0), [z1] "s"(Z1), [dd] "v"(D), [k0] "n"(klit<FORM>(J)), [k1] "n"(klit<FORM>(J + 1)));
+        else if constexpr ((FORM & PF_KO_PERM) != 0) asm(NVB_PD3_TAIL2(NVB_PD3_XOR2) : NVB_PD3_TAIL2_OUT : NVB_PD3_TAIL2_IN, [dd] "v"(D), [k0] "n"(klit<FORM>(J)), [k1] "n"(klit<FORM>(J + 1)));
+        else if constexpr ((FORM & PF_CONST2) != 0) asm(NVB_PD3_TAIL2(NVB_PD3_PERM2) : NVB_PD3_TAIL2_OUT : NVB_PD3_TAIL2_IN, [dd] "v"(D), [k0] "n"(klit<FORM>(J)), [k1] "n"(klit<FORM>(J + 1)));
+        else                                        asm(NVB_PD3_TAIL2(NVB_PD3_PERM2) : NVB_PD3_TAIL2_OUT : NVB_PD3_TAIL2_IN, [dd] "s"(D), [k0] "s"(K0), [k1] "s"(K1));
     }
 
     template <int BAND, int R, int FORM, int J, int END>
@@ -335,6 +368,21 @@
     template <int BAND, int R, int FORM, int END>
     struct Cells<BAND, R, FORM, END, END> {
         static __device__ __forceinline__ void run(PairState<BAND>&, const ColumnFrame<BAND>&, const uint32_t Ein, uint32_t& E, uint32_t&, uint32_t, uint32_t) { E = Ein; }
+    };
+
+    template <int BAND, int R, int FORM, int J, int END>
+    struct SubCells {
+        static __device__ __forceinline__ void run(PairState<BAND>& st, const ColumnFrame<BAND>& fr, const uint32_t Ein, uint32_t& E, uint32_t& rowkey, const uint32_t (&w)[BAND])
+        {
+            uint32_t En;
+            cell2<FORM, J>(st.F[J], st.F[J + 1], st.F[J + 2], st.S[J], st.S[J + 1], st.S[J + 2], Ein, En, rowkey, w[J], w[J + 1], fr.D, 0u, 0u,
+                           fr.z[(2 * R + J) & 15], fr.z[(2 * R + J + 1) & 15], fr.k[J], fr.k[J + 1]);
+            SubCells<BAND, R, FORM, J + 2, END>::run(st, fr, En, E, rowkey, w);
+        }
+    };
+    template <int BAND, int R, int FORM, int END>
+    struct SubCells<BAND, R, FORM, END, END> {
+        static __device__ __forceinline__ void run(PairState<BAND>&, const ColumnFrame<BAND>&, const uint32_t Ein, uint32_t& E, uint32_t&, const uint32_t (&)[BAND]) { E = Ein; }
     };
 
     template <int BAND>
@@ -350,17 +398,36 @@
     }
 
     template <int BAND, int R, int FORM>
-    static __device__ __forceinline__ void row(PairState<BAND>& st, ColumnFrame<BAND>& fr, const uint32_t i, const uint32_t g_new, const uint32_t tlo, const uint32_t thi, uint32_t& rk2)
+    static __device__ __forceinline__ void row(PairState<BAND>& st, ColumnFrame<BAND>& fr, const uint32_t i, const uint32_t g_new, const uint32_t tlo, const uint32_t thi, uint32_t& rk2,
+                                               const uint32_t* sub = nullptr)
     {
         static_assert(BAND == 15, "a row's zeros, 2 i ... 2 i + BAND - 1, and the two the next row adds fill the ring of 16; columns go two at a time");
         fr.z[(2 * R + BAND - 2) & 15] += fr.step;
         fr.z[(2 * R + BAND - 1) & 15] += fr.step;
         uint32_t rowkey, E;
-        col0<FORM>(st.F[0], st.F[1], st.S[0], st.S[1], rowkey, st.tc[R & 15], fr.D, tlo, thi, fr.z[(2 * R) & 15], fr.k[0]);
-        Cells<BAND, R, FORM, 1, BAND - 2>::run(st, fr, st.S[0], E, rowkey, tlo, thi);
-        st.tc[(R + BAND - 1) & 15] = g_new;
-        tail2<FORM, BAND - 2>(st.F[BAND - 2], st.S[BAND - 2], st.S[BAND - 1], E, rowkey, st.tc[(R + BAND - 2) & 15], g_new, fr.D, tlo, thi,
-                              fr.z[(2 * R + BAND - 2) & 15], fr.z[(2 * R + BAND - 1) & 15], fr.k[BAND - 2], fr.k[BAND - 1]);
+        if constexpr ((FORM & PF_SUBLDS) != 0)
+        {
+            constexpr int HEAD = 8, SPLIT = 5;
+            st.tc[(R + BAND - 1) & 15] = g_new;
+            uint32_t w[BAND], Em;
+            #pragma unroll
+            for (int j = 0; j < HEAD; ++j) w[j] = *reinterpret_cast<const uint32_t*>(reinterpret_cast<const char*>(sub) + (tlo ^ st.tc[(R + j) & 15]));
+            col0<FORM>(st.F[0], st.F[1], st.S[0], st.S[1], rowkey, w[0], fr.D, 0u, 0u, fr.z[(2 * R) & 15], fr.k[0]);
+            SubCells<BAND, R, FORM, 1, SPLIT>::run(st, fr, st.S[0], Em, rowkey, w);
+            #pragma unroll
+            for (int j = HEAD; j < BAND; ++j) w[j] = *reinterpret_cast<const uint32_t*>(reinterpret_cast<const char*>(sub) + (tlo ^ st.tc[(R + j) & 15]));
+            SubCells<BAND, R, FORM, SPLIT, BAND - 2>::run(st, fr, Em, E, rowkey, w);
+            tail2<FORM, BAND - 2>(st.F[BAND - 2], st.S[BAND - 2], st.S[BAND - 1], E, rowkey, w[BAND - 2], w[BAND - 1], fr.D, 0u, 0u,
+                                  fr.z[(2 * R + BAND - 2) & 15], fr.z[(2 * R + BAND - 1) & 15], fr.k[BAND - 2], fr.k[BAND - 1]);
+        }
+        else
+        {
+            col0<FORM>(st.F[0], st.F[1], st.S[0], st.S[1], rowkey, st.tc[R & 15], fr.D, tlo, thi, fr.z[(2 * R) & 15], fr.k[0]);
+            Cells<BAND, R, FORM, 1, BAND - 2>::run(st, fr, st.S[0], E, rowkey, tlo, thi);
+            st.tc[(R + BAND - 1) & 15] = g_new;
+            tail2<FORM, BAND - 2>(st.F[BAND - 2], st.S[BAND - 2], st.S[BAND - 1], E, rowkey, st.tc[(R + BAND - 2) & 15], g_new, fr.D, tlo, thi,
+                                  fr.z[(2 * R + BAND - 2) & 15], fr.z[(2 * R + BAND - 1) & 15], fr.k[BAND - 2], fr.k[BAND - 1]);
+        }
         if constexpr ((FORM & PF_FOLD2) != 0)
         {
             if constexpr ((R & 1) == 0) rk2 = rowkey;
@@ -383,14 +450,24 @@
     {
         if ((FORM & PF_KO_BOUND) || i0 + R < M)
         {
-            const uint32_t g = ((XT[R >> 3] >> (2 * (R & 7))) & 0x00030003u) | CELL::SEL_BASE;
-            if constexpr (CELL::COLUMN)
+            if constexpr ((FORM & PF_SUBLDS) != 0)
             {
+                constexpr int K = R >> 1;
+                const uint32_t zw = uint32_t(((R & 1) ? PB : PA) >> (32 * (K >> 2))), xw = XT[R & 1];
+                uint32_t rw = (K & 3) == 0 ? (zw << 2) & 0x3FCu : (zw >> (8 * (K & 3) - 2)) & 0x3FCu;
+                uint32_t cw = K == 0 ? (xw << 2) & 0x3Cu : (xw >> (4 * K - 2)) & 0x3Cu;
+                asm("" : "+v"(rw)); asm("" : "+v"(cw));
+                CELL::template row<BAND, R, FORM>(st, fr, i0 + R, cw, rw, 0u, rk2, tab);
+            }
+            else if constexpr (CELL::COLUMN)
+            {
+                const uint32_t g = ((XT[R >> 3] >> (2 * (R & 7))) & 0x00030003u) | CELL::SEL_BASE;
                 if (FORM & PF_KO_TABLE) CELL::template row<BAND, R, FORM>(st, fr, i0 + R, g, KT[0], KT[1], rk2);
                 else                    CELL::template row<BAND, R, FORM>(st, fr, i0 + R, g, tab[uint32_t(PA >> (4 * R)) & 15u], tab[uint32_t(PB >> (4 * R)) & 15u], rk2);
             }
             else
             {
+                const uint32_t g = ((XT[R >> 3] >> (2 * (R & 7))) & 0x00030003u) | CELL::SEL_BASE;
                 if (FORM & PF_KO_TABLE) CELL::template row<BAND, R, FORM>(st, i0 + R, D, G, g, KT[0], KT[1]);
                 else                    CELL::template row<BAND, R, FORM>(st, i0 + R, D, G, g, tab[uint32_t(PA >> (4 * R)) & 15u], tab[uint32_t(PB >> (4 * R)) & 15u]);
             }
@@ -404,17 +481,27 @@
 
 constexpr int PAIR_LANES = 128;
 template <int BAND, typename CELL, int FORM>
-__global__ void __launch_bounds__(PAIR_LANES)
+__global__ void __launch_bounds__(PAIR_LANES) __attribute__((amdgpu_waves_per_eu((FORM & PF_SUBLDS) ? 5 : 1)))
 banded_gotoh_pair_kernel(const GotohParams p)
 {
     static_assert(BAND >= 3 && BAND <= 16, "the ring of 16");
-    constexpr bool STREAM = (FORM & PF_STREAM) != 0, KEY = (FORM & PF_SINK_KEY) != 0, FOLD2 = (FORM & PF_FOLD2) != 0;
+    constexpr bool STREAM = (FORM & PF_STREAM) != 0, KEY = (FORM & PF_SINK_KEY) != 0, FOLD2 = (FORM & PF_FOLD2) != 0, SUBLDS = (FORM & PF_SUBLDS) != 0;
+    static_assert(!(FORM & (PF_SUBLDS | PF_KO_PERM)) || ((FORM & PF_FOLD2) && (FORM & PF_CONST2) == PF_CONST2), "the LDS words and the probe's xor row are forms of the library's row");
+    static_assert(!SUBLDS || !(FORM & (PF_KO_TABLE | PF_KO_PERM)), "the LDS words have no lookup to knock out");
     static_assert(!(FORM & (PF_FOLD2 | PF_CONST2)) || CELL::COLUMN, "the pair fold and the literals are the column frame's");
     static_assert(!FOLD2 || !(FORM & (PF_SINK_KEY | PF_KO_SINK | PF_KO_BOUND)), "the pair fold is the compare-and-select fold's, over the job's own rows");
     static_assert(!(FORM & PF_GE3) || (FORM & PF_CONST2), "|G_e| is the literal form's parameter");
     constexpr bool P4 = !(FORM & PF_PAT2), PBE = (FORM & PF_PBE) != 0, TBE = (FORM & PF_TBE) != 0;
     __shared__ uint32_t s_tab[16];
-    if (threadIdx.x < 16u)
+    __shared__ uint32_t s_sub[256];
+    if constexpr (SUBLDS)
+    {
+        const uint32_t tg = uint32_t(-p.gap_ext * 32);
+        const uint32_t sm = uint32_t((p.match - p.gap_open) * 32) + tg, sx = uint32_t((p.mismatch - p.gap_open) * 32) + tg;
+        for (uint32_t k = threadIdx.x; k < 256u; k += uint32_t(PAIR_LANES))
+            s_sub[k] = (sub_code_a(k) == 0u ? sm : sx) | ((sub_code_b(k) == 0u ? sm : sx) << 16);
+    }
+    else if (threadIdx.x < 16u)
     {
         const uint32_t tg = CELL::COLUMN ? uint32_t(-p.gap_ext * 32) : 0u;
         const uint32_t sm = uint32_t((p.match - p.gap_open) * 32) + tg, sx = uint32_t((p.mismatch - p.gap_open) * 32) + tg;
@@ -451,7 +538,8 @@
         const uint32_t TA = fetch16_2bit(ts[0], tb[0]), TB = fetch16_2bit(ts[1], tb[1]);
         #pragma unroll
         for (int j = 0; j < BAND - 1; ++j)
-            st.tc[j] = CELL::SEL_BASE | ((TA >> (2 * j)) & 3u) | (((TB >> (2 * j)) & 3u) << 16);
+            st.tc[j] = SUBLDS ? (((TA >> (2 * j)) & 3u) | (((TB >> (2 * j)) & 3u) << 2)) << 2
+                              : CELL::SEL_BASE | ((TA >> (2 * j)) & 3u) | (((TB >> (2 * j)) & 3u) << 16);
     }
 
     const uint32_t plast = stream_last_off(p.pat.s), tlast = stream_last_off(p.txt.s);
@@ -487,8 +575,18 @@
             PAn = fetch_pattern16(ps[0], pb[0] + i0 + 16u); PBn = fetch_pattern16(ps[1], pb[1] + i0 + 16u);
             TAn = fetch16_2bit(ts[0], tb[0] + i0 + 16u + BAND - 1); TBn = fetch16_2bit(ts[1], tb[1] + i0 + 16u + BAND - 1);
         }
-        const uint32_t XT[2] = { (TA & 0xFFFFu) | (TB << 16), (TA >> 16) | (TB & 0xFFFF0000u) };
-        PairRows<CELL, BAND, FORM, 0, 16>::run(st, fr, i0, M, D, G, PA, PB, XT, s_tab, KT, rk2);
+        if constexpr (SUBLDS)
+        {
+            uint64_t RE, RO;
+            sub_row_words(PA, PB, RE, RO);
+            const uint32_t XT[2] = { sub_bfi(0x33333333u, TA, TB << 2), sub_bfi(0x33333333u, TA >> 2, TB) };
+            PairRows<CELL, BAND, FORM, 0, 16>::run(st, fr, i0, M, D, G, RE, RO, XT, s_sub, KT, rk2);
+        }
+        else
+        {
+            const uint32_t XT[2] = { (TA & 0xFFFFu) | (TB << 16), (TA >> 16) | (TB & 0xFFFF0000u) };
+            PairRows<CELL, BAND, FORM, 0, 16>::run(st, fr, i0, M, D, G, PA, PB, XT, s_tab, KT, rk2);
+        }
         if (FORM & PF_KO_FETCH)
         {
             PA = (PA << 4) | (PA >> 60); PB = (PB << 8) | (PB >> 56);
diff --git a/nvbio_amd/csrc/banded_gotoh_pair_b15_sub.hip b/nvbio_amd/csrc/banded_gotoh_pair_b15_sub.hip
--- /dev/null
+++ b/nvbio_amd/csrc/banded_gotoh_pair_b15_sub.hip
@@ -0,0 +1,6 @@
+#include "banded_gotoh_pair.h"
+namespace nvb {
+#define NVB_INST(CELL, F) template hipError_t launch_band_pair<15, CELL, (F)>(const GotohParams&, hipStream_t);
+NVB_PAIR_INSTANCES_B15_SUB(NVB_INST)
+#undef NVB_INST
+}
diff --git a/nvbio_amd/csrc/common.h b/nvbio_amd/csrc/common.h
--- a/nvbio_amd/csrc/common.h
+++ b/nvbio_amd/csrc/common.h
@@ -15,10 +15,11 @@
     const char* frame  = "";
     const char* row    = "";
     const char* consts = "";
+    const char* sub    = "";
 };
 extern thread_local PairLaunch g_last_pair;
 
-enum TestSwitch { SW_FORCE_32BIT = 0, SW_NO_STAGING, SW_FULL_GENERIC, SW_ED_SWEEP, SW_FULL_SINGLE_JOB, SW_FULL_ROWS, SW_TRACEBACK_LANES, SW_SELECT_LANES, SW_BANDED_PAIR, SW_PAIR_ROW, SW_PAIR_CONST, SW_COUNT };
+enum TestSwitch { SW_FORCE_32BIT = 0, SW_NO_STAGING, SW_FULL_GENERIC, SW_ED_SWEEP, SW_FULL_SINGLE_JOB, SW_FULL_ROWS, SW_TRACEBACK_LANES, SW_SELECT_LANES, SW_BANDED_PAIR, SW_PAIR_ROW, SW_PAIR_CONST, SW_PAIR_SUB, SW_COUNT };
 int test_switch(TestSwitch which);
 
 
```

Result: faster. 6.948 billion reads/s (median of 6 runs) (+4.9%).
